# marianaGarcez/SpatialFlink

Measured on AMD Instinct MI355X. Metric: points/sec per window (kNN k=50, range r) at 1/2/4/8 MI355X; % HBM roofline, higher is better.
Workload: dtype f64

## Files before the change

### include/geoflink_hip.h

```cpp
#ifndef GEOFLINK_HIP_H
#define GEOFLINK_HIP_H

#include <stddef.h>
#include <stdint.h>

#ifdef __cplusplus
extern "C" {
#endif

#define GF_ABI_VERSION 2

#define GF_OK             0
#define GF_ERR_ARG       -1
#define GF_ERR_CAPACITY  -2
#define GF_ERR_HIP       -3
#define GF_ERR_NOMEM     -4
#define GF_ERR_LAYERS    -5
#define GF_ERR_ALIGN     -7
#define GF_ERR_COMM      -8

#define GF_METRIC_SQRT  0
#define GF_METRIC_HYPOT 1

#define GF_K_KNN_SCAN    0
#define GF_K_KNN_SAMPLE  1
#define GF_K_KNN_SELECT  2
#define GF_K_RANGE_SCAN  3
#define GF_K_ASSIGN      4
#define GF_K_JOIN_PROBE  5
#define GF_K_RANGE_TEST  6
#define GF_K_JOIN_BUCKET 7
#define GF_K_KNN_MERGE   8
#define GF_K_CSV_PARSE   9
#define GF_K_BUCKET      10
#define GF_K_JOIN_COMPACT 11
#define GF_K_TRAJ_GROUP  12
#define GF_K_TSTATS      13
#define GF_K_TRAJ_SELECT 14
#define GF_K_TAGG        15
#define GF_K_TKNN        16
#define GF_K_TJOIN       17
#define GF_K_TRANGE      18
#define GF_K_GEOM        19
#define GF_K_COUNT       20

typedef struct gf_ctx gf_ctx;

typedef struct {
  int32_t n;
  int32_t reserved;
  double minX, maxX, minY, maxY;
  double cellLength;
} gf_grid;

#define GF_OBJID_NUMERIC_MIN (-(INT64_C(1) << 62))
#define GF_OBJID_NUMERIC_END (INT64_C(1) << 62)
#define GF_OBJID_NULL INT64_MAX
typedef struct gf_objid_dict gf_objid_dict;

typedef struct {
  const double* x;
  const double* y;
  const int64_t* objID;
  const int64_t* ts;
  int64_t n;
} gf_points;

typedef struct {
  int32_t npoly;
  const int32_t* ring_off;
  const int32_t* vert_off;
  const double* vx;
  const double* vy;
} gf_polygons;

typedef struct {
  int32_t nline;
  const int32_t* vert_off;
  const double* vx;
  const double* vy;
} gf_linestrings;

int         gf_abi_version(void);
const char* gf_build_info(void);
int         gf_build_is_product(void);
const char* gf_status_string(int status);
int         gf_device_count(int* n);
int         gf_ctx_create(int device, gf_ctx** out);
void        gf_ctx_destroy(gf_ctx* ctx);
int         gf_ctx_set_stream(gf_ctx* ctx, void* hip_stream);
void*       gf_ctx_stream(gf_ctx* ctx);
int         gf_ctx_synchronize(gf_ctx* ctx);
int         gf_ctx_join(gf_ctx* ctx);
int         gf_ctx_fork(gf_ctx* ctx);
const char* gf_ctx_last_error(gf_ctx* ctx);
#define GF_FLAG_JOIN_LEGACY 1
#define GF_FLAG_JOIN_COARSE 2
#define GF_FLAG_GEOJSON_WALK 4
#define GF_FLAG_JOIN_STREAM 8
#define GF_FLAG_GEOJSON_WAVE 16
#define GF_FLAG_GEOJSON_CHECK 32
int gf_ctx_set_flag(gf_ctx* ctx, int flag, int value);
int gf_geojson_check_counts(gf_ctx* ctx, unsigned long long out[4]);

int         gf_ctx_set_timing(gf_ctx* ctx, int mask);
int         gf_ctx_set_timing_period(gf_ctx* ctx, int period);
int         gf_ctx_timing(gf_ctx* ctx, int kernel_id, double* total_ms, int64_t* launches);

int gf_grid_make(int32_t n, double minX, double maxX, double minY, double maxY, gf_grid* out);
int gf_grid_layers(const gf_grid* g, double r, int32_t* guaranteed, int32_t* candidate);
int gf_cell_of(const gf_grid* g, double x, double y, int32_t* cx, int32_t* cy);
int gf_format_cell_id(int32_t cx, int32_t cy, char* buf, int32_t cap);
int gf_parse_cell_id(const char* id, int32_t* cx, int32_t* cy);

int gf_assign_cells(gf_ctx* ctx, const gf_grid* g, const gf_points* pts, int32_t* cx, int32_t* cy);

int gf_bucket_by_cell(gf_ctx* ctx, const gf_grid* g, const gf_points* pts, uint32_t* perm,
                      uint32_t* cell_start);

int gf_shard_by_columns(gf_ctx* ctx, const gf_grid* g, const gf_points* pts, int32_t nbands, const int32_t* band_lo,
                        uint32_t* perm, uint32_t* offsets);
int gf_gather_points(gf_ctx* ctx, const gf_points* pts, const uint32_t* perm, int64_t begin, int64_t end, double* x,
                     double* y, int64_t* objID, int64_t* ts);

typedef struct gf_range_plan gf_range_plan;
int  gf_range_pp_plan_create(gf_ctx* ctx, const gf_grid* g, const double* qx, const double* qy,
                             int32_t nq, double r, int approximate, int metric, gf_range_plan** out);
int  gf_range_ppoly_plan_create(gf_ctx* ctx, const gf_grid* g, const gf_polygons* polys, double r,
                                int approximate, int metric, gf_range_plan** out);
void gf_range_plan_destroy(gf_range_plan* plan);
int  gf_range_run(gf_range_plan* plan, const gf_points* pts, uint64_t* bitmap,
                  uint64_t* multi_bitmap, int64_t* counts);
int  gf_range_run_batch(gf_range_plan* plan, int32_t nwin, const gf_points* pts, uint64_t* const* bitmaps,
                        int64_t* const* counts, uint32_t* const* idx, const int64_t* idx_cap, int64_t* const* idx_count);
int  gf_range_plan_stats(const gf_range_plan* plan, int64_t* none_cells, int64_t* candidate_cells,
                         int64_t* guaranteed_cells, int64_t* inside_cells);
int  gf_range_plan_set_tuning(gf_range_plan* plan, int32_t scan_blocks, int32_t defer_mode);
int  gf_range_plan_set_drain_lanes(gf_range_plan* plan, int32_t lanes);
int  gf_bitmap_to_indices(gf_ctx* ctx, const uint64_t* bitmap, int64_t n, uint32_t* idx,
                          int64_t cap, int64_t* count);
int  gf_bitmap_to_indices_async(gf_ctx* ctx, const uint64_t* bitmap, int64_t n, uint32_t* idx,
                                int64_t cap, int64_t* count);

typedef struct gf_knn_plan gf_knn_plan;
int    gf_knn_pp_plan_create(gf_ctx* ctx, const gf_grid* g, double qx, double qy, double r,
                             int32_t k, int metric, gf_knn_plan** out);
int    gf_knn_ppoly_plan_create(gf_ctx* ctx, const gf_grid* g, const gf_polygons* polys, double r, int32_t k,
                                int approximate, int metric, gf_knn_plan** out);
void   gf_knn_plan_destroy(gf_knn_plan* plan);
int    gf_knn_plan_set_capacity(gf_knn_plan* plan, int64_t cap);
int    gf_knn_plan_set_tuning(gf_knn_plan* plan, int32_t scan_blocks, int32_t unroll, int32_t nontemporal);
int    gf_knn_plan_set_hint(gf_knn_plan* plan, int enable);
int    gf_knn_plan_set_index_base(gf_knn_plan* plan, int64_t base);
int    gf_knn_plan_set_pipeline(gf_knn_plan* plan, int depth);
int    gf_knn_plan_flush(gf_knn_plan* plan);
typedef struct {
  int32_t status;
  int32_t n;
  int32_t k;
  int32_t flags;
  int64_t candidates;
  double threshold;
} gf_knn_header;
size_t gf_knn_result_bytes(int32_t k);
int    gf_knn_enqueue(gf_knn_plan* plan, const gf_points* pts, void* result);
int    gf_knn_decode(gf_knn_plan* plan, const gf_points* pts, const void* result_host,
                     int64_t* objID, double* dist, int64_t* idx, int32_t* n_out);
int    gf_knn_run(gf_knn_plan* plan, const gf_points* pts, int64_t* objID, double* dist,
                  int64_t* idx, int32_t* n_out);
int    gf_knn_merge_dev(gf_ctx* ctx, int32_t k, const void* records, int32_t nrec, void* result);
#define GF_MERGE_SHARD_MAJOR  0
#define GF_MERGE_WINDOW_MAJOR 1
#define GF_MERGE_FOREIGN_KEYS 0x100
#define GF_KNN_STATUS_FOREIGN_KEYS 2
int    gf_knn_merge_dev_batch(gf_ctx* ctx, int32_t k, const void* records, int32_t nrec, int32_t nwin,
                              int32_t layout, void* results);
size_t gf_knn_string_record_bytes(int32_t k, int64_t cap_bytes);
int gf_knn_attach_strings(gf_objid_dict* dict, int32_t k, const void* records, int32_t nrec, int64_t cap_bytes,
                          void* out);
int gf_knn_merge_dev_strings(gf_ctx* ctx, int32_t k, int64_t cap_bytes, const void* records, int32_t nrec,
                             int32_t nwin, int32_t layout, void* results);
int gf_knn_string_record_decode(const void* record, int32_t k, int64_t cap_bytes, int32_t* status, int64_t* objID,
                                double* dist, int64_t* idx, char* buf, int64_t buf_cap, int64_t* offs, int32_t* n_out);
int    gf_knn_merge_host(int32_t k, int32_t nlists, const int32_t* counts, const int64_t* objID,
                         const double* dist, const int64_t* idx, int64_t* out_objID,
                         double* out_dist, int64_t* out_idx, int32_t* n_out);

#define GF_COMM_ID_BYTES 128
typedef struct gf_comm gf_comm;
int  gf_comm_available(void);
int  gf_comm_unique_id(uint8_t* id);
int  gf_comm_create(const uint8_t* id, int32_t nranks, int32_t rank, int device, gf_comm** out);
int  gf_comm_create_all(int32_t ndev, const int* devices, gf_comm** out );
void gf_comm_destroy(gf_comm* comm);
int  gf_comm_info(const gf_comm* comm, int32_t* nranks, int32_t* rank, int* device);
const char* gf_comm_last_error(const gf_comm* comm);
int  gf_comm_check(gf_comm* comm);
int gf_knn_exchange_batch(gf_comm* comm, gf_ctx* ctx, int32_t k, const void* records, int32_t nwin, void* merged);
int gf_knn_exchange_strings_batch(gf_comm* comm, gf_objid_dict* dict, int32_t k, int64_t cap_bytes,
                                  const void* records, int32_t nwin, void* merged);
int gf_knn_exchange_group(int32_t n, gf_comm* const* comms, gf_ctx* const* ctxs, int32_t k,
                          const void* const* records, int32_t nwin, void* const* merged);

typedef struct gf_knn_sliding gf_knn_sliding;
int  gf_knn_sliding_create(gf_knn_plan* plan, int64_t size_ms, int64_t slide_ms, gf_knn_sliding** out);
void gf_knn_sliding_destroy(gf_knn_sliding* s);
int  gf_knn_sliding_geometry(const gf_knn_sliding* s, int64_t* pane_ms, int32_t* panes_per_window,
                             int32_t* panes_per_slide, int32_t* ring_panes);
int  gf_knn_sliding_push(gf_knn_sliding* s, int64_t pane_index, const gf_points* pane, void* window_result,
                         int32_t* closed, int64_t* window_end);
int  gf_knn_sliding_flush(gf_knn_sliding* s);
int  gf_knn_sliding_decode(gf_knn_sliding* s, int64_t window_end, const void* result_host, int64_t* objID,
                           double* dist, int64_t* idx, int32_t* n_out);

typedef struct gf_range_sliding gf_range_sliding;
int  gf_range_sliding_create(gf_range_plan* plan, int64_t size_ms, int64_t slide_ms, gf_range_sliding** out);
void gf_range_sliding_destroy(gf_range_sliding* s);
int  gf_range_sliding_geometry(const gf_range_sliding* s, int64_t* pane_ms, int32_t* panes_per_window,
                               int32_t* panes_per_slide);
int  gf_range_sliding_push(gf_range_sliding* s, int64_t pane_index, const gf_points* pane, uint32_t* idx,
                           int64_t cap, int64_t* count, int32_t* closed, int64_t* window_end, int64_t* window_n);

int  gf_pane_bounds(gf_ctx* ctx, const int64_t* ts, int64_t n, int64_t pane_ms, int64_t first_pane, int32_t npanes,
                    int64_t* bounds);

int  gf_objid_dict_create(gf_ctx* ctx, gf_objid_dict** out);
void gf_objid_dict_destroy(gf_objid_dict* d);
int  gf_ctx_objid_dict(gf_ctx* ctx, gf_objid_dict** out);
int  gf_objid_dict_size(const gf_objid_dict* d, int64_t* n);
int  gf_objid_intern(gf_objid_dict* d, const char* bytes, const int64_t* offs, int64_t n, int64_t* keys);
int  gf_objid_decode(gf_objid_dict* d, const int64_t* keys, int64_t n, char* buf, int64_t cap, int64_t* offs);

typedef struct {
  char delimiter;
  char reserved[3];
  int32_t objid_field;
  int32_t time_field;
  int32_t x_field;
  int32_t y_field;
} gf_csv_schema;
#define GF_CSV_OK              0
#define GF_CSV_NUMBER_FORMAT   1
#define GF_CSV_UNSUPPORTED     2
#define GF_CSV_MISSING_FIELD   3
#define GF_CSV_EMPTY_LINE      4
int gf_csv_parse(gf_ctx* ctx, const char* text, int64_t len, const gf_csv_schema* schema, const gf_grid* grid,
                 double* x, double* y, int64_t* objID, int64_t* ts, int32_t* cx, int32_t* cy, int64_t cap,
                 int64_t* n_out, int64_t* bad_line, int32_t* bad_kind);
int gf_csv_parse_dict(gf_ctx* ctx, gf_objid_dict* dict, const char* text, int64_t len, const gf_csv_schema* schema,
                      const gf_grid* grid, double* x, double* y, int64_t* objID, int64_t* ts, int32_t* cx, int32_t* cy,
                      int64_t cap, int64_t* n_out, int64_t* bad_line, int32_t* bad_kind);

typedef struct {
  const char* objid_property;
  const char* time_property;
  int32_t date_format;
  int32_t tz_offset_minutes;
  int32_t value_lines;
} gf_geojson_schema;
int gf_geojson_parse(gf_ctx* ctx, gf_objid_dict* dict, const char* text, int64_t len, const gf_geojson_schema* schema,
                     const gf_grid* grid, double* x, double* y, int64_t* objID, int64_t* ts, int32_t* cx,
                     int32_t* cy, int64_t cap, int64_t* n_out, int64_t* bad_line, int32_t* bad_kind);

typedef struct {
  int32_t kind;
  int64_t obj_cap, ring_cap, vert_cap;
  int32_t* ring_off;
  int32_t* vert_off;
  double *vx, *vy;
  int64_t *objID, *ts;
} gf_geoms_out;
int gf_geojson_parse_geoms(gf_ctx* ctx, gf_objid_dict* dict , const char* text, int64_t len,
                           const gf_geojson_schema* schema, const gf_geoms_out* out, int64_t* nobj, int64_t* nrings,
                           int64_t* nverts, int64_t* bad_line, int32_t* bad_kind);

int gf_join_pp(gf_ctx* ctx, const gf_grid* ugrid, const gf_grid* qgrid, const gf_points* ordinary,
               const gf_points* query, double r, int approximate, int metric, uint32_t* pairs,
               int64_t cap, int64_t* npairs);
int gf_join_pp_async(gf_ctx* ctx, const gf_grid* ugrid, const gf_grid* qgrid, const gf_points* ordinary,
                     const gf_points* query, double r, int approximate, int metric, uint32_t* pairs,
                     int64_t cap, unsigned long long* total);

int gf_join_ppoly_plan_create(gf_ctx* ctx, const gf_grid* qgrid, const gf_polygons* polys, double r,
                              int approximate, int metric, gf_range_plan** out);
int gf_join_ppoly_run(gf_range_plan* plan, const gf_grid* ugrid, const gf_points* points, uint32_t* pairs,
                      int64_t cap, int64_t* npairs);
int gf_join_ppoly(gf_ctx* ctx, const gf_grid* ugrid, const gf_grid* qgrid, const gf_points* points,
                  const gf_polygons* polys, double r, int approximate, int metric, uint32_t* pairs,
                  int64_t cap, int64_t* npairs);

int gf_range_pls_plan_create(gf_ctx* ctx, const gf_grid* g, const gf_linestrings* lines, double r,
                             int approximate, int metric, gf_range_plan** out);
int gf_knn_pls_plan_create(gf_ctx* ctx, const gf_grid* g, const gf_linestrings* lines , double r,
                           int32_t k, int approximate, int metric, gf_knn_plan** out);
int gf_join_pls_plan_create(gf_ctx* ctx, const gf_grid* qgrid, const gf_linestrings* lines, double r,
                            int approximate, int metric, gf_range_plan** out);
int gf_join_pls(gf_ctx* ctx, const gf_grid* ugrid, const gf_grid* qgrid, const gf_points* points,
                const gf_linestrings* lines, double r, int approximate, int metric, uint32_t* pairs,
                int64_t cap, int64_t* npairs);
int gf_range_plan_set_chain_mode(gf_range_plan* plan, int mode);
int gf_knn_plan_set_chain_mode(gf_knn_plan* plan, int mode);

typedef struct gf_traj_groups gf_traj_groups;
int  gf_traj_group(gf_ctx* ctx, const gf_points* pts, gf_traj_groups** out);
void gf_traj_groups_destroy(gf_traj_groups* g);
int  gf_traj_groups_info(const gf_traj_groups* g, int64_t* ntraj, int64_t* n);
int  gf_traj_groups_read(gf_traj_groups* g, int64_t* keys, int64_t* seg_off, uint32_t* perm);
int  gf_traj_groups_set_long_threshold(gf_traj_groups* g, int64_t len);
int  gf_tstats_run(gf_traj_groups* g, const gf_points* pts, const int64_t* id_set, int64_t nset,
                   int64_t* keys, double* spatial, int64_t* temporal, double* speed, int64_t cap, int64_t* count);
int  gf_traj_select(gf_traj_groups* g, const gf_points* pts, const uint64_t* bitmap, int64_t* keys, int64_t* off,
                    int64_t cap_traj, double* x, double* y, int64_t* ts, uint32_t* idx, int64_t cap_pts,
                    int64_t* ntraj_out, int64_t* npts_out);

typedef struct gf_tagg gf_tagg;
int  gf_tagg_group(gf_ctx* ctx, const gf_grid* grid, const gf_points* pts, gf_tagg** out);
int  gf_tagg_run(gf_tagg* t, const gf_points* pts);
void gf_tagg_destroy(gf_tagg* t);
int  gf_tagg_info(const gf_tagg* t, int64_t* cells, int64_t* groups, int64_t* n);
int  gf_tagg_set_thresholds(gf_tagg* t, int64_t long_group, int64_t big_cell);
int  gf_tagg_read_cells(gf_tagg* t, int32_t* cx, int32_t* cy, int64_t* count, int64_t* multi, int64_t* sum,
                        int64_t* minLen, int64_t* minKey, int64_t* maxLen, int64_t* maxKey, int64_t cap, int64_t* cells);
int  gf_tagg_read_all(gf_tagg* t, int64_t* off, int64_t* keys, int64_t* len, int64_t cap_cells, int64_t cap_groups,
                      int64_t* cells, int64_t* groups);
int  gf_tagg_rows(const char* function, int64_t cells, const int64_t* count, const int64_t* multi, const int64_t* sum,
                  const int64_t* minLen, const int64_t* minKey, const int64_t* maxLen, const int64_t* maxKey,
                  uint8_t* emit, int64_t* value, int64_t* key, int32_t* kind);

#define GF_TKNN_GRID  0
#define GF_TKNN_NAIVE 1
typedef struct gf_tknn gf_tknn;
int  gf_tknn_run(gf_traj_groups* g, const gf_grid* grid, const gf_points* pts, double qx, double qy, double r,
                 int32_t k, int mode, gf_tknn** out);
void gf_tknn_destroy(gf_tknn* t);
int  gf_tknn_info(const gf_tknn* t, int64_t* rows, int64_t* npts, int64_t* in_cells, int64_t* pairs, int64_t* records);
int  gf_tknn_read(gf_tknn* t, int64_t* keys, double* dist, int32_t* cells, int64_t* off, int64_t cap_rows, double* x,
                  double* y, int64_t* ts, uint32_t* idx, int64_t cap_pts);
int  gf_tknn_set_thresholds(gf_tknn* t, int64_t big_cell);

#define GF_TJOIN_PAIR 0
#define GF_TJOIN_SINGLE 1
typedef struct gf_tjoin gf_tjoin;
int  gf_tjoin_run(gf_traj_groups* go, const gf_points* opts, gf_traj_groups* gq, const gf_points* qpts,
                  const gf_grid* grid, double r, int mode, gf_tjoin** out);
void gf_tjoin_destroy(gf_tjoin* t);
int  gf_tjoin_info(const gf_tjoin* t, int64_t* rows, int64_t* emitted, int64_t* otraj, int64_t* opoints,
                   int64_t* qtraj, int64_t* qpoints, int64_t* probe_passes);
int  gf_tjoin_read_rows(gf_tjoin* t, int64_t* okey, int64_t* qkey, uint32_t* p_first, uint32_t* q_latest,
                        uint8_t* emit, int32_t* oslot, int32_t* qslot, int64_t cap);
int  gf_tjoin_read_trajs(gf_tjoin* t, int side, int64_t* keys, int64_t* off, int64_t cap_traj,
                         double* x, double* y, int64_t* ts, uint32_t* idx, int64_t cap_pts);
int  gf_tjoin_set_table_slots(gf_tjoin* t, int64_t slots);

typedef struct gf_trange_plan gf_trange_plan;
int  gf_trange_plan_create(gf_ctx* ctx, const gf_grid* g, const gf_polygons* polys, gf_trange_plan** out);
void gf_trange_plan_destroy(gf_trange_plan* p);
int  gf_trange_plan_stats(const gf_trange_plan* p, int64_t* none_cells, int64_t* test_cells, int64_t* inside_cells,
                          int64_t* list_entries, int64_t* wide_polygons);
int  gf_trange_plan_set_thresholds(gf_trange_plan* p, int32_t wide_ring);
int  gf_trange_points(gf_trange_plan* p, const gf_points* pts, uint64_t* bitmap, int64_t* count);
int  gf_trange_run(gf_trange_plan* p, gf_traj_groups* g, const gf_points* pts, int64_t* keys, int64_t* off,
                   int64_t cap_traj, double* x, double* y, int64_t* ts, uint32_t* idx, int64_t cap_pts,
                   int64_t* ntraj_out, int64_t* npts_out);
int  gf_trange_info(const gf_trange_plan* p, int64_t* cell_points, int64_t* inside_points, int64_t* wide_ring,
                    int64_t* wave_path);
int  gf_tfilter_run(gf_traj_groups* g, const gf_points* pts, const int64_t* id_set, int64_t nset, int64_t* keys,
                    int64_t* off, int64_t cap_traj, double* x, double* y, int64_t* ts, uint32_t* idx, int64_t cap_pts,
                    int64_t* ntraj_out, int64_t* npts_out);

#define GF_GEOM_POLYGON    1
#define GF_GEOM_LINESTRING 2
typedef struct {
  int32_t kind;
  int32_t nrings;
  int64_t nobj;
  const int32_t* ring_off;
  const int32_t* vert_off;
  const double* vx;
  const double* vy;
  const int64_t* objID;
  const int64_t* ts;
} gf_geoms;
typedef struct gf_geom_index gf_geom_index;
int  gf_geom_prepare(gf_ctx* ctx, const gf_grid* g, const gf_geoms* geoms, gf_geom_index** out);
void gf_geom_index_destroy(gf_geom_index* ix);
int  gf_geom_index_info(gf_geom_index* ix, int64_t* nobj, int64_t* nvert, int64_t* invalid, int64_t* wide);
int  gf_geom_index_read(gf_geom_index* ix, double* env, int32_t* cells);
int  gf_geom_index_set_thresholds(gf_geom_index* ix, int32_t wide_vertices);
typedef struct gf_geom_query gf_geom_query;
int  gf_geom_query_create(gf_ctx* ctx, const gf_grid* g, const double* qx, const double* qy, int32_t nq, double r,
                          int approximate, int metric, gf_geom_query** out);
void gf_geom_query_destroy(gf_geom_query* q);
int  gf_geom_range_run(gf_geom_query* q, gf_geom_index* ix, uint64_t* bitmap, int64_t* counts);
int  gf_geom_knn_enqueue(gf_geom_query* q, gf_geom_index* ix, int32_t k, void* result);
int  gf_geom_info(const gf_geom_query* q, int64_t* filtered, int64_t* all_guaranteed, int64_t* tested,
                  int64_t* wave_path);

int  gf_geom_query_create_polygons(gf_ctx* ctx, const gf_grid* g, const gf_polygons* polys, double r, int approximate,
                                   int metric, gf_geom_query** out);
int  gf_geom_query_create_linestrings(gf_ctx* ctx, const gf_grid* g, const gf_linestrings* lines, double r,
                                      int approximate, int metric, gf_geom_query** out);
int  gf_geom_query_set_chain_mode(gf_geom_query* q, int mode);

typedef struct gf_geom_join gf_geom_join;
int  gf_geom_join_create(gf_ctx* ctx, gf_geom_join** out);
void gf_geom_join_destroy(gf_geom_join* j);
int  gf_geom_join_run(gf_geom_join* j, gf_geom_index* ix_ord, gf_geom_index* ix_qry, double r, int approximate, int metric,
                      int first_is_ordinary, uint32_t* pairs, int64_t cap, int64_t* npairs, int64_t* nrep);
int  gf_geom_join_run_points(gf_geom_join* j, gf_geom_index* ix_ord, const gf_grid* qgrid, const gf_points* q, double r,
                             int approximate, int metric, uint32_t* pairs, int64_t cap, int64_t* npairs, int64_t* nrep);
int  gf_geom_join_info(const gf_geom_join* j, int64_t* candidates, int64_t* box_dropped, int64_t* tested,
                       int64_t* wave_path, int64_t* long_objects, int64_t* long_queries);
int  gf_geom_join_set_tuning(gf_geom_join* j, int32_t tile_side, int64_t long_tiles, int brute);

int  gf_pinned_alloc(size_t bytes, void** ptr);
void gf_pinned_free(void* ptr);

typedef struct gf_window gf_window;
int  gf_window_create(gf_ctx* ctx, int64_t capacity, gf_window** out);
void gf_window_destroy(gf_window* w);
int  gf_window_upload(gf_window* w, const double* x, const double* y, const int64_t* objID,
                      const int64_t* ts, int64_t n);
int  gf_window_points(gf_window* w, gf_points* out);
int  gf_window_upload_mapped(gf_window* w, const double* x, const double* y, const int64_t* objID_pinned, int64_t n);
int  gf_host_pinned(const void* p, int* pinned);

int gf_synth_uniform(int64_t seed, int64_t n, double minX, double maxX, double minY, double maxY,
                     double* x, double* y);

#ifdef __cplusplus
}
#endif
#endif
```

### spatialflink_amd/_lib.py

```python
from __future__ import annotations

import ctypes as C
import os
import threading

_HERE = os.path.dirname(os.path.abspath(__file__))
LIB_PATH = os.environ.get("GF_LIB_PATH") or os.path.join(_HERE, "libgeoflink_hip.so")

GF_OK = 0
OBJID_NUMERIC_MIN, OBJID_NUMERIC_END = -(1 << 62), 1 << 62
OBJID_NULL = (1 << 63) - 1
GF_MERGE_SHARD_MAJOR, GF_MERGE_WINDOW_MAJOR = 0, 1
GF_MERGE_FOREIGN_KEYS = 0x100
KNN_STATUS_FOREIGN_KEYS = 2
GF_ERR_ARG = -1
GF_ERR_CAPACITY = -2
GF_ERR_HIP = -3
GF_ERR_NOMEM = -4
GF_ERR_LAYERS = -5
GF_ERR_ALIGN = -7
GF_ERR_COMM = -8
GF_COMM_ID_BYTES = 128

METRIC_SQRT = 0
METRIC_HYPOT = 1
TKNN_GRID = 0
TKNN_NAIVE = 1
TJOIN_PAIR = 0
TJOIN_SINGLE = 1

FLAG_JOIN_LEGACY = 1
FLAG_JOIN_COARSE = 2
FLAG_GEOJSON_WALK = 4
FLAG_GEOJSON_WAVE = 16
FLAG_GEOJSON_CHECK = 32
FLAG_JOIN_STREAM = 8
(K_KNN_SCAN, K_KNN_SAMPLE, K_KNN_SELECT, K_RANGE_SCAN, K_ASSIGN, K_JOIN_PROBE, K_RANGE_TEST, K_JOIN_BUCKET,
 K_KNN_MERGE, K_CSV_PARSE, K_BUCKET, K_JOIN_COMPACT, K_TRAJ_GROUP, K_TSTATS, K_TRAJ_SELECT, K_TAGG, K_TKNN,
 K_TJOIN, K_TRANGE, K_GEOM) = range(20)
GEOM_POLYGON = 1
GEOM_LINESTRING = 2

EXPORTS = [
    "gf_abi_version", "gf_build_info", "gf_build_is_product", "gf_status_string", "gf_device_count", "gf_ctx_create", "gf_ctx_destroy",
    "gf_ctx_set_stream", "gf_ctx_stream", "gf_ctx_synchronize", "gf_ctx_join", "gf_ctx_fork", "gf_ctx_last_error", "gf_ctx_set_timing", "gf_ctx_set_timing_period", "gf_ctx_set_flag",
    "gf_geojson_check_counts",
    "gf_ctx_timing", "gf_grid_make", "gf_grid_layers", "gf_cell_of", "gf_format_cell_id", "gf_parse_cell_id",
    "gf_assign_cells", "gf_bucket_by_cell", "gf_range_pp_plan_create", "gf_range_ppoly_plan_create",
    "gf_range_plan_destroy", "gf_range_run", "gf_range_run_batch", "gf_range_plan_stats", "gf_range_plan_set_tuning", "gf_range_plan_set_drain_lanes", "gf_bitmap_to_indices", "gf_bitmap_to_indices_async", "gf_knn_pp_plan_create",
    "gf_knn_ppoly_plan_create",
    "gf_knn_plan_destroy", "gf_knn_plan_set_capacity", "gf_knn_plan_set_index_base", "gf_knn_plan_set_tuning", "gf_knn_plan_set_hint", "gf_knn_plan_set_pipeline", "gf_knn_plan_flush",
    "gf_knn_result_bytes", "gf_knn_enqueue",
    "gf_knn_decode", "gf_knn_run", "gf_knn_merge_dev", "gf_knn_merge_dev_batch", "gf_knn_merge_host",
    "gf_knn_sliding_create", "gf_knn_sliding_destroy", "gf_knn_sliding_geometry", "gf_knn_sliding_push",
    "gf_knn_sliding_flush", "gf_knn_sliding_decode", "gf_range_sliding_create", "gf_range_sliding_destroy",
    "gf_range_sliding_geometry", "gf_range_sliding_push", "gf_pane_bounds", "gf_csv_parse", "gf_csv_parse_dict", "gf_geojson_parse",
    "gf_geojson_parse_geoms",
    "gf_objid_dict_create", "gf_objid_dict_destroy", "gf_ctx_objid_dict", "gf_objid_dict_size", "gf_objid_intern",
    "gf_objid_decode", "gf_join_pp", "gf_join_pp_async",
    "gf_join_ppoly_plan_create", "gf_join_ppoly_run", "gf_join_ppoly",
    "gf_range_pls_plan_create", "gf_knn_pls_plan_create", "gf_join_pls_plan_create", "gf_join_pls",
    "gf_range_plan_set_chain_mode", "gf_knn_plan_set_chain_mode",
    "gf_window_create",
    "gf_window_destroy", "gf_window_upload", "gf_window_points", "gf_synth_uniform", "gf_pinned_alloc",
    "gf_pinned_free", "gf_knn_string_record_bytes", "gf_knn_attach_strings", "gf_knn_merge_dev_strings",
    "gf_knn_string_record_decode", "gf_window_upload_mapped", "gf_shard_by_columns", "gf_gather_points",
    "gf_host_pinned", "gf_comm_available", "gf_comm_unique_id", "gf_comm_create", "gf_comm_create_all",
    "gf_comm_destroy", "gf_comm_info", "gf_comm_last_error", "gf_comm_check", "gf_knn_exchange_batch",
    "gf_knn_exchange_strings_batch", "gf_knn_exchange_group",
    "gf_traj_group", "gf_traj_groups_destroy", "gf_traj_groups_info", "gf_traj_groups_read",
    "gf_traj_groups_set_long_threshold", "gf_tstats_run", "gf_traj_select",
    "gf_tagg_group", "gf_tagg_run", "gf_tagg_destroy", "gf_tagg_info", "gf_tagg_set_thresholds", "gf_tagg_read_cells",
    "gf_tagg_read_all", "gf_tagg_rows",
    "gf_tknn_run", "gf_tknn_destroy", "gf_tknn_info", "gf_tknn_read", "gf_tknn_set_thresholds",
    "gf_tjoin_run", "gf_tjoin_destroy", "gf_tjoin_info", "gf_tjoin_read_rows", "gf_tjoin_read_trajs",
    "gf_tjoin_set_table_slots",
    "gf_trange_plan_create", "gf_trange_plan_destroy", "gf_trange_plan_stats", "gf_trange_plan_set_thresholds",
    "gf_trange_points", "gf_trange_run", "gf_trange_info", "gf_tfilter_run",
    "gf_geom_prepare", "gf_geom_index_destroy", "gf_geom_index_info", "gf_geom_index_read",
    "gf_geom_index_set_thresholds", "gf_geom_query_create", "gf_geom_query_destroy", "gf_geom_range_run",
    "gf_geom_knn_enqueue", "gf_geom_info",
    "gf_geom_query_create_polygons", "gf_geom_query_create_linestrings", "gf_geom_query_set_chain_mode",
    "gf_geom_join_create", "gf_geom_join_destroy", "gf_geom_join_run", "gf_geom_join_run_points", "gf_geom_join_info",
    "gf_geom_join_set_tuning",
]


class GfGrid(C.Structure):
    _fields_ = [("n", C.c_int32), ("reserved", C.c_int32), ("minX", C.c_double), ("maxX", C.c_double),
                ("minY", C.c_double), ("maxY", C.c_double), ("cellLength", C.c_double)]


class GfPoints(C.Structure):
    _fields_ = [("x", C.c_void_p), ("y", C.c_void_p), ("objID", C.c_void_p), ("ts", C.c_void_p),
                ("n", C.c_int64)]


class GfPolygons(C.Structure):
    _fields_ = [("npoly", C.c_int32), ("ring_off", C.c_void_p), ("vert_off", C.c_void_p),
                ("vx", C.c_void_p), ("vy", C.c_void_p)]


class GfLineStrings(C.Structure):
    _fields_ = [("nline", C.c_int32), ("vert_off", C.c_void_p), ("vx", C.c_void_p), ("vy", C.c_void_p)]


class GfGeomsOut(C.Structure):
    _fields_ = [("kind", C.c_int32), ("obj_cap", C.c_int64), ("ring_cap", C.c_int64), ("vert_cap", C.c_int64),
                ("ring_off", C.c_void_p), ("vert_off", C.c_void_p), ("vx", C.c_void_p), ("vy", C.c_void_p),
                ("objID", C.c_void_p), ("ts", C.c_void_p)]


class GfGeoms(C.Structure):
    _fields_ = [("kind", C.c_int32), ("nrings", C.c_int32), ("nobj", C.c_int64), ("ring_off", C.c_void_p),
                ("vert_off", C.c_void_p), ("vx", C.c_void_p), ("vy", C.c_void_p), ("objID", C.c_void_p),
                ("ts", C.c_void_p)]


class GfKnnHeader(C.Structure):
    _fields_ = [("status", C.c_int32), ("n", C.c_int32), ("k", C.c_int32), ("flags", C.c_int32),
                ("candidates", C.c_int64), ("threshold", C.c_double)]


class GeoFlinkError(RuntimeError):
    def __init__(self, status, msg=""):
        self.status = status
        super().__init__(f"{msg} (status {status}: {status_string(status) if _lib else ''})")


class CandidateLayersError(GeoFlinkError):
    """The reference's System.exit(1): 'candidateNeighboringLayers cannot be 0 or less'
    (UniformGrid.java:272-276), raised instead of terminating the process."""


_lib = None
_lock = threading.Lock()


def lib():
    global _lib
    if _lib is not None:
        return _lib
    with _lock:
        if _lib is not None:
            return _lib
        if not os.path.exists(LIB_PATH):
            raise ImportError(
                f"{LIB_PATH} is missing: build it with `make` (or __graft_entry__.build()). "
                "There is no CPU fallback for the window-evaluation path.")
        import torch

        L = C.CDLL(LIB_PATH)
        P, i32, i64, d, sz = C.c_void_p, C.c_int32, C.c_int64, C.c_double, C.c_size_t
        pi32, pi64, pd = C.POINTER(i32), C.POINTER(i64), C.POINTER(d)
        sig = {
            "gf_abi_version": ([], C.c_int),
            "gf_build_info": ([], C.c_char_p),
            "gf_build_is_product": ([], C.c_int),
            "gf_status_string": ([C.c_int], C.c_char_p),
            "gf_device_count": ([C.POINTER(C.c_int)], C.c_int),
            "gf_ctx_create": ([C.c_int, C.POINTER(P)], C.c_int),
            "gf_ctx_destroy": ([P], None),
            "gf_ctx_set_stream": ([P, P], C.c_int),
            "gf_ctx_stream": ([P], P),
            "gf_ctx_synchronize": ([P], C.c_int),
            "gf_ctx_join": ([P], C.c_int),
            "gf_ctx_fork": ([P], C.c_int),
            "gf_ctx_last_error": ([P], C.c_char_p),
            "gf_ctx_set_timing": ([P, C.c_int], C.c_int),
            "gf_ctx_set_flag": ([P, C.c_int, C.c_int], C.c_int),
            "gf_geojson_check_counts": ([P, P], C.c_int),
            "gf_ctx_set_timing_period": ([P, C.c_int], C.c_int),
            "gf_ctx_timing": ([P, C.c_int, pd, pi64], C.c_int),
            "gf_grid_make": ([i32, d, d, d, d, C.POINTER(GfGrid)], C.c_int),
            "gf_grid_layers": ([C.POINTER(GfGrid), d, pi32, pi32], C.c_int),
            "gf_cell_of": ([C.POINTER(GfGrid), d, d, pi32, pi32], C.c_int),
            "gf_format_cell_id": ([i32, i32, C.c_char_p, i32], C.c_int),
            "gf_parse_cell_id": ([C.c_char_p, pi32, pi32], C.c_int),
            "gf_assign_cells": ([P, C.POINTER(GfGrid), C.POINTER(GfPoints), P, P], C.c_int),
            "gf_bucket_by_cell": ([P, C.POINTER(GfGrid), C.POINTER(GfPoints), P, P], C.c_int),
            "gf_range_pp_plan_create": ([P, C.POINTER(GfGrid), P, P, i32, d, C.c_int, C.c_int, C.POINTER(P)], C.c_int),
            "gf_range_ppoly_plan_create": ([P, C.POINTER(GfGrid), C.POINTER(GfPolygons), d, C.c_int, C.c_int,
                                            C.POINTER(P)], C.c_int),
            "gf_range_plan_destroy": ([P], None),
            "gf_range_run": ([P, C.POINTER(GfPoints), P, P, P], C.c_int),
            "gf_range_run_batch": ([P, i32, C.POINTER(GfPoints), C.POINTER(P), C.POINTER(P), C.POINTER(P), pi64,
                                    C.POINTER(P)], C.c_int),
            "gf_range_plan_stats": ([P, pi64, pi64, pi64, pi64], C.c_int),
            "gf_range_plan_set_tuning": ([P, C.c_int32, C.c_int32], C.c_int),
            "gf_range_plan_set_drain_lanes": ([P, i32], C.c_int),
            "gf_bitmap_to_indices": ([P, P, i64, P, i64, pi64], C.c_int),
            "gf_bitmap_to_indices_async": ([P, P, i64, P, i64, P], C.c_int),
            "gf_knn_pp_plan_create": ([P, C.POINTER(GfGrid), d, d, d, i32, C.c_int, C.POINTER(P)], C.c_int),
            "gf_knn_ppoly_plan_create": ([P, C.POINTER(GfGrid), C.POINTER(GfPolygons), d, i32, C.c_int, C.c_int,
                                          C.POINTER(P)], C.c_int),
            "gf_knn_plan_destroy": ([P], None),
            "gf_knn_plan_set_capacity": ([P, i64], C.c_int),
            "gf_knn_plan_set_index_base": ([P, i64], C.c_int),
            "gf_knn_plan_set_tuning": ([P, i32, i32, i32], C.c_int),
            "gf_knn_plan_set_hint": ([P, C.c_int], C.c_int),
            "gf_knn_plan_set_pipeline": ([P, C.c_int], C.c_int),
            "gf_knn_plan_flush": ([P], C.c_int),
            "gf_knn_result_bytes": ([i32], sz),
            "gf_knn_enqueue": ([P, C.POINTER(GfPoints), P], C.c_int),
            "gf_knn_decode": ([P, C.POINTER(GfPoints), P, P, P, P, pi32], C.c_int),
            "gf_knn_run": ([P, C.POINTER(GfPoints), P, P, P, pi32], C.c_int),
            "gf_knn_merge_dev": ([P, i32, P, i32, P], C.c_int),
            "gf_knn_merge_dev_batch": ([P, i32, P, i32, i32, i32, P], C.c_int),
            "gf_knn_merge_host": ([i32, i32, P, P, P, P, P, P, P, pi32], C.c_int),
            "gf_knn_sliding_create": ([P, i64, i64, C.POINTER(P)], C.c_int),
            "gf_knn_sliding_destroy": ([P], None),
            "gf_knn_sliding_geometry": ([P, pi64, pi32, pi32, pi32], C.c_int),
            "gf_knn_sliding_push": ([P, i64, C.POINTER(GfPoints), P, pi32, pi64], C.c_int),
            "gf_knn_sliding_flush": ([P], C.c_int),
            "gf_knn_sliding_decode": ([P, i64, P, P, P, P, pi32], C.c_int),
            "gf_range_sliding_create": ([P, i64, i64, C.POINTER(P)], C.c_int),
            "gf_range_sliding_destroy": ([P], None),
            "gf_range_sliding_geometry": ([P, pi64, pi32, pi32], C.c_int),
            "gf_range_sliding_push": ([P, i64, C.POINTER(GfPoints), P, i64, P, pi32, pi64, pi64], C.c_int),
            "gf_pane_bounds": ([P, P, i64, i64, i64, i32, P], C.c_int),
            "gf_csv_parse": ([P, P, i64, P, C.POINTER(GfGrid), P, P, P, P, P, P, i64, pi64, pi64, pi32], C.c_int),
            "gf_geojson_parse": ([P, P, P, i64, P, C.POINTER(GfGrid), P, P, P, P, P, P, i64, pi64, pi64, pi32],
                                 C.c_int),
            "gf_geojson_parse_geoms": ([P, P, P, i64, P, C.POINTER(GfGeomsOut), pi64, pi64, pi64, pi64, pi32], C.c_int),
            "gf_csv_parse_dict": ([P, P, P, i64, P, C.POINTER(GfGrid), P, P, P, P, P, P, i64, pi64, pi64, pi32],
                                  C.c_int),
            "gf_objid_dict_create": ([P, C.POINTER(P)], C.c_int),
            "gf_objid_dict_destroy": ([P], None),
            "gf_ctx_objid_dict": ([P, C.POINTER(P)], C.c_int),
            "gf_objid_dict_size": ([P, pi64], C.c_int),
            "gf_objid_intern": ([P, C.c_char_p, P, i64, P], C.c_int),
            "gf_objid_decode": ([P, P, i64, P, i64, P], C.c_int),
            "gf_join_pp": ([P, C.POINTER(GfGrid), C.POINTER(GfGrid), C.POINTER(GfPoints), C.POINTER(GfPoints), d,
                            C.c_int, C.c_int, P, i64, pi64], C.c_int),
            "gf_join_pp_async": ([P, C.POINTER(GfGrid), C.POINTER(GfGrid), C.POINTER(GfPoints), C.POINTER(GfPoints), d,
                                  C.c_int, C.c_int, P, i64, P], C.c_int),
            "gf_join_ppoly_plan_create": ([P, C.POINTER(GfGrid), C.POINTER(GfPolygons), d, C.c_int, C.c_int,
                                           C.POINTER(P)], C.c_int),
            "gf_join_ppoly_run": ([P, C.POINTER(GfGrid), C.POINTER(GfPoints), P, i64, pi64], C.c_int),
            "gf_join_ppoly": ([P, C.POINTER(GfGrid), C.POINTER(GfGrid), C.POINTER(GfPoints), C.POINTER(GfPolygons), d,
                               C.c_int, C.c_int, P, i64, pi64], C.c_int),
            "gf_range_pls_plan_create": ([P, C.POINTER(GfGrid), C.POINTER(GfLineStrings), d, C.c_int, C.c_int,
                                          C.POINTER(P)], C.c_int),
            "gf_knn_pls_plan_create": ([P, C.POINTER(GfGrid), C.POINTER(GfLineStrings), d, i32, C.c_int, C.c_int,
                                        C.POINTER(P)], C.c_int),
            "gf_join_pls_plan_create": ([P, C.POINTER(GfGrid), C.POINTER(GfLineStrings), d, C.c_int, C.c_int,
                                         C.POINTER(P)], C.c_int),
            "gf_join_pls": ([P, C.POINTER(GfGrid), C.POINTER(GfGrid), C.POINTER(GfPoints), C.POINTER(GfLineStrings), d,
                             C.c_int, C.c_int, P, i64, pi64], C.c_int),
            "gf_range_plan_set_chain_mode": ([P, C.c_int], C.c_int),
            "gf_knn_plan_set_chain_mode": ([P, C.c_int], C.c_int),
            "gf_window_create": ([P, i64, C.POINTER(P)], C.c_int),
            "gf_window_destroy": ([P], None),
            "gf_window_upload": ([P, P, P, P, P, i64], C.c_int),
            "gf_window_points": ([P, C.POINTER(GfPoints)], C.c_int),
            "gf_window_upload_mapped": ([P, P, P, P, i64], C.c_int),
            "gf_shard_by_columns": ([P, C.POINTER(GfGrid), C.POINTER(GfPoints), i32, P, P, P], C.c_int),
            "gf_gather_points": ([P, C.POINTER(GfPoints), P, i64, i64, P, P, P, P], C.c_int),
            "gf_host_pinned": ([P, C.POINTER(C.c_int)], C.c_int),
            "gf_synth_uniform": ([i64, i64, d, d, d, d, P, P], C.c_int),
            "gf_pinned_alloc": ([sz, C.POINTER(P)], C.c_int),
            "gf_pinned_free": ([P], None),
            "gf_knn_string_record_bytes": ([i32, i64], sz),
            "gf_knn_attach_strings": ([P, i32, P, i32, i64, P], C.c_int),
            "gf_knn_merge_dev_strings": ([P, i32, i64, P, i32, i32, i32, P], C.c_int),
            "gf_knn_string_record_decode": ([P, i32, i64, pi32, P, P, P, P, i64, P, pi32], C.c_int),
            "gf_comm_available": ([], C.c_int),
            "gf_comm_unique_id": ([P], C.c_int),
            "gf_comm_create": ([P, i32, i32, C.c_int, C.POINTER(P)], C.c_int),
            "gf_comm_create_all": ([i32, P, P], C.c_int),
            "gf_comm_destroy": ([P], None),
            "gf_comm_info": ([P, pi32, pi32, C.POINTER(C.c_int)], C.c_int),
            "gf_comm_last_error": ([P], C.c_char_p),
            "gf_comm_check": ([P], C.c_int),
            "gf_knn_exchange_batch": ([P, P, i32, P, i32, P], C.c_int),
            "gf_knn_exchange_strings_batch": ([P, P, i32, i64, P, i32, P], C.c_int),
            "gf_knn_exchange_group": ([i32, P, P, i32, P, i32, P], C.c_int),
            "gf_traj_group": ([P, C.POINTER(GfPoints), C.POINTER(P)], C.c_int),
            "gf_traj_groups_destroy": ([P], None),
            "gf_traj_groups_info": ([P, pi64, pi64], C.c_int),
            "gf_traj_groups_read": ([P, P, P, P], C.c_int),
            "gf_traj_groups_set_long_threshold": ([P, i64], C.c_int),
            "gf_tstats_run": ([P, C.POINTER(GfPoints), P, i64, P, P, P, P, i64, pi64], C.c_int),
            "gf_traj_select": ([P, C.POINTER(GfPoints), P, P, P, i64, P, P, P, P, i64, pi64, pi64], C.c_int),
            "gf_tagg_group": ([P, C.POINTER(GfGrid), C.POINTER(GfPoints), C.POINTER(P)], C.c_int),
            "gf_tagg_run": ([P, C.POINTER(GfPoints)], C.c_int),
            "gf_tagg_destroy": ([P], None),
            "gf_tagg_info": ([P, pi64, pi64, pi64], C.c_int),
            "gf_tagg_set_thresholds": ([P, i64, i64], C.c_int),
            "gf_tagg_read_cells": ([P, P, P, P, P, P, P, P, P, P, i64, pi64], C.c_int),
            "gf_tagg_read_all": ([P, P, P, P, i64, i64, pi64, pi64], C.c_int),
            "gf_tagg_rows": ([C.c_char_p, i64, P, P, P, P, P, P, P, P, P, P, pi32], C.c_int),
            "gf_tknn_run": ([P, C.POINTER(GfGrid), C.POINTER(GfPoints), C.c_double, C.c_double, C.c_double, C.c_int32,
                             C.c_int, C.POINTER(P)], C.c_int),
            "gf_tknn_destroy": ([P], None),
            "gf_tknn_info": ([P, pi64, pi64, pi64, pi64, pi64], C.c_int),
            "gf_tknn_read": ([P, P, P, P, P, i64, P, P, P, P, i64], C.c_int),
            "gf_tknn_set_thresholds": ([P, i64], C.c_int),
            "gf_tjoin_run": ([P, C.POINTER(GfPoints), P, C.POINTER(GfPoints), C.POINTER(GfGrid), C.c_double, C.c_int,
                              C.POINTER(P)], C.c_int),
            "gf_tjoin_destroy": ([P], None),
            "gf_tjoin_info": ([P, pi64, pi64, pi64, pi64, pi64, pi64, pi64], C.c_int),
            "gf_tjoin_read_rows": ([P, P, P, P, P, P, P, P, i64], C.c_int),
            "gf_tjoin_read_trajs": ([P, C.c_int, P, P, i64, P, P, P, P, i64], C.c_int),
            "gf_tjoin_set_table_slots": ([P, i64], C.c_int),
            "gf_trange_plan_create": ([P, C.POINTER(GfGrid), C.POINTER(GfPolygons), C.POINTER(P)], C.c_int),
            "gf_trange_plan_destroy": ([P], None),
            "gf_trange_plan_stats": ([P, pi64, pi64, pi64, pi64, pi64], C.c_int),
            "gf_trange_plan_set_thresholds": ([P, C.c_int32], C.c_int),
            "gf_trange_points": ([P, C.POINTER(GfPoints), P, P], C.c_int),
            "gf_trange_run": ([P, P, C.POINTER(GfPoints), P, P, i64, P, P, P, P, i64, pi64, pi64], C.c_int),
            "gf_trange_info": ([P, pi64, pi64, pi64, pi64], C.c_int),
            "gf_tfilter_run": ([P, C.POINTER(GfPoints), P, i64, P, P, i64, P, P, P, P, i64, pi64, pi64], C.c_int),
            "gf_geom_prepare": ([P, C.POINTER(GfGrid), C.POINTER(GfGeoms), C.POINTER(P)], C.c_int),
            "gf_geom_index_destroy": ([P], None),
            "gf_geom_index_info": ([P, pi64, pi64, pi64, pi64], C.c_int),
            "gf_geom_index_read": ([P, P, P], C.c_int),
            "gf_geom_index_set_thresholds": ([P, i32], C.c_int),
            "gf_geom_query_create": ([P, C.POINTER(GfGrid), P, P, i32, d, C.c_int, C.c_int, C.POINTER(P)], C.c_int),
            "gf_geom_query_destroy": ([P], None),
            "gf_geom_range_run": ([P, P, P, P], C.c_int),
            "gf_geom_knn_enqueue": ([P, P, i32, P], C.c_int),
            "gf_geom_info": ([P, pi64, pi64, pi64, pi64], C.c_int),
            "gf_geom_query_create_polygons": ([P, C.POINTER(GfGrid), C.POINTER(GfPolygons), d, C.c_int, C.c_int,
                                              C.POINTER(P)], C.c_int),
            "gf_geom_query_create_linestrings": ([P, C.POINTER(GfGrid), C.POINTER(GfLineStrings), d, C.c_int, C.c_int,
                                                 C.POINTER(P)], C.c_int),
            "gf_geom_query_set_chain_mode": ([P, C.c_int], C.c_int),
            "gf_geom_join_create": ([P, C.POINTER(P)], C.c_int),
            "gf_geom_join_destroy": ([P], None),
            "gf_geom_join_run": ([P, P, P, d, C.c_int, C.c_int, C.c_int, P, i64, pi64, pi64], C.c_int),
            "gf_geom_join_run_points": ([P, P, C.POINTER(GfGrid), C.POINTER(GfPoints), d, C.c_int, C.c_int, P, i64, pi64,
                                         pi64], C.c_int),
            "gf_geom_join_info": ([P, pi64, pi64, pi64, pi64, pi64, pi64], C.c_int),
            "gf_geom_join_set_tuning": ([P, i32, i64, C.c_int], C.c_int),
        }
        for name, (argt, rest) in sig.items():
            if os.environ.get("GF_LIB_PATH") and not hasattr(L, name):
                continue
            fn = getattr(L, name)
            fn.argtypes = argt
            fn.restype = rest
        _lib = L
        return _lib


def status_string(s):
    return lib().gf_status_string(int(s)).decode()


def check(status, ctx=None, what=""):
    if status == GF_OK:
        return
    detail = ""
    if ctx is not None:
        try:
            detail = lib().gf_ctx_last_error(ctx).decode()
        except Exception:
            detail = ""
    msg = f"{what}: {detail}" if detail else what
    if status == GF_ERR_LAYERS:
        raise CandidateLayersError(status, msg or "candidateNeighboringLayers cannot be 0 or less")
    if status == GF_ERR_ARG:
        raise ValueError(f"{msg} (IllegalArgumentException)")
    raise GeoFlinkError(status, msg)


class Context:

    def __init__(self, device: int = 0):
        h = C.c_void_p()
        st = lib().gf_ctx_create(int(device), C.byref(h))
        if st != GF_OK:
            raise GeoFlinkError(st, f"gf_ctx_create(device={device}) failed: is a GPU visible?")
        self.handle = h
        self.device = device

    def __del__(self):
        h = getattr(self, "handle", None)
        if h and _lib is not None:
            _lib.gf_ctx_destroy(h)
            self.handle = None

    def set_stream(self, stream_ptr: int | None):
        check(lib().gf_ctx_set_stream(self.handle, C.c_void_p(stream_ptr or 0)), self.handle, "set_stream")

    def synchronize(self):
        check(lib().gf_ctx_synchronize(self.handle), self.handle, "synchronize")

    def set_timing(self, mask: int):
        check(lib().gf_ctx_set_timing(self.handle, int(mask)), self.handle, "set_timing")

    def set_timing_period(self, period: int):
        check(lib().gf_ctx_set_timing_period(self.handle, int(period)), self.handle, "set_timing_period")

    def timing(self, kernel_id: int):
        ms, n = C.c_double(), C.c_int64()
        check(lib().gf_ctx_timing(self.handle, int(kernel_id), C.byref(ms), C.byref(n)), self.handle, "timing")
        return ms.value, n.value


_ctx_cache: dict = {}


def context(device: int | None = None) -> Context:
    import torch

    if device is None:
        device = torch.cuda.current_device()
    key = (int(device), threading.get_ident())
    ctx = _ctx_cache.get(key)
    if ctx is None:
        ctx = Context(int(device))
        _ctx_cache[key] = ctx
    ctx.set_stream(torch.cuda.current_stream(device).cuda_stream)
    return ctx


def device_count() -> int:
    n = C.c_int()
    lib().gf_device_count(C.byref(n))
    return n.value
```

### spatialflink_amd/csrc/geomingest.cpp

```cpp
#define GF_TU_NAME geomingest_cpp
#include "gf_buildtag.hpp"

#include <cstring>
#include <string>

#include "gf_host.hpp"
#include "k_geomingest.hpp"

using namespace gf;

constexpr int64_t kGeomMeanLineDefault = 768;

static int32_t geom_lds_cap(int64_t mean) {
  const int64_t cap = (mean * kGeomLines * 5 / 4 + 1023) & ~(int64_t)1023;
  return (int32_t)std::min<int64_t>(std::max<int64_t>(cap, 16 * 1024), kCsvLdsMax);
}

static int geom_bad_line(gf_ctx* ctx, const CsvErr& he, int64_t* bad_line, int32_t* bad_kind) {
  if (bad_line) *bad_line = (int64_t)he.line;
  if (bad_kind) *bad_kind = he.kind;
  static const char* what[] = {"ok", "a position's ordinate is not a number",
                               "outside the restated subset (see gf_geojson_parse_geoms)",
                               "malformed JSON / no geometry / a ring or linestring JTS refuses", "empty line"};
  const int k = he.kind >= 0 && he.kind <= 4 ? he.kind : 1;
  return set_err(ctx, GF_ERR_ARG, "gf_geojson_parse_geoms: line " + std::to_string(he.line) + ": " + what[k]);
}

extern "C" int gf_geojson_parse_geoms(gf_ctx* ctx, gf_objid_dict* dict, const char* text, int64_t len,
                                      const gf_geojson_schema* sc, const gf_geoms_out* out, int64_t* nobj,
                                      int64_t* nrings, int64_t* nverts, int64_t* bad_line, int32_t* bad_kind) {
  if (!ctx) return GF_ERR_ARG;
  const char* fn = "gf_geojson_parse_geoms: ";
  if (!sc || (sc->date_format != 0 && sc->date_format != 1) || (sc->value_lines != 0 && sc->value_lines != 1))
    return set_err(ctx, GF_ERR_ARG, std::string(fn) + "bad schema");
  if (!out || (out->kind != GF_GEOM_POLYGON && out->kind != GF_GEOM_LINESTRING))
    return set_err(ctx, GF_ERR_ARG, std::string(fn) + "kind must be GF_GEOM_POLYGON or GF_GEOM_LINESTRING");
  const bool poly = out->kind == GF_GEOM_POLYGON;
  const int64_t obj_cap = out->obj_cap, ring_cap = poly ? out->ring_cap : 0, vert_cap = out->vert_cap;
  const bool any_cap = obj_cap > 0 || ring_cap > 0 || vert_cap > 0;
  if (!nobj || !nrings || !nverts || len < 0 || (len > 0 && !text) || obj_cap < 0 || out->ring_cap < 0 || vert_cap < 0 ||
      (obj_cap > 0 && (!out->objID || !out->ts)) || (vert_cap > 0 && (!out->vx || !out->vy)) ||
      (any_cap && !out->vert_off) || (poly && any_cap && !out->ring_off))
    return set_err(ctx, GF_ERR_ARG, std::string(fn) + "bad argument");
  if ((uintptr_t)text & 15) return set_err(ctx, GF_ERR_ALIGN, std::string(fn) + "text must be 16-byte aligned");
  if (len >= ((int64_t)1 << 33)) return set_err(ctx, GF_ERR_ARG, std::string(fn) + "text of 8 GiB or more");
  if (dict && dict->ctx != ctx) return set_err(ctx, GF_ERR_ARG, std::string(fn) + "dictionary of another context");
  GeomIngestArgs a{};
  a.len_obj = a.len_ts = -1;
  for (int k = 0; k < 2; ++k) {
    const char* name = k ? sc->time_property : sc->objid_property;
    if (!name) continue;
    const size_t n = std::strlen(name);
    if (n >= (size_t)kGeoPropMax) return set_err(ctx, GF_ERR_ARG, std::string(fn) + "property name longer than 63 bytes");
    std::memcpy(k ? a.prop_ts : a.prop_obj, name, n);
    (k ? a.len_ts : a.len_obj) = (int32_t)n;
  }
  int st = bind(ctx);
  if (st) return st;
  if (!dict && (st = ctx_dict(ctx, &dict))) return st;
  *nobj = *nrings = *nverts = 0;
  if (bad_line) *bad_line = -1;
  if (bad_kind) *bad_kind = GF_CSV_OK;
  if (len == 0) {
    if (out->vert_off) GF_HIP_CHECK(ctx, hipMemsetAsync(out->vert_off, 0, sizeof(int32_t), ctx->stream));
    if (poly && out->ring_off) GF_HIP_CHECK(ctx, hipMemsetAsync(out->ring_off, 0, sizeof(int32_t), ctx->stream));
    GF_HIP_CHECK(ctx, hipStreamSynchronize(ctx->stream));
    return GF_OK;
  }
  a.text = text;
  a.len = len;
  a.kind = out->kind;
  a.value_lines = sc->value_lines;
  a.date_fmt = sc->date_format;
  a.tz_off_ms = (int64_t)sc->tz_offset_minutes * 60000;
  a.lds_cap = geom_lds_cap(ctx->geom_mean_line > 0 ? ctx->geom_mean_line : kGeomMeanLineDefault);
  const int64_t nseg = (len + kCsvSeg - 1) / kCsvSeg;
  int64_t nl_cap = len / 32 + 2;
  GeomHead h{};
  GeomHead* d_head = nullptr;
  for (int pass = 0; pass < 2; ++pass) {
    const int64_t G = nl_cap + 1;
    Arena ar;
    uint32_t *tot = nullptr, *cnt_r = nullptr, *cnt_v = nullptr, *off_r = nullptr, *off_v = nullptr;
    CsvErr* err = nullptr;
    int64_t* nl = nullptr;
    ar.take(d_head, 1);
    ar.take(tot, 1);
    ar.take(err, 1);
    ar.take(nl, (size_t)nl_cap);
    ar.take(cnt_r, (size_t)G);
    ar.take(cnt_v, (size_t)G);
    ar.take(off_r, (size_t)G + 1);
    ar.take(off_v, (size_t)G + 1);
    ar.take(a.cpos, (size_t)G);
    ar.take(a.tcode, (size_t)G);
    ar.take(a.ts_s, (size_t)G);
    ar.take(a.obj_s, (size_t)G);
    const size_t tmp_n = (size_t)std::max<int64_t>(ring_cap, 1);
    ar.take(a.tmp.area, tmp_n);
    ar.take(a.tmp.start, tmp_n);
    ar.take(a.tmp.count, tmp_n);
    ar.take(a.tmp.order, tmp_n);
    if ((st = ar.alloc(ctx))) return st;
    if ((st = dict_reserve_batch(dict, (uint64_t)G, (uint64_t)G))) return st;
    if ((st = lookback_launch(ctx, nseg, nseg, "launch_csv_nlindex", [&](const ExpandState& es) {
          return launch_csv_nlindex(ctx->stream, text, len, nseg, nl, nl_cap, tot, es, err, dict->counters + 2);
        })))
      return st;
    a.nl = nl;
    a.nl_total = tot;
    a.nl_cap = nl_cap;
    a.grid_lines = G;
    a.cnt_r = cnt_r;
    a.cnt_v = cnt_v;
    a.off_r = off_r;
    a.off_v = off_v;
    a.err = err;
    a.head = d_head;
    a.dict_work = (DictWork*)dict->work[0];
    a.dict_n = (uint32_t*)(dict->counters + 2);
    a.dict_bytes = dict->counters + 3;
    GF_HIP_CHECK(ctx, launch_geomingest_a(ctx, a));
    if ((st = scan1(ctx, cnt_r, G, off_r))) return st;
    if ((st = scan1(ctx, cnt_v, G, off_v))) return st;
    GF_HIP_CHECK(ctx, launch_geomingest_head(ctx, a));
    if ((st = read_scalar_sync(ctx, d_head, &h))) return st;
    if ((int64_t)h.newlines <= nl_cap) break;
    nl_cap = (int64_t)h.newlines + 1;
  }
  const int64_t lines = (int64_t)h.lines;
  if (lines >= (int64_t)INT32_MAX) return set_err(ctx, GF_ERR_ARG, std::string(fn) + "2^31 - 1 lines or more");
  if (h.err.line != ~0ull) {
    a.fill = 0;
    a.limit = (int64_t)h.err.line;
    if (a.limit > 0) {
      GF_HIP_CHECK(ctx, launch_geomingest_b(ctx, a));
      GF_HIP_CHECK(ctx, launch_geomingest_head(ctx, a));
      if ((st = read_scalar_sync(ctx, d_head, &h))) return st;
    }
    return geom_bad_line(ctx, h.err, bad_line, bad_kind);
  }
  if (h.nrings > (unsigned long long)INT32_MAX || h.nverts > (unsigned long long)INT32_MAX)
    return set_err(ctx, GF_ERR_ARG, std::string(fn) + "the window's rings or vertices do not fit int32 offsets");
  *nobj = lines;
  *nrings = (int64_t)h.nrings;
  *nverts = (int64_t)h.nverts;
  ctx->geom_mean_line = (len + lines - 1) / lines;
  if (lines > obj_cap || *nrings > ring_cap || *nverts > vert_cap)
    return set_err(ctx, GF_ERR_CAPACITY, std::string(fn) + "the window exceeds a capacity (counts returned)");
  a.fill = 1;
  a.limit = lines;
  a.lds_cap = geom_lds_cap(ctx->geom_mean_line);
  a.ring_off = out->ring_off;
  a.vert_off = out->vert_off;
  a.vx = out->vx;
  a.vy = out->vy;
  a.objID = out->objID;
  a.ts = out->ts;
  GF_HIP_CHECK(ctx, launch_geomingest_b(ctx, a));
  GF_HIP_CHECK(ctx, launch_geomingest_head(ctx, a));
  if ((st = read_scalar_sync(ctx, d_head, &h))) return st;
  if (h.err.line != ~0ull) return geom_bad_line(ctx, h.err, bad_line, bad_kind);
  const uint32_t nw = (uint32_t)h.dict_n;
  if (nw > 0) {
    if ((st = dict_reserve_table(dict, nw, h.dict_bytes))) return st;
    if ((st = dict_run(dict, text, 1, nw, (uint64_t)lines, out->objID))) return st;
  }
  return GF_OK;
}
```

### spatialflink_amd/csrc/gf_geojson.hpp

```cpp
#pragma once

#include <cstdint>

#include "gf_text.hpp"

namespace gf {

GF_DHD inline bool jws(char c) { return c == ' ' || c == '\t' || c == '\n' || c == '\r'; }
template <class Src>
GF_DHD inline int64_t jskip(const Src& s, int64_t p, int64_t e) {
  while (p < e && jws(s(p))) ++p;
  return p;
}
template <class Src>
GF_DHD inline int64_t jstr_end(const Src& s, int64_t p, int64_t e, bool* esc) {
  for (++p; p < e; ++p) {
    const char c = s(p);
    if (c == '\\') {
      *esc = true;
      ++p;
    } else if (c == '"') {
      return p + 1;
    }
  }
  return -1;
}
template <class Src>
GF_DHD inline int64_t jval_end(const Src& s, int64_t p, int64_t e) {
  char c = s(p);
  if (c == '"') {
    bool esc = false;
    return jstr_end(s, p, e, &esc);
  }
  if (c == '{' || c == '[') {
    int depth = 0;
    while (p < e) {
      c = s(p);
      if (c == '"') {
        bool esc = false;
        p = jstr_end(s, p, e, &esc);
        if (p < 0) return -1;
        continue;
      }
      if (c == '{' || c == '[') ++depth;
      else if ((c == '}' || c == ']') && --depth == 0) return p + 1;
      ++p;
    }
    return -1;
  }
  int64_t q = p;
  while (q < e && !(s(q) == ',' || s(q) == '}' || s(q) == ']' || jws(s(q)))) ++q;
  return q > p ? q : -1;
}
template <class Src>
GF_DHD inline int64_t jfind(const Src& s, int64_t p, int64_t e, const char* key, int klen) {
  int64_t found = -1;
  bool esc_key = false;
  p = jskip(s, p + 1, e);
  if (p < e && s(p) == '}') return -1;
  while (p < e && s(p) == '"') {
    bool esc = false;
    const int64_t ke = jstr_end(s, p, e, &esc);
    if (ke < 0) return -3;
    esc_key |= esc;
    bool match = !esc && ke - p - 2 == klen;
    for (int i = 0; match && i < klen; ++i) match = s(p + 1 + i) == key[i];
    p = jskip(s, jskip(s, ke, e) + 1, e);
    const int64_t ve = jval_end(s, p, e);
    if (ve < 0) return -3;
    if (match) found = p;
    p = jskip(s, ve, e);
    if (p >= e || s(p) != ',') break;
    p = jskip(s, p + 1, e);
  }
  return esc_key ? -3 : found;
}
template <class Src>
GF_DHD inline bool jnumber(const Src& s, int64_t p, int64_t q, bool* integral) {
  int64_t i = p;
  if (i < q && s(i) == '-') ++i;
  if (i >= q) return false;
  if (s(i) == '0') ++i;
  else if (s(i) >= '1' && s(i) <= '9') while (i < q && s(i) >= '0' && s(i) <= '9') ++i;
  else return false;
  *integral = true;
  if (i < q && s(i) == '.') {
    *integral = false;
    const int64_t d = ++i;
    while (i < q && s(i) >= '0' && s(i) <= '9') ++i;
    if (i == d) return false;
  }
  if (i < q && (s(i) == 'e' || s(i) == 'E')) {
    *integral = false;
    ++i;
    if (i < q && (s(i) == '+' || s(i) == '-')) ++i;
    const int64_t d = i;
    while (i < q && s(i) >= '0' && s(i) <= '9') ++i;
    if (i == d) return false;
  }
  return i == q;
}
GF_DHD inline int64_t days_from_civil(int64_t y, int64_t m) {
  y -= m <= 2;
  const int64_t era = (y >= 0 ? y : y - 399) / 400;
  const int64_t yoe = y - era * 400;
  const int64_t doy = (153 * (m + (m > 2 ? -3 : 9)) + 2) / 5;
  return era * 146097 + yoe * 365 + yoe / 4 - yoe / 100 + doy - 719468;
}
template <class Src>
GF_DHD inline int jdate(const Src& s, int64_t p, int64_t q, int64_t tz_off_ms, int64_t* ms) {
  const char sep[5] = {'-', '-', ' ', ':', ':'};
  int64_t f[6];
  for (int k = 0; k < 6; ++k) {
    int nd = 0;
    int64_t v = 0;
    while (p < q && s(p) >= '0' && s(p) <= '9' && nd < 10) {
      v = v * 10 + (s(p) - '0');
      ++p;
      ++nd;
    }
    if (nd == 0) return 1;
    if (nd == 10) return 2;
    f[k] = v;
    if (k < 5) {
      if (p >= q || s(p) != sep[k]) return 1;
      ++p;
    }
  }
  const int64_t m0 = f[1] - 1;
  const int64_t y = f[0] + (m0 >= 0 ? m0 / 12 : (m0 - 11) / 12);
  const int64_t m = m0 - 12 * (y - f[0]) + 1;
  const int64_t days = days_from_civil(y, m) + f[2] - 1;
  const int64_t secs = ((days * 24 + f[3]) * 60 + f[4]) * 60 + f[5];
  if (secs < -12219292800ll) return 2;
  *ms = secs * 1000 - tz_off_ms;
  return 0;
}

constexpr int kGeoMaxDepth = 256;
GF_DHD inline bool jtok_char(char c) {
  return (c >= '0' && c <= '9') || (c >= 'a' && c <= 'z') || (c >= 'A' && c <= 'Z') || c == '+' || c == '-' || c == '.';
}
template <class Src>
GF_DHD inline bool jtoo_deep(const Src& s, int64_t p, int64_t e) {
  int d = 0;
  bool str = false;
  for (int64_t i = p; i < e; ++i) {
    const char c = s(i);
    if (str) {
      if (c == '\\') ++i;
      else if (c == '"') str = false;
    } else if (c == '"') {
      str = true;
    } else if (c == '{' || c == '[') {
      if (++d > kGeoMaxDepth) return true;
    } else if (c == '}' || c == ']') {
      --d;
    }
  }
  return false;
}
GF_DHD inline bool jhex(char c) { return (c >= '0' && c <= '9') || (c >= 'a' && c <= 'f') || (c >= 'A' && c <= 'F'); }
template <class Src>
GF_DHD inline int64_t jstr_valid(const Src& s, int64_t p, int64_t e) {
  for (++p; p < e; ++p) {
    const uint8_t c = (uint8_t)s(p);
    if (c == '"') return p + 1;
    if (c < 0x20) return -1;
    if (c == '\\') {
      if (++p >= e) return -1;
      const char x = s(p);
      if (x == 'u') {
        if (p + 4 >= e) return -1;
        for (int k = 1; k <= 4; ++k)
          if (!jhex(s(p + k))) return -1;
        p += 4;
      } else if (!(x == '"' || x == '\\' || x == '/' || x == 'b' || x == 'f' || x == 'n' || x == 'r' || x == 't')) {
        return -1;
      }
    } else if (c >= 0x80) {
      const int n = (c & 0xE0) == 0xC0 ? 1 : (c & 0xF0) == 0xE0 ? 2 : (c & 0xF8) == 0xF0 ? 3 : -1;
      if (n < 0) return -1;
      for (int k = 0; k < n; ++k)
        if (++p >= e || ((uint8_t)s(p) & 0xC0) != 0x80) return -1;
    }
  }
  return -1;
}
template <class Src>
GF_DHD inline int jtok_valid(const Src& s, int64_t p, int64_t q, const uint64_t* T) {
  const int64_t n = q - p;
  const char c = s(p);
  if (c == 't' || c == 'f' || c == 'n') {
    const char* w = c == 't' ? "true" : c == 'f' ? "false" : "null";
    const int wl = c == 'f' ? 5 : 4;
    if (n != wl) return 1;
    for (int k = 0; k < wl; ++k)
      if (s(p + k) != w[k]) return 1;
    return 0;
  }
  bool integral;
  if (!jnumber(s, p, q, &integral)) return 1;
  if (integral) {
    int64_t v;
    return n < 19 || parse_java_long(s, Field{p, q}, &v) == kNumOk ? 0 : 2;
  }
  double v;
  if (parse_java_double(s, Field{p, q}, T, &v) != kNumOk) return 2;
  return (v == v && v - v != 0.0) ? 2 : 0;
}
template <class Src>
GF_DHD GF_NOINLINE int jvalidate(Src s, int64_t p, int64_t e, const uint64_t* T) {
  if (jtoo_deep(s, p, e)) return kCsvUnsupported;
  enum { V, A0, K0, K, CO, AF };
  uint64_t obj[kGeoMaxDepth / 64] = {0, 0, 0, 0};
  int depth = 0, st = V;
  bool poison = false;
  int64_t i = p;
  while (true) {
    i = jskip(s, i, e);
    if (i >= e) break;
    const char c = s(i);
    if (st == V || st == A0) {
      if (c == '{' || c == '[') {
        const int d = depth++;
        const uint64_t bit = 1ull << (d & 63);
        obj[d >> 6] = c == '{' ? obj[d >> 6] | bit : obj[d >> 6] & ~bit;
        st = c == '{' ? K0 : A0;
        ++i;
      } else if (c == '"') {
        if ((i = jstr_valid(s, i, e)) < 0) return kCsvMissingField;
        st = AF;
      } else if (jtok_char(c)) {
        int64_t q = i;
        while (q < e && jtok_char(s(q))) ++q;
        const int t = jtok_valid(s, i, q, T);
        if (t == 1) return kCsvMissingField;
        poison |= t == 2;
        i = q;
        st = AF;
      } else if (st == A0 && c == ']') {
        --depth;
        ++i;
        st = AF;
      } else {
        return kCsvMissingField;
      }
    } else if (st == K0 || st == K) {
      if (c == '"') {
        if ((i = jstr_valid(s, i, e)) < 0) return kCsvMissingField;
        st = CO;
      } else if (st == K0 && c == '}') {
        --depth;
        ++i;
        st = AF;
      } else {
        return kCsvMissingField;
      }
    } else if (st == CO) {
      if (c != ':') return kCsvMissingField;
      ++i;
      st = V;
    } else {
      if (depth == 0) return kCsvMissingField;
      const bool isobj = (obj[(depth - 1) >> 6] >> ((depth - 1) & 63)) & 1;
      if (c == ',') {
        st = isobj ? K : V;
      } else if (c == (isobj ? '}' : ']')) {
        --depth;
        st = AF;
      } else {
        return kCsvMissingField;
      }
      ++i;
    }
  }
  if (st != AF || depth != 0) return kCsvMissingField;
  return poison ? kCsvUnsupported : kCsvOk;
}

struct GeoPos {
  int64_t V, tV, cV, gV, tG, cG, prV, tsP, qP;
  bool escV, escG, escP;
};
enum { kTyNone, kTyPoint, kTyOtherGeom, kTyFeature, kTyFeatureColl, kTyEscaped,
       kTyLineString, kTyPolygon, kTyMultiPoint, kTyMultiLineString, kTyMultiPolygon, kTyGeomColl };
template <class Src>
GF_DHD inline int geo_type_full(const Src& s, int64_t t, int64_t e) {
  if (t < 0 || s(t) != '"') return kTyNone;
  bool esc = false;
  const int64_t te = jstr_end(s, t, e, &esc);
  if (esc) return kTyEscaped;
  const int n = (int)(te - t - 2);
  auto is = [&](const char* w, int wl) {
    if (n != wl) return false;
    for (int k = 0; k < wl; ++k)
      if (s(t + 1 + k) != w[k]) return false;
    return true;
  };
  if (is("Point", 5)) return kTyPoint;
  if (is("LineString", 10)) return kTyLineString;
  if (is("Polygon", 7)) return kTyPolygon;
  if (is("MultiPoint", 10)) return kTyMultiPoint;
  if (is("MultiLineString", 15)) return kTyMultiLineString;
  if (is("MultiPolygon", 12)) return kTyMultiPolygon;
  if (is("GeometryCollection", 18)) return kTyGeomColl;
  if (is("Feature", 7)) return kTyFeature;
  if (is("FeatureCollection", 17)) return kTyFeatureColl;
  return kTyNone;
}
template <class Src>
GF_DHD inline int geo_type(const Src& s, int64_t t, int64_t e) {
  const int ty = geo_type_full(s, t, e);
  return ty >= kTyLineString ? (int)kTyOtherGeom : ty;
}
template <class Src>
GF_DHD inline int point_coords(const Src& s, int64_t c, int64_t e, const uint64_t* T, double* x, double* y) {
  if (c < 0 || s(c) != '[') return kCsvMissingField;
  int64_t i = jskip(s, c + 1, e);
  double x0 = 0.0, y0 = 0.0;
  int n = 0;
  while (i < e && s(i) != ']') {
    const int64_t ve = jval_end(s, i, e);
    if (n < 3) {
      const char c0 = s(i);
      if (c0 == '-' || (c0 >= '0' && c0 <= '9')) {
        if (n < 2) {
          bool integral = false;
          jnumber(s, i, ve, &integral);
          double v;
          const int st = parse_java_double(s, Field{i, ve}, T, &v);
          if (st) return st == kNumUnsupported ? kCsvUnsupported : kCsvNumberFormat;
          v = integral && v == 0.0 ? 0.0 : v;
          if (n == 0) x0 = v;
          else y0 = v;
        }
      } else {
        return n < 2 ? kCsvNumberFormat : kCsvUnsupported;
      }
    }
    ++n;
    i = jskip(s, ve, e);
    if (i < e && s(i) == ',') i = jskip(s, i + 1, e);
  }
  if (n < 2) return kCsvUnsupported;
  *x = x0;
  *y = y0;
  return kCsvOk;
}

struct GeoProps {
  const char* kts;
  const char* kobj;
  int32_t len_ts, len_obj, date_fmt;
  int64_t tz_off_ms;
  const uint64_t* pow5;
};

template <class Src>
GF_DHD inline int geo_props(const GeoProps& a, const Src& s, int64_t e, int64_t t, int64_t q, LineOut* o) {
  if (a.len_ts >= 0 && t >= 0) {
    const int64_t te = jval_end(s, t, e);
    if (a.date_fmt == 0) {
      bool integral;
      if (!jnumber(s, t, te, &integral) || !integral) return kCsvNumberFormat;
      if (parse_java_long(s, Field{t, te}, &o->ts)) return kCsvNumberFormat;
    } else {
      if (s(t) != '"') return kCsvNumberFormat;
      bool esc = false;
      jstr_end(s, t, e, &esc);
      if (esc) return kCsvUnsupported;
      int64_t ms = 0;
      const int st = jdate(s, t + 1, te - 1, a.tz_off_ms, &ms);
      if (st == 2) return kCsvUnsupported;
      if (st == 0) o->ts = ms;
    }
  }
  if (a.len_obj >= 0 && q >= 0) {
    const int64_t qe = jval_end(s, q, e);
    Field f{q, qe};
    const char c0 = s(q);
    if (c0 == '"') {
      bool esc = false;
      jstr_end(s, q, e, &esc);
      if (esc) return kCsvUnsupported;
      f = Field{q + 1, qe - 1};
    } else if (c0 == '{' || c0 == '[') {
      return kCsvUnsupported;
    } else if (c0 == '-' || (c0 >= '0' && c0 <= '9')) {
      bool integral;
      jnumber(s, q, qe, &integral);
      if (!integral) return kCsvUnsupported;
      if (qe - q == 2 && c0 == '-' && s(q + 1) == '0') {
        o->obj = 0;
        return kCsvOk;
      }
    }
    o->dict = !canonical_objid_key(s, f, &o->obj);
    o->f_obj = f;
    if (o->dict && f.e - f.b > (int64_t)kDictLenMask) return kCsvUnsupported;
  }
  return kCsvOk;
}

template <class Src>
GF_DHD inline int geo_eval_body(const GeoProps& a, const Src& s, int64_t e, const GeoPos& g, LineOut* o) {
  if (g.V < 0 || s(g.V) != '{') return kCsvMissingField;
  if (g.escV) return kCsvUnsupported;
  o->ts = 0;
  o->obj = GF_OBJID_NULL;
  o->dict = false;
  bool have = false;
  const int tv = geo_type(s, g.tV, e);
  if (tv == kTyOtherGeom || tv == kTyFeatureColl || tv == kTyEscaped) return kCsvUnsupported;
  if (tv == kTyPoint) {
    const int st = point_coords(s, g.cV, e, a.pow5, &o->x, &o->y);
    if (st == kCsvUnsupported) return st;
    have = st == kCsvOk;
  }
  if (!have) {
    if (g.gV < 0 || s(g.gV) != '{') return kCsvMissingField;
    if (g.escG) return kCsvUnsupported;
    const int tg = geo_type(s, g.tG, e);
    if (tg == kTyNone) return kCsvMissingField;
    if (tg != kTyPoint) return kCsvUnsupported;
    const int st = point_coords(s, g.cG, e, a.pow5, &o->x, &o->y);
    if (st) return st;
  }
  if (g.prV < 0 || s(g.prV) != '{') return kCsvOk;
  if (g.escP && (a.len_ts >= 0 || a.len_obj >= 0)) return kCsvUnsupported;
  return geo_props(a, s, e, g.tsP, g.qP, o);
}
template <class Src>
GF_DHD GF_NOINLINE int geo_eval(const GeoProps& a, const Src& s, int64_t e, const GeoPos& g, LineOut* o) {
  return geo_eval_body(a, s, e, g, o);
}

template <class Src>
GF_DHD inline int geo_walk_find(const GeoProps& a, const Src& s, int64_t p, int64_t e, int vlines, GeoPos* gp) {
  GeoPos g{-1, -1, -1, -1, -1, -1, -1, -1, -1, false, false, false};
  auto find = [&](int64_t obj, const char* k, int kl, int64_t* out) {
    if (obj < 0 || s(obj) != '{') return true;
    const int64_t f = jfind(s, obj, e, k, kl);
    *out = f < 0 ? -1 : f;
    return f != -3;
  };
  if (vlines) g.V = p;
  else if (!find(p, "value", 5, &g.V)) return kCsvUnsupported;
  g.escV = !find(g.V, "type", 4, &g.tV);
  find(g.V, "coordinates", 11, &g.cV);
  find(g.V, "geometry", 8, &g.gV);
  find(g.V, "properties", 10, &g.prV);
  g.escG = !find(g.gV, "type", 4, &g.tG);
  find(g.gV, "coordinates", 11, &g.cG);
  g.escP = !find(g.prV, a.kts, a.len_ts >= 0 ? a.len_ts : 0, &g.tsP);
  find(g.prV, a.kobj, a.len_obj >= 0 ? a.len_obj : 0, &g.qP);
  *gp = g;
  return kCsvOk;
}
template <class Src>
GF_DHD GF_NOINLINE int eval_geojson_walk(GeoProps a, Src s, int64_t p, int64_t e, int vlines, LineOut* o) {
  const int vs = jvalidate(s, p, e, a.pow5);
  if (vs) return vs;
  GeoPos g;
  const int fs = geo_walk_find(a, s, p, e, vlines, &g);
  if (fs) return fs;
  return geo_eval(a, s, e, g, o);
}

enum : uint8_t { JS_VAL, JS_ARR0, JS_OBJ0, JS_KEY, JS_COLON, JS_AFT, JS_VSTR, JS_KSTR, JS_TOK, JS_N, JS_ERR = 9 };
enum : uint8_t { JC_WS, JC_LBRACE, JC_RBRACE, JC_LBRACK, JC_RBRACK, JC_QUOTE, JC_COMMA, JC_COLON, JC_BSL, JC_TOK,
                 JC_OTHER, JC_WSC, JC_CTRL, JC_HIGH };
enum : uint8_t { JA_NONE, JA_PUSH_OBJ, JA_PUSH_ARR, JA_POP_OBJ, JA_POP_ARR, JA_COMMA, JA_KEY_BEGIN, JA_KEY_END };
enum : int { JR_NONE, JR_TOP, JR_VAL, JR_GEO, JR_PROP };
enum : int { JK_NONE, JK_VALUE, JK_GEO, JK_PROP };
enum : uint8_t { TS_IDLE, TS_S0, TS_NEED1, TS_NEED2, TS_NEED3, TS_MINUS, TS_ZERO, TS_INT, TS_DOT, TS_FRAC, TS_E,
                 TS_ESIGN, TS_EXP1, TS_EXP2, TS_LIT, TS_ERR };
constexpr uint32_t kTsAccept = (1u << TS_ZERO) | (1u << TS_INT) | (1u << TS_FRAC) | (1u << TS_EXP1) | (1u << TS_EXP2);
constexpr int kGeoKeys = 7;

GF_DHD inline uint8_t jclass(int c) {
  switch (c) {
    case ' ': return JC_WS;
    case '\t': case '\n': case '\r': return JC_WSC;
    case '{': return JC_LBRACE;
    case '}': return JC_RBRACE;
    case '[': return JC_LBRACK;
    case ']': return JC_RBRACK;
    case '"': return JC_QUOTE;
    case ',': return JC_COMMA;
    case ':': return JC_COLON;
    case '\\': return JC_BSL;
    default: break;
  }
  if (c < 0x20) return JC_CTRL;
  if (c >= 0x80) return JC_HIGH;
  if ((c >= '0' && c <= '9') || (c >= 'a' && c <= 'z') || (c >= 'A' && c <= 'Z') || c == '+' || c == '-' || c == '.')
    return JC_TOK;
  return JC_OTHER;
}
GF_DHD inline uint8_t jtrans(int st, int cl) {
  auto E = [](int n, int act) { return (uint8_t)(n | act << 4); };
  if (st == JS_VSTR || st == JS_KSTR) {
    if (cl == JC_QUOTE) return st == JS_VSTR ? E(JS_AFT, 0) : E(JS_COLON, JA_KEY_END);
    if (cl == JC_BSL || cl == JC_WSC || cl == JC_CTRL) return E(JS_ERR, 0);
    return E(st, 0);
  }
  if (st == JS_TOK) {
    if (cl == JC_TOK) return E(JS_TOK, 0);
    st = JS_AFT;
  }
  if (cl == JC_WS || cl == JC_WSC) return E(st, 0);
  switch (st) {
    case JS_VAL: case JS_ARR0:
      if (cl == JC_LBRACE) return E(JS_OBJ0, JA_PUSH_OBJ);
      if (cl == JC_LBRACK) return E(JS_ARR0, JA_PUSH_ARR);
      if (cl == JC_QUOTE) return E(JS_VSTR, 0);
      if (cl == JC_TOK) return E(JS_TOK, 0);
      if (st == JS_ARR0 && cl == JC_RBRACK) return E(JS_AFT, JA_POP_ARR);
      return E(JS_ERR, 0);
    case JS_OBJ0:
      if (cl == JC_QUOTE) return E(JS_KSTR, JA_KEY_BEGIN);
      if (cl == JC_RBRACE) return E(JS_AFT, JA_POP_OBJ);
      return E(JS_ERR, 0);
    case JS_KEY: return cl == JC_QUOTE ? E(JS_KSTR, JA_KEY_BEGIN) : E(JS_ERR, 0);
    case JS_COLON: return cl == JC_COLON ? E(JS_VAL, 0) : E(JS_ERR, 0);
    case JS_AFT:
      if (cl == JC_COMMA) return E(JS_VAL, JA_COMMA);
      if (cl == JC_RBRACE) return E(JS_AFT, JA_POP_OBJ);
      if (cl == JC_RBRACK) return E(JS_AFT, JA_POP_ARR);
      return E(JS_ERR, 0);
    default: return E(JS_ERR, 0);
  }
}
GF_DHD inline uint8_t jtok_trans(int t, int b) {
  const bool dig = b >= '0' && b <= '9', e = b == 'e' || b == 'E';
  const bool let = (b >= 'a' && b <= 'z') || (b >= 'A' && b <= 'Z');
  switch (t) {
    case TS_IDLE:
      if (b == '"') return TS_S0;
      if (b == '-') return TS_MINUS;
      if (b == '0') return TS_ZERO;
      if (dig) return TS_INT;
      if (b == 't' || b == 'f' || b == 'n') return TS_LIT;
      return TS_ERR;
    case TS_S0:
      if (b < 0x80) return TS_S0;
      if ((b & 0xE0) == 0xC0) return TS_NEED1;
      if ((b & 0xF0) == 0xE0) return TS_NEED2;
      if ((b & 0xF8) == 0xF0) return TS_NEED3;
      return TS_ERR;
    case TS_NEED1: return (b & 0xC0) == 0x80 ? TS_S0 : TS_ERR;
    case TS_NEED2: return (b & 0xC0) == 0x80 ? TS_NEED1 : TS_ERR;
    case TS_NEED3: return (b & 0xC0) == 0x80 ? TS_NEED2 : TS_ERR;
    case TS_MINUS: return b == '0' ? TS_ZERO : dig ? TS_INT : TS_ERR;
    case TS_ZERO: return b == '.' ? TS_DOT : e ? TS_E : TS_ERR;
    case TS_INT: return dig ? TS_INT : b == '.' ? TS_DOT : e ? TS_E : TS_ERR;
    case TS_DOT: return dig ? TS_FRAC : TS_ERR;
    case TS_FRAC: return dig ? TS_FRAC : e ? TS_E : TS_ERR;
    case TS_E: return dig ? TS_EXP1 : (b == '+' || b == '-') ? TS_ESIGN : TS_ERR;
    case TS_ESIGN: return dig ? TS_EXP1 : TS_ERR;
    case TS_EXP1: return dig ? TS_EXP2 : TS_ERR;
    case TS_EXP2: return TS_ERR;
    case TS_LIT: return let ? TS_LIT : TS_ERR;
    default: return TS_ERR;
  }
}

struct K16 {
  uint64_t hi, lo;
};
GF_DHD constexpr K16 geo_pack16(const char* s, int n) {
  uint64_t hi = 0, lo = 0;
  for (int i = 0; i < n; ++i) {
    hi = (hi << 8) | (lo >> 56);
    lo = (lo << 8) | (uint8_t)s[i];
  }
  return K16{hi, lo};
}
struct GeoTabs {
  GF_LDS_PTR(uint64_t) tab;
  GF_LDS_PTR(uint64_t) ttab;
  GF_LDS_PTR(char) keys;
  int32_t klen[kGeoKeys];
  K16 pts, pobj;
};

template <class Src>
GF_DHD inline bool jkey_eq(const Src& s, int64_t ks, int len, const GeoTabs& gt, int k) {
  if (gt.klen[k] != len) return false;
  bool eq = true;
  for (int i = 0; eq && i < len; ++i) eq = s(ks + i) == gt.keys[k * kGeoPropMax + i];
  return eq;
}

template <class Src>
GF_DHD inline int64_t jmember_value(const Src& s, int64_t k, int64_t e) {
  return jskip(s, jskip(s, k + 1, e) + 1, e);
}

enum { GN_V, GN_TV, GN_CV, GN_GV, GN_PRV, GN_TG, GN_CG, GN_TP, GN_QP, kGeoNotes };
struct GeoLoc {
  int st, depth, pend;
  uint32_t ts;
  bool bad;
  uint64_t kinds;
  uint32_t roles;
  int32_t ks, tb;
  uint64_t khi, klo;
  int32_t n[kGeoNotes];
};
GF_DHD inline void geo_loc_init(GeoLoc& L) {
  L.st = JS_VAL;
  L.depth = 0;
  L.pend = JK_NONE;
  L.ts = TS_IDLE;
  L.bad = false;
  L.kinds = 0;
  L.roles = 0;
  L.ks = 0;
  L.tb = 0;
  L.khi = 0;
  L.klo = 0;
  for (int k = 0; k < kGeoNotes; ++k) L.n[k] = -1;
}
GF_DHD inline void geo_step(GeoLoc& L, uint32_t byte, int32_t i, const LBytes& s, int64_t p, const GeoTabs& gt,
                            int top_role) {
  constexpr K16 kValue = geo_pack16("value", 5), kGeom = geo_pack16("geometry", 8);
  constexpr K16 kProps = geo_pack16("properties", 10), kCoord = geo_pack16("coordinates", 11);
  constexpr K16 kType = geo_pack16("type", 4);
  const int32_t lts = gt.klen[4], lobj = gt.klen[5];
  const int st = L.st;
  const uint32_t ts = L.ts;
  const uint32_t ent = (uint32_t)(gt.tab[byte] >> (7 * st)) & 0x7Fu;
  const uint32_t nts = (uint32_t)(gt.ttab[byte] >> (4 * ts)) & 15u;
  int nst = (int)(ent & 15u);
  const int act = (int)(ent >> 4);
  const bool in_tok = nst == JS_TOK, in_str = nst == JS_VSTR || nst == JS_KSTR;
  const bool tok_end = st == JS_TOK && !in_tok;
  const bool lit = tok_end && ts == TS_LIT;
  bool bad = L.bad;
  bad |= tok_end && !lit && !(((kTsAccept >> ts) & 1u) && i - L.tb < 19);
  if (lit) {
    const int n = i - L.tb;
    const char c0 = s(p + L.tb);
    bool ok = n == (c0 == 'f' ? 5 : 4);
    const char* wd = c0 == 't' ? "true" : c0 == 'f' ? "false" : "null";
    for (int q = 1; ok && q < n; ++q) ok = s(p + L.tb + q) == wd[q];
    bad |= !ok;
  }
  L.tb = in_tok && st != JS_TOK ? i : L.tb;
  bad |= (in_str || st == JS_VSTR || st == JS_KSTR) && nts == TS_ERR;
  L.ts = in_tok || in_str ? nts : TS_IDLE;
  const bool in_key = st == JS_KSTR && nst == JS_KSTR;
  const uint64_t khi = L.khi, klo = L.klo;
  const uint64_t nhi = (khi << 8) | (klo >> 56), nlo = (klo << 8) | byte;
  const bool kb = act == JA_KEY_BEGIN;
  L.khi = kb ? 0ull : in_key ? nhi : khi;
  L.klo = kb ? 0ull : in_key ? nlo : klo;
  L.ks = kb ? i + 1 : L.ks;
  const int depth = L.depth;
  const int role = (unsigned)depth <= 7u ? (int)(L.roles >> (4 * depth)) & 15 : JR_NONE;
  const bool push = act == JA_PUSH_OBJ || act == JA_PUSH_ARR, pop = act == JA_POP_OBJ || act == JA_POP_ARR;
  int child = depth == 0 ? top_role
            : role == JR_TOP ? (int)(0x0020u >> (4 * L.pend)) & 15
            : role == JR_VAL ? (int)(0x4300u >> (4 * L.pend)) & 15
            : JR_NONE;
  child = act == JA_PUSH_ARR ? JR_NONE : child;
  const int nd = depth + 1;
  const uint64_t nbit = 1ull << (nd & 63);
  L.kinds = push ? (act == JA_PUSH_OBJ ? L.kinds | nbit : L.kinds & ~nbit) : L.kinds;
  const uint32_t rsh = 4u * (uint32_t)(nd & 7);
  L.roles = push && nd <= 7 ? (L.roles & ~(15u << rsh)) | ((uint32_t)child << rsh) : L.roles;
  const bool kobj = (L.kinds >> (depth & 63)) & 1;
  bad |= push && nd > 63;
  bad |= pop && (depth <= 0 || kobj != (act == JA_POP_OBJ));
  bad |= act == JA_COMMA && depth <= 0;
  nst = act == JA_COMMA ? (kobj ? JS_KEY : JS_VAL) : nst;
  L.depth = depth + (int)push - (int)pop;
  const bool kend = act == JA_KEY_END;
  const int len = i - L.ks;
  const uint64_t chi = L.khi, clo = L.klo;
  const bool e_type = len == 4 && clo == kType.lo, e_value = len == 5 && clo == kValue.lo;
  const bool e_geom = len == 8 && clo == kGeom.lo;
  const bool e_props = len == 10 && clo == kProps.lo && chi == kProps.hi;
  const bool e_coord = len == 11 && clo == kCoord.lo && chi == kCoord.hi;
  const bool top = kend && role == JR_TOP, val = kend && role == JR_VAL;
  const bool geo = kend && role == JR_GEO, prop = kend && role == JR_PROP;
  const bool m_value = top && e_value;
  const bool v_type = val && e_type, v_coord = val && e_coord;
  const bool v_geom = val && e_geom, v_props = val && e_props;
  bool p_ts = prop && len == lts && lts <= 16 && clo == gt.pts.lo && chi == gt.pts.hi;
  bool p_obj = prop && len == lobj && lobj <= 16 && clo == gt.pobj.lo && chi == gt.pobj.hi;
  if ((lts > 16 || lobj > 16) && prop && len > 16) {
    p_ts = jkey_eq(s, p + L.ks, len, gt, 4);
    p_obj = jkey_eq(s, p + L.ks, len, gt, 5);
  }
  L.pend = kend ? (m_value ? JK_VALUE : v_geom ? JK_GEO : v_props ? JK_PROP : JK_NONE) : L.pend;
  L.n[GN_V] = m_value ? i : L.n[GN_V];
  L.n[GN_TV] = v_type ? i : L.n[GN_TV];
  L.n[GN_CV] = v_coord ? i : L.n[GN_CV];
  L.n[GN_GV] = v_geom ? i : L.n[GN_GV];
  L.n[GN_PRV] = v_props ? i : L.n[GN_PRV];
  L.n[GN_TG] = geo && e_type ? i : L.n[GN_TG];
  L.n[GN_CG] = geo && e_coord ? i : L.n[GN_CG];
  L.n[GN_TP] = p_ts ? i : L.n[GN_TP];
  L.n[GN_QP] = p_obj ? i : L.n[GN_QP];
  bad |= nst == JS_ERR;
  L.bad = bad;
  L.st = nst == JS_ERR ? JS_AFT : nst;
}
GF_DHD inline bool geo_loc_ok(const GeoLoc& L) { return !L.bad && L.st == JS_AFT && L.depth == 0; }
template <class Src>
GF_DHD inline void geo_notes_pos(const Src& s, int64_t p, int64_t e, int vlines, const int32_t* n, GeoPos* g) {
  auto val = [&](int32_t k) { return k < 0 ? (int64_t)-1 : jmember_value(s, p + k, e); };
  const int32_t vb = vlines ? -1 : n[GN_V];
  g->V = vlines ? p : val(n[GN_V]);
  g->tV = val(n[GN_TV] > vb ? n[GN_TV] : -1);
  g->cV = val(n[GN_CV] > vb ? n[GN_CV] : -1);
  const int32_t gv = n[GN_GV] > vb ? n[GN_GV] : -1, pv = n[GN_PRV] > vb ? n[GN_PRV] : -1;
  g->gV = val(gv);
  g->tG = val(gv >= 0 && n[GN_TG] > gv ? n[GN_TG] : -1);
  g->cG = val(gv >= 0 && n[GN_CG] > gv ? n[GN_CG] : -1);
  g->prV = val(pv);
  g->tsP = val(pv >= 0 && n[GN_TP] > pv ? n[GN_TP] : -1);
  g->qP = val(pv >= 0 && n[GN_QP] > pv ? n[GN_QP] : -1);
  g->escV = g->escG = g->escP = false;
}
#ifndef GF_GEO_UNROLL
#define GF_GEO_UNROLL 2
#endif
GF_DHD inline void geo_word(GeoLoc& L, int32_t w, int32_t o0, int32_t o1, const LBytes& s, int64_t p, const GeoTabs& gt,
                            int top_role) {
  const uint32_t word = *reinterpret_cast<const uint32_t*>(s.p + w);
#pragma unroll GF_GEO_UNROLL
  for (int k = 0; k < 4; ++k) {
    const int32_t i = w + k - o0;
    const uint32_t byte = i < 0 || w + k >= o1 ? (uint32_t)' ' : (word >> (8 * k)) & 0xFFu;
    geo_step(L, byte, i, s, p, gt, top_role);
  }
}

GF_DHD inline bool geo_locate_notes(const LBytes& s, int64_t p, int64_t e, const GeoTabs& gt, int vlines,
                                    int32_t* n) {
  if (e - p >= INT32_MAX) return false;
  GeoLoc L;
  geo_loc_init(L);
  const int top_role = vlines ? JR_VAL : JR_TOP;
  const int32_t o0 = (int32_t)(p - s.base), o1 = (int32_t)(e - s.base);
  for (int32_t w = o0 & ~3; w < o1 && !L.bad; w += 4) geo_word(L, w, o0, o1, s, p, gt, top_role);
  if (!geo_loc_ok(L)) return false;
  for (int k = 0; k < kGeoNotes; ++k) n[k] = L.n[k];
  return true;
}
GF_DHD inline bool geo_locate(const LBytes& s, int64_t p, int64_t e, const GeoTabs& gt, int vlines,
                                           GeoPos* g) {
  int32_t n[kGeoNotes];
  if (!geo_locate_notes(s, p, e, gt, vlines, n)) return false;
  geo_notes_pos(s, p, e, vlines, n, g);
  return true;
}


template <class Src>
GF_DHD inline int geojson_line(const GeoTabs& gt, const GeoProps& gp, const Src& s, int64_t p, int64_t e, int vlines,
                               LineOut* o) {
  LineOut w{0, 0, 0.0, 0.0, false, {0, 0}};
  const int st = eval_geojson_walk(gp, s, p, e, vlines, &w);
  *o = w;
  return st;
}
GF_DHD inline int geojson_line(const GeoTabs& gt, const GeoProps& gp, const LBytes& s, int64_t p, int64_t e,
                               int vlines, bool fast, LineOut* o) {
  if (fast) {
    GeoPos g;
    if (geo_locate(s, p, e, gt, vlines, &g)) return geo_eval_body(gp, s, e, g, o);
  }
  LineOut w{0, 0, 0.0, 0.0, false, {0, 0}};
  const int st = eval_geojson_walk(gp, s, p, e, vlines, &w);
  *o = w;
  return st;
}

enum : uint32_t {
  WB_Q = 1u << 0,
  WB_BAD = 1u << 1,
  WB_WSC = 1u << 2,
  WB_OTH = 1u << 3,
  WB_OB = 1u << 4, WB_CB = 1u << 5, WB_OA = 1u << 6, WB_CA = 1u << 7, WB_CO = 1u << 8, WB_CM = 1u << 9,
  WB_TOK = 1u << 10,
  WB_DOT = 1u << 11, WB_E = 1u << 12
};
enum : uint32_t { WT_NONE, WT_OB, WT_OA, WT_CB, WT_CA, WT_CO, WT_CM, WT_SK, WT_SV, WT_TK };
constexpr uint32_t kWtValueEnd = (1u << WT_CB) | (1u << WT_CA) | (1u << WT_SV) | (1u << WT_TK);
GF_DHD inline uint32_t wave_class(int b) {
  const int cl = jclass(b);
  uint32_t f = 0, t = WT_NONE;
  switch (cl) {
    case JC_QUOTE: f = WB_Q; t = WT_SV; break;
    case JC_BSL: case JC_CTRL: case JC_HIGH: f = WB_BAD; break;
    case JC_WSC: f = WB_WSC; break;
    case JC_OTHER: f = WB_OTH; break;
    case JC_LBRACE: f = WB_OB; t = WT_OB; break;
    case JC_RBRACE: f = WB_CB; t = WT_CB; break;
    case JC_LBRACK: f = WB_OA; t = WT_OA; break;
    case JC_RBRACK: f = WB_CA; t = WT_CA; break;
    case JC_COLON: f = WB_CO; t = WT_CO; break;
    case JC_COMMA: f = WB_CM; t = WT_CM; break;
    case JC_TOK:
      f = WB_TOK | (b == '.' ? WB_DOT : 0u) | (b == 'e' || b == 'E' ? WB_E : 0u);
      t = WT_TK;
      break;
    default: break;
  }
  return f | t << 24;
}

GF_DHD inline void geo_tab_entry(int b, uint64_t* tab, uint64_t* ttab) {
  const int cl = jclass(b);
  uint64_t t = 0, u = 0;
  for (int st = 0; st < JS_N; ++st) t |= (uint64_t)jtrans(st, cl) << (7 * st);
  for (int ts = 0; ts < 16; ++ts) u |= (uint64_t)jtok_trans(ts, b) << (4 * ts);
  *tab = t;
  *ttab = u;
}

}
```

### spatialflink_amd/csrc/gf_geojson_geom.hpp

```cpp
#pragma once

#include "gf_geojson.hpp"

namespace gf {

struct GeomNote {
  int32_t tcode;
  int32_t nrings;
  int32_t nverts;
  int64_t cpos;
};

GF_DHD inline bool jnum_start(char c) { return c == '-' || (c >= '0' && c <= '9'); }
template <class Src>
GF_DHD inline int64_t jarr_next(const Src& s, int64_t ve, int64_t e) {
  int64_t i = jskip(s, ve, e);
  if (i < e && s(i) == ',') i = jskip(s, i + 1, e);
  return i;
}
template <class Src>
GF_DHD inline double jnum_value(const Src& s, int64_t p, int64_t e, const uint64_t* T, int64_t* end) {
  const int64_t ve = jval_end(s, p, e);
  bool integral = false;
  jnumber(s, p, ve, &integral);
  double v = 0.0;
  parse_java_double(s, Field{p, ve}, T, &v);
  *end = ve;
  return integral && v == 0.0 ? 0.0 : v;
}

template <class Src>
GF_DHD inline int gpos_check(const Src& s, int64_t p, int64_t e, int64_t* end) {
  if (s(p) != '[') return kCsvMissingField;
  int64_t i = jskip(s, p + 1, e);
  int n = 0;
  while (i < e && s(i) != ']') {
    if (n < 2 && !jnum_start(s(i))) return kCsvNumberFormat;
    n += n < 3;
    i = jarr_next(s, jval_end(s, i, e), e);
  }
  *end = i + 1;
  return n == 2 ? kCsvOk : kCsvUnsupported;
}
template <class Src>
GF_DHD inline int gchain_check(const Src& s, int64_t p, int64_t e, int least, int64_t* count, int64_t* end) {
  if (s(p) != '[') return kCsvMissingField;
  int64_t i = jskip(s, p + 1, e);
  if (i < e && s(i) == ']') return kCsvUnsupported;
  int64_t n = 0;
  while (i < e && s(i) != ']') {
    int64_t pe = 0;
    const int st = gpos_check(s, i, e, &pe);
    if (st) return st;
    ++n;
    i = jarr_next(s, pe, e);
  }
  *count = n;
  *end = i + 1;
  return n < least ? kCsvMissingField : kCsvOk;
}
template <class Src>
GF_DHD inline int gpoly_check(const Src& s, int64_t p, int64_t e, int64_t* nrings, int64_t* nverts, int64_t* end) {
  if (s(p) != '[') return kCsvMissingField;
  int64_t i = jskip(s, p + 1, e);
  if (i < e && s(i) == ']') return kCsvUnsupported;
  int64_t nr = 0, nv = 0;
  while (i < e && s(i) != ']') {
    int64_t n = 0, re = 0;
    const int st = gchain_check(s, i, e, 4, &n, &re);
    if (st) return st;
    ++nr;
    nv += n;
    i = jarr_next(s, re, e);
  }
  *nrings = nr;
  *nverts = nv;
  *end = i + 1;
  return kCsvOk;
}
template <class Src>
GF_DHD inline int64_t geom_taken(const Src& s, int64_t cpos, int64_t e, int tcode) {
  return tcode == kTyMultiPolygon || tcode == kTyMultiLineString ? jskip(s, cpos + 1, e) : cpos;
}
template <class Src>
GF_DHD inline int geom_struct(const Src& s, int64_t cpos, int64_t e, int tcode, int64_t* nrings, int64_t* nverts) {
  const bool poly = tcode == kTyPolygon || tcode == kTyMultiPolygon;
  int64_t end = 0, nr = 0, nv = 0;
  if (tcode == kTyPolygon) return gpoly_check(s, cpos, e, nrings, nverts, &end);
  *nrings = 0;
  if (tcode == kTyLineString) return gchain_check(s, cpos, e, 2, nverts, &end);
  int64_t i = jskip(s, cpos + 1, e);
  if (i < e && s(i) == ']') return kCsvUnsupported;
  for (bool first = true; i < e && s(i) != ']'; first = false) {
    const int st = poly ? gpoly_check(s, i, e, &nr, &nv, &end) : gchain_check(s, i, e, 2, &nv, &end);
    if (st) return st;
    if (first) {
      *nrings = nr;
      *nverts = nv;
    }
    i = jarr_next(s, end, e);
  }
  return kCsvOk;
}

template <class Src>
GF_DHD inline int64_t gpos_read(const Src& s, int64_t p, int64_t e, const uint64_t* T, double* x, double* y) {
  int64_t i = jskip(s, p + 1, e), ve = 0;
  *x = jnum_value(s, i, e, T, &ve);
  i = jarr_next(s, ve, e);
  *y = jnum_value(s, i, e, T, &ve);
  return jskip(s, ve, e) + 1;
}
template <class Src>
GF_DHD inline bool gring_closed(const Src& s, int64_t p, int64_t e, const uint64_t* T, int64_t* end) {
  int64_t i = jskip(s, p + 1, e), last = i;
  double x0, y0, x1, y1;
  gpos_read(s, i, e, T, &x0, &y0);
  while (s(i) != ']') {
    last = i;
    i = jarr_next(s, jval_end(s, i, e), e);
  }
  gpos_read(s, last, e, T, &x1, &y1);
  *end = i + 1;
  return x0 == x1 && y0 == y1;
}
template <class Src>
GF_DHD inline bool gpoly_closed(const Src& s, int64_t p, int64_t e, const uint64_t* T, int64_t* end) {
  int64_t i = jskip(s, p + 1, e);
  while (s(i) != ']') {
    int64_t re = 0;
    if (!gring_closed(s, i, e, T, &re)) return false;
    i = jarr_next(s, re, e);
  }
  *end = i + 1;
  return true;
}
template <class Src>
GF_DHD inline bool geom_closed(const Src& s, int64_t cpos, int64_t e, int tcode, const uint64_t* T) {
  int64_t end = 0;
  if (tcode == kTyPolygon) return gpoly_closed(s, cpos, e, T, &end);
  if (tcode != kTyMultiPolygon) return true;
  int64_t i = jskip(s, cpos + 1, e);
  while (s(i) != ']') {
    if (!gpoly_closed(s, i, e, T, &end)) return false;
    i = jarr_next(s, end, e);
  }
  return true;
}

template <class Src>
GF_DHD inline bool jdup_names(const Src& s, int64_t obj, int64_t e) {
  bool esc = false;
  auto after = [&](int64_t ke) {
    return jskip(s, jval_end(s, jskip(s, jskip(s, ke, e) + 1, e), e), e);
  };
  int64_t p = jskip(s, obj + 1, e);
  while (p < e && s(p) == '"') {
    const int64_t ke = jstr_end(s, p, e, &esc);
    const int64_t nx = after(ke);
    int64_t q = nx;
    while (q < e && s(q) == ',') {
      q = jskip(s, q + 1, e);
      const int64_t qe = jstr_end(s, q, e, &esc);
      bool same = qe - q == ke - p;
      for (int64_t k = 0; same && k < ke - p; ++k) same = s(q + k) == s(p + k);
      if (same) return true;
      q = after(qe);
    }
    if (nx >= e || s(nx) != ',') break;
    p = jskip(s, nx + 1, e);
  }
  return false;
}
GF_DHD inline bool geom_type_allowed(int kind, int t) {
  return kind == GF_GEOM_POLYGON ? (t == kTyPolygon || t == kTyMultiPolygon)
                                 : (t == kTyLineString || t == kTyMultiLineString);
}
template <class Src>
GF_DHD inline int geom_build(const Src& s, int64_t V, int64_t c, int64_t e, int tcode, bool values, const uint64_t* T,
                             GeomNote* o) {
  if (c < 0 || s(c) != '[') return kCsvMissingField;
  for (int64_t i = V; i < c; ++i) {
    const char b = s(i);
    if (b == '[' || b == ']' || b == '\\') return kCsvUnsupported;
  }
  int64_t nr = 0, nv = 0;
  const int st = geom_struct(s, c, e, tcode, &nr, &nv);
  if (st) return st;
  if (values && !geom_closed(s, c, e, tcode, T)) return kCsvMissingField;
  o->tcode = tcode;
  o->nrings = (int32_t)nr;
  o->nverts = (int32_t)nv;
  o->cpos = c;
  return kCsvOk;
}

template <class Src>
GF_DHD inline int geom_eval_body(const GeoProps& a, const Src& s, int64_t e, const GeoPos& g, int kind, bool values,
                                 GeomNote* n, LineOut* o) {
  if (g.V < 0 || s(g.V) != '{') return kCsvMissingField;
  if (g.escV) return kCsvUnsupported;
  if (jdup_names(s, g.V, e)) return kCsvUnsupported;
  o->ts = 0;
  o->obj = GF_OBJID_NULL;
  o->dict = false;
  const int tv = geo_type_full(s, g.tV, e);
  if (tv == kTyFeatureColl || tv == kTyEscaped) return kCsvUnsupported;
  const bool own = tv == kTyPoint || tv >= kTyLineString;
  bool have = false;
  if (own) {
    if (!geom_type_allowed(kind, tv)) return kCsvUnsupported;
    const int st = geom_build(s, g.V, g.cV, e, tv, values, a.pow5, n);
    if (st == kCsvUnsupported) return st;
    have = st == kCsvOk;
  }
  if (!have) {
    if (g.gV < 0 || s(g.gV) != '{') return kCsvMissingField;
    if (g.escG) return kCsvUnsupported;
    if (jdup_names(s, g.gV, e)) return kCsvUnsupported;
    const int tg = geo_type_full(s, g.tG, e);
    if (tg == kTyNone) return kCsvMissingField;
    if (!geom_type_allowed(kind, tg)) return kCsvUnsupported;
    const int st = geom_build(s, g.V, g.cG, e, tg, values, a.pow5, n);
    if (st) return st;
    if (own) return kCsvUnsupported;
  }
  if (g.prV < 0 || s(g.prV) != '{') return kCsvOk;
  if (g.escP && (a.len_ts >= 0 || a.len_obj >= 0)) return kCsvUnsupported;
  return geo_props(a, s, e, g.tsP, g.qP, o);
}

template <class Src>
GF_DHD GF_NOINLINE int geom_line_eval(GeoProps a, Src s, int64_t p, int64_t e, int vlines, int kind, bool values,
                                      GeomNote* n, LineOut* o) {
  if (e - p >= (int64_t)INT32_MAX) return kCsvUnsupported;
  const int vs = jvalidate(s, p, e, a.pow5);
  if (vs) return vs;
  GeoPos g;
  const int fs = geo_walk_find(a, s, p, e, vlines, &g);
  if (fs) return fs;
  return geom_eval_body(a, s, e, g, kind, values, n, o);
}

template <class Src>
GF_DHD inline int32_t gchain_read(const Src& s, int64_t p, int64_t e, const uint64_t* T, double* x, double* y,
                                  double* area2, int64_t* end) {
  int64_t i = jskip(s, p + 1, e);
  int32_t n = 0;
  double a = 0.0, px = 0.0, py = 0.0;
  while (s(i) != ']') {
    double cx, cy;
    const int64_t pe = gpos_read(s, i, e, T, &cx, &cy);
    if (x) {
      x[n] = cx;
      y[n] = cy;
    }
    if (n > 0) a += px * cy - cx * py;
    px = cx;
    py = cy;
    ++n;
    i = jarr_next(s, pe, e);
  }
  *area2 = a;
  *end = i + 1;
  return n;
}
struct RingTmp {
  double* area;
  int64_t* start;
  int32_t* count;
  int32_t* order;
};
template <class Src>
GF_DHD inline void geom_fill(const Src& s, int64_t e, const GeomNote& n, const uint64_t* T, int32_t vbase, int32_t* voff,
                             const RingTmp& t, double* vx, double* vy) {
  const int64_t op = geom_taken(s, n.cpos, e, n.tcode);
  double a2 = 0.0;
  int64_t end = 0;
  if (n.nrings == 0) {
    gchain_read(s, op, e, T, vx + vbase, vy + vbase, &a2, &end);
    return;
  }
  if (n.nrings == 1) {
    voff[0] = vbase;
    gchain_read(s, jskip(s, op + 1, e), e, T, vx + vbase, vy + vbase, &a2, &end);
    return;
  }
  int64_t i = jskip(s, op + 1, e);
  for (int32_t r = 0; r < n.nrings; ++r) {
    t.start[r] = i;
    t.count[r] = gchain_read(s, i, e, T, (double*)nullptr, (double*)nullptr, &a2, &end);
    t.area[r] = (a2 < 0.0 ? -a2 : a2) / 2.0;
    i = jarr_next(s, end, e);
  }
  int32_t m = 0;
  for (int32_t r = 0; r < n.nrings; ++r) {
    const double ar = t.area[r];
    if (m == 0 || t.area[t.order[m - 1]] >= ar) {
      t.order[m++] = r;
      continue;
    }
    int32_t at = 0;
    while (at < m && !(t.area[t.order[at]] <= ar)) ++at;
    for (int32_t k = m; k > at; --k) t.order[k] = t.order[k - 1];
    t.order[at] = r;
    ++m;
  }
  int32_t off = vbase;
  for (int32_t k = 0; k < n.nrings; ++k) {
    const int32_t r = t.order[k];
    voff[k] = off;
    gchain_read(s, t.start[r], e, T, vx + off, vy + off, &a2, &end);
    off += t.count[r];
  }
}

}
```

### spatialflink_amd/csrc/gf_internal.hpp

```cpp
#pragma once

#include <hip/hip_runtime.h>

#include <cstdint>
#include <string>
#include <vector>

#include "../../include/geoflink_hip.h"
#include "gf_text.hpp"
#include "gf_numerics.hpp"

struct gf_ctx {
  int device = 0;
  hipStream_t stream = nullptr;
  hipStream_t own_stream = nullptr;
  std::string last_error;
  int timing = 0;
  int timing_period = 1;
  int64_t timing_seq[GF_K_COUNT] = {};
  struct Ev { hipEvent_t a, b; int kid; };
  std::vector<Ev> pending;
  std::vector<hipEvent_t> pool;
  std::vector<hipEvent_t> order_pool;
  double acc_ms[GF_K_COUNT] = {};
  int64_t acc_n[GF_K_COUNT] = {};
  void* scratch = nullptr;
  size_t scratch_bytes = 0;
  void* pinned = nullptr;
  size_t pinned_bytes = 0;
  int num_cus = 256;
  int join_legacy = 0;
  int join_coarse = 0;
  int join_stream = 0;
  int geojson_walk = 0;
  int geojson_wave = 0;
  unsigned long long* geojson_check = nullptr;
  int64_t csv_mean_line[2] = {0, 0};
  int64_t geom_mean_line = 0;
  int join_async_done = 0;
  double join_ppp = 0.0;
  hipStream_t aux = nullptr;
  hipStream_t aux2 = nullptr;
  gf_objid_dict* dict = nullptr;
  unsigned long long* expand_ticket = nullptr;
  unsigned long long expand_base = 0;
  unsigned long long* expand_status = nullptr;
  int64_t expand_status_cap = 0;
  uint32_t expand_epoch = 0;
  unsigned long long* join_gctr = nullptr;
  unsigned long long* join_hint = nullptr;
  void* csv_head = nullptr;
  uint64_t* join_hist = nullptr;
  unsigned long long* join_ovf = nullptr;
  int64_t join_hint_no = 0;
};

struct gf_objid_dict {
  gf_ctx* ctx = nullptr;
  void* slots = nullptr;
  uint64_t cap = 0;
  char* arena = nullptr;
  uint64_t arena_cap = 0;
  unsigned long long* counters = nullptr;
  unsigned long long* idmap = nullptr;
  uint64_t idmap_cap = 0;
  int64_t size = 0;
  uint32_t round = 2;
  void* work[3] = {nullptr, nullptr, nullptr};
  uint64_t work_cap = 0;
  uint32_t* slot_of = nullptr;
  uint32_t* flag = nullptr;
  uint32_t* rank = nullptr;
  uint32_t* tmp = nullptr;
  uint64_t line_cap = 0;
  char* src = nullptr;
  uint64_t src_cap = 0;
  std::vector<unsigned long long> h_idmap;
  std::vector<char> h_arena;
};

namespace gf {

int set_err(gf_ctx* ctx, int code, const std::string& msg);
int hip_err(gf_ctx* ctx, hipError_t e, const char* what);
void* ctx_scratch(gf_ctx* ctx, size_t bytes, int* status);
int sync_aux(gf_ctx* ctx);
void* ctx_pinned(gf_ctx* ctx, size_t bytes, int* status);
int bind(gf_ctx* ctx);

#define GF_HIP_CHECK(ctx, call)                                   \
  do {                                                            \
    hipError_t _e = (call);                                       \
    if (_e != hipSuccess) return ::gf::hip_err((ctx), _e, #call); \
  } while (0)

struct KTimer {
  gf_ctx* ctx;
  int kid;
  hipEvent_t a = nullptr, b = nullptr;
  KTimer(gf_ctx* c, int k);
  ~KTimer();
};

constexpr int kBlock = 256;
constexpr int kMaxK = 512;
constexpr int kFusedSelectMaxK = 256;
constexpr int kSampleBlocks = 128;
constexpr int kSamplePerBlock = 2048;
constexpr int64_t kSampleMinN = 1 << 20;

__device__ __forceinline__ void lds_barrier() {
  __atomic_signal_fence(__ATOMIC_SEQ_CST);
  __builtin_amdgcn_s_waitcnt(0xC07F);
  __builtin_amdgcn_s_barrier();
  __atomic_signal_fence(__ATOMIC_SEQ_CST);
}

__device__ __forceinline__ void wave_lds_sync() {
  __builtin_amdgcn_fence(__ATOMIC_RELEASE, "wavefront");
  __builtin_amdgcn_wave_barrier();
  __builtin_amdgcn_fence(__ATOMIC_ACQUIRE, "wavefront");
}

struct QueryRect {
  AxisIv cgx, cgy;
  AxisIv gx, gy;
  int g_any;
  double minX, minY;
};

struct KnnState {
  uint32_t hist[kDistBins];
  uint32_t ticket;
  uint32_t pad;
  double T;
  double s_pre;
  unsigned long long count;
  double hint_T;
  unsigned long long tr[4];
  unsigned long long maybe;
};

struct KnnScanArgs {
  const double* x;
  const double* y;
  const int64_t* objID;
  int64_t begin, end;
  double qx, qy;
  QueryRect qr;
  double T, s_pre;
  int use_state;
  int metric;
  KnnState* st;
  double* cand_d;
  uint32_t* cand_i;
  int64_t* cand_o;
  unsigned long long cap;
};

struct KnnSampleArgs {
  const double* x;
  const double* y;
  int64_t n;
  double qx, qy;
  QueryRect qr;
  double r, s_r;
  int32_t k;
  int metric;
  int use_hint;
  KnnState* st;
};

struct PolyView {
  const int32_t* ring_off;
  const int32_t* vert_off;
  const double* vx;
  const double* vy;
  const double* ring_env;
  int metric;
  const uint8_t* rect;
};

constexpr int kChainRun = 32;
constexpr int kChainPlainRuns = 2;
constexpr int kChainPlainRunsValue = 4;
struct ChainView {
  const int32_t* run_off;
  const int32_t* vert_off;
  const double* vx;
  const double* vy;
  const double* run_env;
  int metric;
};

struct KnnPolyArgs {
  const double* x;
  const double* y;
  const int64_t* objID;
  int64_t begin, end;
  QueryRect qr;
  PolyView poly;
  double bbox[4];
  int approx;
  double r;
  int32_t k;
  int use_state;
  int use_hint;
  KnnState* st;
  double* cand_d;
  uint32_t* cand_i;
  int64_t* cand_o;
  unsigned long long cap;
  uint32_t* maybe_i;
};

struct KnnSelectArgs {
  KnnState* st;
  const double* cand_d;
  const uint32_t* cand_i;
  const int64_t* cand_o;
  unsigned long long cap;
  int use_state;
  double T;
  double r;
  int32_t k;
  int write_hint;
  int64_t idx_base;
  void* result;
};

constexpr int kRangeMaxParts = 4096;
constexpr int kRangeTicketSlot = 2 * kRangeMaxParts;

struct RangeArgs {
  const double* x;
  const double* y;
  int64_t n;
  uint64_t* bitmap;
  uint64_t* multi;
  uint64_t* partials;
  int64_t* counts;
  int32_t nq;
  QueryRect qr;
  int32_t grid_n;
  double minX, minY, cl;
  const uint8_t* table;
  const uint32_t* rows;
  const uint32_t* rowoff;
  const uint8_t* spans;
  int32_t span_bytes;
  int32_t span_lds;
  const double* xt;
  const double* yt;
  double x_lo, x_hi, y_lo, y_hi;
  double sx_lo, sx_hi;
  double sy_lo, sy_hi;
  int span_mode;
  double inv_cl;
  const int32_t* extra;
  int32_t n_extra;
  const int32_t* cand_off;
  const int32_t* cand_list;
  int approx;
  int metric;
  double r, s_r;
  double thr;
  double qx0, qy0;
  const double* qx;
  const double* qy;
  int32_t npoly;
  const int32_t* ring_off;
  const int32_t* vert_off;
  const double* vx;
  const double* vy;
  const double* bbox;
  const double* ring_env;
  uint32_t* queue;
  uint32_t* queue_count;
  double* queue_xy;
  int64_t seg_cap;
  int32_t drain_lanes;
  const uint8_t* rect;
  const int32_t* brect;
  int32_t g_layers, c_layers;
};

hipError_t launch_assign(gf_ctx* ctx, const gf_grid* g, const gf_points* p, int32_t* cx, int32_t* cy);
hipError_t launch_histogram(hipStream_t s, const uint32_t* keys, int64_t n, uint32_t* hist);
constexpr int kRadixMaxBits = 9;
constexpr int kRadixMaxDigits = 1 << kRadixMaxBits;
constexpr int kRadixThreads = 1024;
constexpr int kRadixTile = 8192;
#ifndef GF_BUCKET_BITS
#define GF_BUCKET_BITS 9
#endif
constexpr int kBucketBits = GF_BUCKET_BITS;
static_assert(kBucketBits >= 1 && kBucketBits <= kRadixMaxBits, "K2 digit bits");
struct RadixArgs {
  const double* x;
  const double* y;
  int64_t n;
  double minX, minY, cl;
  int32_t gn;
  const uint32_t* kin;
  const uint32_t* vin;
  uint32_t* kout;
  uint32_t* vout;
  int shift, bits;
  int nblk;
  uint32_t* M;
  const uint32_t* Ms;
  const uint32_t* n_dev;
  int32_t nbands;
  int32_t band_lo[64];
  uint32_t bins;
  int32_t tile;
  int32_t rowmode;
  int32_t seg;
  const uint32_t* MsA;
  int32_t nblkA;
  uint32_t* cstart;
  uint16_t* kout16;
  const uint16_t* kin16;
  int32_t self_count;
  int32_t rowsort;
  uint32_t* multiseg;
};
int radix_threads();
inline int radix_tile() { return radix_threads() / 64 * 512; }
inline int radix_max_blocks(int num_cus) { return num_cus * (1024 / radix_threads()); }
int radix_row_sort_cap();
constexpr int kMaxShardBands = 64;
size_t radix_scatter_lds_bytes();
hipError_t launch_gather_points(hipStream_t s, const gf_points& in, const uint32_t* perm, int64_t begin, int64_t m,
                                double* ox, double* oy, int64_t* oo, int64_t* ot);
hipError_t launch_radix(gf_ctx* ctx, int stage, const RadixArgs& a, int blocks);
size_t scan_tmp_elems(int64_t L);
hipError_t launch_exclusive_scan(hipStream_t s, const uint32_t* in, int64_t L, uint32_t* out, uint32_t* tmp);
hipError_t launch_word_popcounts(hipStream_t s, const uint64_t* bitmap, int64_t words, uint32_t* pc);
hipError_t launch_expand_bitmap(hipStream_t s, const uint64_t* bitmap, int64_t words, int64_t n,
                                const uint32_t* off, uint32_t* idx, int64_t cap);
constexpr uint64_t kLbAgg = 1ull, kLbInc = 2ull;
__device__ __forceinline__ uint64_t lb_pack(uint32_t epoch, uint64_t flag, uint64_t v) {
  return ((uint64_t)(epoch & 0x3FFFFFFu) << 38) | (flag << 36) | v;
}
struct ExpandState {
  unsigned long long* ticket;
  unsigned long long base;
  unsigned long long* status;
  uint32_t epoch;
};
constexpr int kExpandWords = 1024;
int64_t expand_blocks(int64_t words);
int64_t scan1_blocks(int64_t L);
hipError_t launch_scan1(hipStream_t s, uint32_t* in, int64_t L, uint32_t* out, uint32_t* out2, int64_t n2, int64_t nz,
                        const ExpandState& st, const uint32_t* skip_if_zero = nullptr);
hipError_t launch_expand_bitmap_async(hipStream_t s, const uint64_t* bitmap, int64_t words, int64_t n, uint32_t* idx,
                                      int64_t cap, int64_t* count, const ExpandState& st);
constexpr int kRangeBatchMax = 16;
struct ExpandBatch {
  const uint64_t* bm[kRangeBatchMax];
  int64_t n[kRangeBatchMax];
  uint32_t* idx[kRangeBatchMax];
  int64_t cap[kRangeBatchMax];
  int64_t* count[kRangeBatchMax];
  int32_t tile0[kRangeBatchMax + 1];
  int32_t nwin;
};
hipError_t launch_expand_batch(hipStream_t s, const ExpandBatch& b, const ExpandState& st);

struct DictSlot {
  unsigned long long tag;
  unsigned long long meta;
  long long id;
  unsigned int first;
  unsigned int round;
};
struct DictWork {
  int64_t b;
  int32_t n;
  uint32_t line;
};
struct DictDev {
  DictSlot* slots;
  uint64_t mask;
  char* arena;
  unsigned long long* arena_used;
  unsigned long long* idmap;
};
struct DictBatch {
  const char* src;
  int quotes;
  const DictWork* work;
  uint32_t nwork;
  DictWork* pend_out;
  uint32_t* npend_out;
  uint32_t* slot_of;
  uint32_t* flag;
  const uint32_t* rank;
  uint32_t round, round0;
  int64_t id_base;
  int64_t* keys;
};
hipError_t launch_dict(hipStream_t st, int stage, const DictDev& d, const DictBatch& B);
hipError_t launch_dict_rehash(hipStream_t st, const DictDev& d, int64_t n);
int dict_reserve_batch(gf_objid_dict* d, uint64_t nwork, uint64_t lines);
int dict_reserve_table(gf_objid_dict* d, uint64_t more, uint64_t bytes);
int dict_run(gf_objid_dict* d, const char* src, int quotes, uint32_t nwork, uint64_t lines, int64_t* keys);
int ctx_dict(gf_ctx* ctx, gf_objid_dict** out);

constexpr int64_t kCsvSeg = 64 * 1024;
constexpr int kCsvLds = 24 * 1024;
constexpr int kCsvLdsMax = 64 * 1024;
struct CsvErr {
  unsigned long long line;
  int kind;
  int pad;
};
struct CsvHead {
  unsigned long long newlines;
  unsigned long long lines;
  unsigned long long dict_n;
  unsigned long long dict_bytes;
  CsvErr err;
};
struct CsvArgs {
  const char* text;
  int64_t len;
  const int64_t* nl;
  const uint32_t* nl_total;
  int64_t nl_cap;
  int64_t cap;
  int64_t grid_lines;
  int64_t mean_line;
  CsvHead* head;
  char delim;
  int32_t want[4];
  double* x;
  double* y;
  int64_t* objID;
  int64_t* ts;
  int32_t* cx;
  int32_t* cy;
  double minX, minY, cl;
  CsvErr* err;
  DictWork* dict_work;
  uint32_t* dict_n;
  unsigned long long* dict_bytes;
  int32_t format;
  int32_t len_obj, len_ts;
  int32_t date_fmt;
  int64_t tz_off_ms;
  char prop_obj[kGeoPropMax];
  char prop_ts[kGeoPropMax];
  int32_t lds_cap;
  int32_t geo_fast;
  int32_t geo_wave;
  unsigned long long* geo_check;
  int32_t value_lines;
};
hipError_t launch_csv_nlindex(hipStream_t st, const char* text, int64_t len, int64_t nseg, int64_t* nl, int64_t nl_cap,
                              uint32_t* total, const ExpandState& es, CsvErr* err, unsigned long long* dict_counters);
int lookback_state(gf_ctx* ctx, int64_t blocks, ExpandState* es);
hipError_t launch_csv_parse(gf_ctx* ctx, const CsvArgs& a);

hipError_t launch_pane_bounds(hipStream_t s, const int64_t* ts, int64_t n, int64_t pane_ms, int64_t first_pane,
                              int32_t nb, int64_t* bounds);

constexpr unsigned long long kTrajEmpty = 0x7FFFFFFFFFFFFFFEull;
constexpr int64_t kTrajLongLen = 2048;
struct TrajTable {
  unsigned long long* key;
  uint32_t* first;
  uint64_t mask;
};
struct TrajGroupArgs {
  TrajTable t;
  const int64_t* objID;
  int64_t n;
  uint32_t* flag;
  const uint32_t* rank;
  int64_t* keys;
  uint32_t* did;
  const uint32_t* sorted;
  uint32_t ntraj;
  uint32_t* seg_off;
};
enum TrajGroupStage {
  kTrajGroupInsert = 0,
  kTrajGroupAssign = 1,
  kTrajGroupBounds = 2,
};
hipError_t launch_traj_group(gf_ctx* ctx, int stage, const TrajGroupArgs& a);
struct TStatsArgs {
  const double* x;
  const double* y;
  const int64_t* ts;
  const uint32_t* perm;
  const uint32_t* seg_off;
  int64_t ntraj;
  uint32_t long_len;
  double* S;
  int64_t* T;
  double* V;
  uint32_t* long_list;
  uint32_t* long_count;
};
hipError_t launch_tstats(gf_ctx* ctx, const TStatsArgs& a);
enum TStatsFilterStage {
  kTStatsFilterMark = 0,
  kTStatsFilterPack = 1,
};
hipError_t launch_tstats_filter(gf_ctx* ctx, const TStatsArgs& a, const int64_t* keys, const int64_t* set, int64_t nset,
                                uint32_t* sel, const uint32_t* rank, int64_t* ok, double* oS, int64_t* oT, double* oV,
                                int stage);
struct TrajSelectArgs {
  const double* x;
  const double* y;
  const int64_t* ts;
  int64_t n, ntraj;
  const uint64_t* bitmap;
  const uint32_t* did;
  const uint32_t* sorted;
  const uint32_t* perm;
  const uint32_t* seg_off;
  const int64_t* keys;
  uint32_t* hit;
  uint32_t* len;
  const uint32_t* row;
  const uint32_t* off;
  int64_t* okeys;
  uint32_t* ooff;
  double* ox;
  double* oy;
  int64_t* ots;
  uint32_t* oidx;
};
enum TrajSelectStage {
  kTrajSelectHit = 0,
  kTrajSelectGather = 1,
  kTrajSelectLens = 2,
};
hipError_t launch_traj_select(gf_ctx* ctx, int stage, const TrajSelectArgs& a);

constexpr int64_t kTaggLongLen = 2048;
constexpr int64_t kTaggBigCell = 1024;
struct TaggArgs {
  const double* x;
  const double* y;
  int64_t n;
  double minX, minY, cl;
  int64_t* ckey;
  const uint32_t* cid;
  const uint32_t* oid;
  int64_t* comp;
  const int64_t* ts;
  const uint32_t* perm;
  const uint32_t* seg_off;
  const uint32_t* sorted;
  const int64_t* gkeys;
  const int64_t* okeys;
  int64_t ngroups;
  uint32_t long_len;
  uint32_t* g_cell;
  uint32_t* g_m;
  int64_t* g_key;
  int64_t* g_L;
  int64_t* g_e;
  uint32_t* g_f;
  uint32_t* g_s;
  uint32_t* list;
  uint32_t* list_count;
  const uint32_t* gperm;
  const uint32_t* cell_off;
  const int64_t* ckeys;
  int64_t ncells;
  uint32_t big_cell;
  int32_t* c_cx;
  int32_t* c_cy;
  int64_t* c_count;
  int64_t* c_multi;
  int64_t* c_sum;
  int64_t* c_minLen;
  int64_t* c_minKey;
  int64_t* c_maxLen;
  int64_t* c_maxKey;
  int64_t* all_key;
  int64_t* all_len;
};
enum TaggStage {
  kTaggCellKeys = 0,
  kTaggPairKeys = 1,
  kTaggGroupStats = 2,
  kTaggCells = 3,
};
hipError_t launch_tagg(gf_ctx* ctx, int stage, const TaggArgs& a);

constexpr int64_t kTknnBigCell = 512;
constexpr unsigned long long kTknnNaN = 0x7FF8000000000000ull;
constexpr unsigned long long kTknnNone = ~0ull;
struct TknnArgs {
  const double* x;
  const double* y;
  const uint32_t* did;
  int64_t n;
  double minX, minY, cl, qx, qy;
  int32_t xlo, xhi, ylo, yhi;
  int32_t naive;
  int64_t* e_ckey;
  uint32_t* e_t;
  unsigned long long* e_d;
  uint32_t* e_i;
  uint32_t* counters;
  int64_t m;
  const uint32_t* cid;
  int64_t* comp;
  const uint32_t* pid;
  int64_t npairs;
  const int64_t* pkeys;
  uint32_t* p_first;
  unsigned long long* p_d;
  uint32_t* p_cell;
  uint32_t* p_rec;
  const uint32_t* gperm;
  const uint32_t* gcell;
  const uint32_t* cell_off;
  const uint32_t* sperm;
  uint32_t big_cell;
  int32_t k;
  int64_t ntraj;
  const uint32_t* seg_off;
  unsigned long long* tr_D;
  uint32_t* tr_cells;
  uint32_t* surv;
  const uint32_t* srank;
  uint32_t* slist;
  int64_t rows, npts;
  const uint32_t* order;
  const int64_t* tkeys;
  const uint32_t* perm;
  const int64_t* ts;
  int64_t* o_key;
  double* o_dist;
  int32_t* o_cells;
  uint32_t* o_traj;
  uint32_t* o_len;
  const uint32_t* o_off;
  double* o_x;
  double* o_y;
  int64_t* o_ts;
  uint32_t* o_idx;
};
enum TknnStage {
  kTknnScanWindow = 0,
  kTknnCompose = 1,
  kTknnPairMin = 2,
  kTknnRankSmall = 3,
  kTknnRankBig = 4,
  kTknnCombine = 5,
  kTknnSurvivors = 6,
  kTknnRows = 7,
  kTknnGather = 8,
};
hipError_t launch_tknn(gf_ctx* ctx, int stage, const TknnArgs& a);
hipError_t launch_tknn_word(gf_ctx* ctx, const unsigned long long* src, const uint32_t* index, int shift,
                            const uint32_t* cur, int64_t cnt, uint32_t* out);

constexpr int64_t kTjoinSlots = 1 << 16;
constexpr int64_t kTjoinMinSlots = 16;
constexpr unsigned long long kTjoinEmpty = ~0ull;
constexpr int kTjoinShardStride = 32;
constexpr uint32_t kTjoinMaxShards = 1024;
struct TjoinTable {
  unsigned long long* key;
  uint32_t* qrank;
  uint32_t* pfirst;
  uint64_t mask;
  uint32_t* count;
  uint32_t shard_shift;
  uint32_t shard_cap;
  uint32_t* overflow;
};
struct TjoinArgs {
  const double* qx;
  const double* qy;
  const int64_t* qts;
  const uint32_t* qdid;
  const uint32_t* qseg;
  const uint32_t* qperm;
  const int64_t* qkeys;
  int64_t nq, ntq;
  const uint32_t* bkey;
  const int32_t* qcx;
  const int32_t* qcy;
  unsigned long long* its;
  unsigned long long* comp;
  const uint32_t* ord;
  uint32_t* qrank;
  uint32_t* qord;
  const uint32_t* sidx;
  double2* sxy;
  int4* smeta;
  uint32_t* sqr;
  uint32_t* flag;
  const uint32_t* fscan;
  uint32_t* rstart;
  uint32_t* boff;
  int64_t nb;
  const double* ox;
  const double* oy;
  const int64_t* ots;
  const uint32_t* odid;
  const uint32_t* oseg;
  const uint32_t* operm;
  const int64_t* okeys;
  int64_t no, nto;
  unsigned long long* ocell;
  const uint32_t* oord;
  double minX, minY, cl, r;
  int32_t qn;
  int64_t c;
  int32_t single;
  TjoinTable t;
  int64_t slots, rows;
  uint32_t* occ;
  const uint32_t* cpos;
  unsigned long long* rkey;
  uint32_t* rqr;
  uint32_t* rpf;
  const uint32_t* rorder;
  int64_t* o_okey;
  int64_t* o_qkey;
  uint32_t* o_pfirst;
  uint32_t* o_qlatest;
  uint8_t* o_emit;
  int32_t* o_oslot;
  int32_t* o_qslot;
  uint32_t* o_to;
  uint32_t* o_tq;
  uint32_t* mark[2];
  const uint32_t* mrank[2];
  uint32_t* counters;
  int32_t side;
  int64_t nt;
  uint32_t* tlist[2];
  uint32_t* tlen[2];
  const uint32_t* toff[2];
  int64_t m, npts;
  int64_t* c_keys;
  double* c_x;
  double* c_y;
  int64_t* c_ts;
  uint32_t* c_idx;
};
enum TjoinStage {
  kTjoinQueryKeys = 0,
  kTjoinQueryRank = 1,
  kTjoinQueryScatter = 2,
  kTjoinRunStarts = 3,
  kTjoinRunEnds = 4,
  kTjoinCellKeys = 5,
  kTjoinProbe = 6,
  kTjoinOccupied = 7,
  kTjoinCompact = 8,
  kTjoinRows = 9,
  kTjoinRowSlots = 10,
  kTjoinSideList = 11,
  kTjoinTotals = 12,
  kTjoinGather = 13,
};
hipError_t launch_tjoin(gf_ctx* ctx, int stage, const TjoinArgs& a);

struct TrangeArgs {
  const double* x;
  const double* y;
  int64_t n;
  const uint32_t* did;
  uint32_t* hit;
  uint64_t* bitmap;
  int32_t grid_n;
  double minX, minY, cl;
  const uint8_t* cls;
  const int32_t* cand_off;
  const int32_t* cand_list;
  const int32_t* extra;
  int32_t n_extra;
  PolyView poly;
  const uint8_t* wide;
  uint2* work;
  uint32_t work_cap;
  unsigned long long* ctr;
  int64_t* count;
};
enum TrangeStage {
  kTrangeMark = 0,
  kTrangeWaves = 1,
  kTrangeCount = 2,
};
hipError_t launch_trange(gf_ctx* ctx, int stage, const TrangeArgs& a);

struct GeomArgs {
  int32_t kind;
  int64_t nobj, nrings;
  const int32_t* ring_off;
  const int32_t* vert_off;
  const double* vx;
  const double* vy;
  const int64_t* objID;
  int32_t wide_vertices;
  double minX, minY, cl;
  double* ring_env;
  uint8_t* ring_ok;
  uint32_t* ring_wide;
  double* env;
  int32_t* cells;
  uint8_t* valid;
  int32_t* nvert;
  unsigned long long* ictr;
  int32_t grid_n;
  const int32_t* satN;
  const int32_t* satG;
  const double* qx;
  const double* qy;
  int32_t nq;
  double r;
  int approx, metric;
  int knn;
  uint64_t* bitmap;
  uint32_t* work_short;
  uint32_t* work_wide;
  unsigned long long* qctr;
  int64_t* counts;
  KnnState* st;
  double* cand_d;
  uint32_t* cand_i;
  int64_t* cand_o;
};
enum GeomStage {
  kGeomRingEnv = 0,
  kGeomRingEnvWide = 1,
  kGeomObjects = 2,
  kGeomClassify = 3,
  kGeomExactShort = 4,
  kGeomExactWide = 5,
  kGeomCount = 6,
};
hipError_t launch_geom(gf_ctx* ctx, int stage, const GeomArgs& a);

struct GeomPairArgs {
  GeomArgs g;
  int32_t qkind;
  const int32_t* q_ring_off;
  const int32_t* q_vert_off;
  const double* qvx;
  const double* qvy;
  const double* q_ring_env;
  const double* q_env;
  const int32_t* q_run_off;
  const double* q_run_env;
  int32_t corner;
  int32_t q_rect[4];
};
enum GeomPairStage {
  kGeomPairClassify = 0,
  kGeomPairShort = 1,
  kGeomPairWide = 2,
};
hipError_t launch_geompair(gf_ctx* ctx, int stage, const GeomPairArgs& a);

struct GeomJoinSide {
  int32_t kind;
  int32_t wide_vertices;
  int64_t n;
  const int32_t* ring_off;
  const int32_t* vert_off;
  const double* vx;
  const double* vy;
  const double* ring_env;
  const double* env;
  const int32_t* cells;
  const uint8_t* valid;
  const int32_t* nvert;
};
struct GeomJoinArgs {
  GeomJoinSide o, q;
  const double* px;
  const double* py;
  int32_t* pcells;
  double qminX, qminY, qcl;
  int32_t n;
  int32_t c;
  int32_t out_members;
  int32_t whole;
  double r;
  int approx, metric, first_is_ordinary;
  int32_t shift;
  int64_t nt;
  int64_t long_tiles;
  int brute;
  uint32_t* short_o;
  uint32_t* long_o;
  uint32_t* short_q;
  uint32_t* long_q;
  uint32_t* act_q;
  uint32_t* tile_cnt;
  uint32_t* tile_off;
  uint32_t* tile_cur;
  uint32_t* tile_q;
  uint32_t* cand;
  unsigned long long n_lane, n_wave;
  unsigned long long rect_pairs;
  uint32_t* pairs;
  int64_t cap;
  unsigned long long* ctr;
};
enum GeomJoinCtr {
  kGeomJoinCtrShortO = 0, kGeomJoinCtrLongO = 1, kGeomJoinCtrShortQ = 2, kGeomJoinCtrLongQ = 3, kGeomJoinCtrActQ = 4,
  kGeomJoinCtrEntries = 5,
  kGeomJoinCtrCand = 6,
  kGeomJoinCtrFar = 7,
  kGeomJoinCtrLane = 8,
  kGeomJoinCtrWave = 9,
  kGeomJoinCtrLaneCur = 10,
  kGeomJoinCtrWaveCur = 11,
  kGeomJoinCtrHits = 12,
  kGeomJoinCtrRep = 13,
  kGeomJoinCtrOut = 14,
  kGeomJoinCtrs = 16,
};
enum GeomJoinStage {
  kGeomJoinPointCells = 0,
  kGeomJoinClass = 1,
  kGeomJoinScatter = 2,
  kGeomJoinProbeCount = 3,
  kGeomJoinProbeWrite = 4,
  kGeomJoinExact = 5,
};
hipError_t launch_geomjoin(gf_ctx* ctx, int stage, const GeomJoinArgs& a);
int knn_sorted_record(gf_ctx* ctx, const double* cd, const int64_t* co, const uint32_t* ci, unsigned long long* count,
                      unsigned long long* maybe, int64_t m, int32_t k, double T, int64_t idx_base, void* result);

hipError_t launch_knn_sample(gf_ctx* ctx, const KnnSampleArgs& a);
hipError_t launch_knn_scan(gf_ctx* ctx, const KnnScanArgs& a, int blocks, int unroll, int nt);
hipError_t launch_knn_select(gf_ctx* ctx, const KnnSelectArgs& a);
struct KnnLargeArgs {
  const double* cd;
  const int64_t* co;
  const uint32_t* ci;
  uint32_t* perm;
  int64_t m;
  int field;
  uint32_t* keys;
  uint32_t* out;
  uint32_t* cnt;
  int pass;
  unsigned long long* lane_count;
  unsigned long long* lane_maybe;
  int32_t k;
  double T;
  int64_t idx_base;
  void* result;
};
hipError_t launch_knn_large(gf_ctx* ctx, int op, const KnnLargeArgs& a);
constexpr int32_t kMaxKLarge = 1 << 24;
int knn_exact_record(gf_knn_plan* P, const gf_points* pts, void* result);

hipError_t launch_knn_poly_sample(gf_ctx* ctx, const KnnPolyArgs& a, int chain);
hipError_t launch_knn_poly_scan(gf_ctx* ctx, const KnnPolyArgs& a, int blocks, int chain);
struct KnnSelectArgs;
struct KnnMergeArgs;
hipError_t launch_knn_poly_fused(gf_ctx* ctx, const KnnPolyArgs& a, const KnnSelectArgs& prev, int has_prev,
                                 int blocks, const KnnMergeArgs* merge, int chain);
__host__ __device__ inline size_t merge_any_hash(int64_t e) {
  size_t h = 1024;
  while (h < 2 * (size_t)e) h <<= 1;
  return h;
}
__host__ __device__ inline size_t merge_any_bytes(int32_t nrec, int32_t k) {
  const int64_t e = (int64_t)nrec * k;
  return ((size_t)e * 24 + merge_any_hash(e) * 12 + 255) & ~(size_t)255;
}
hipError_t launch_knn_merge(gf_ctx* ctx, int32_t k, const void* records, int32_t nrec, size_t rec_stride,
                            int32_t nwin, size_t win_stride, void* result, size_t res_stride, int foreign,
                            void* scratch);
__host__ __device__ inline size_t str_side_off(int32_t k) { return ((size_t)4 * (k + 1) + 7) & ~(size_t)7; }
__host__ __device__ inline size_t str_record_bytes(int32_t k, int64_t cap) {
  return 32 + (size_t)24 * k + 16 + str_side_off(k) + (((size_t)cap + 7) & ~(size_t)7);
}
__host__ __device__ inline size_t strmerge_pow2(int64_t e) {
  size_t p = 2;
  while (p < (size_t)e) p <<= 1;
  return p;
}
__host__ __device__ inline size_t strmerge_bytes(int32_t nrec, int32_t k) {
  const int64_t e = (int64_t)nrec * k;
  return ((size_t)e * 40 + strmerge_pow2(e) * 4 + strmerge_pow2(2 * e) * 8 + (size_t)k * 16 + 1024) & ~(size_t)255;
}
hipError_t launch_knn_attach_strings(gf_ctx* ctx, int32_t k, const unsigned long long* idmap, const char* arena,
                                     int64_t dict_size, const void* records, int32_t nrec, int64_t cap, void* out);
hipError_t launch_knn_merge_strings(gf_ctx* ctx, int32_t k, int64_t cap, const void* records, int32_t nrec,
                                    size_t rec_stride, int32_t nwin, size_t win_stride, void* results, void* scratch);
constexpr int kMaxMergeRecs = 64;
struct KnnRecList {
  const char* rec[kMaxMergeRecs];
};
hipError_t launch_knn_merge_list(gf_ctx* ctx, int32_t k, const KnnRecList& list, int32_t nrec, void* result,
                                 void* scratch);
constexpr int kFusedMergeMaxK = 128;
struct KnnMergeArgs {
  int32_t nrec;
  void* result;
  KnnRecList list;
};
hipError_t launch_knn_fused(gf_ctx* ctx, const KnnScanArgs& a, const KnnSelectArgs& prev, int has_prev,
                            int scan_blocks, int unroll, int nt, const KnnMergeArgs* merge);
int knn_enqueue_merge(gf_knn_plan* P, const gf_points* pts, void* result, const KnnMergeArgs* merge, int* merged);
bool knn_select_pending(const gf_knn_plan* P);

hipError_t launch_range(gf_ctx* ctx, const RangeArgs& a, int table_mode, int poly, int blocks);
struct RangeWin {
  const double* x;
  const double* y;
  int64_t n;
  uint64_t* bitmap;
  uint64_t* multi;
  uint64_t* partials;
  int64_t* counts;
};
struct RangeBatch {
  RangeWin w[kRangeBatchMax];
};
hipError_t launch_range_batch(gf_ctx* ctx, const RangeArgs& a, const RangeBatch& b, int nwin, int table_mode, int poly,
                              int blocks);
struct RangeGatherArgs {
  const uint32_t* list[kMaxMergeRecs];
  const int64_t* cnt[kMaxMergeRecs];
  int64_t base[kMaxMergeRecs];
  int32_t npanes;
  int64_t total;
  uint32_t* out;
  int64_t* count;
};
hipError_t launch_range_window_gather(hipStream_t s, const RangeGatherArgs& a);
hipError_t launch_join_ppoly(gf_ctx* ctx, const RangeArgs& a, int blocks, int jblocks, uint32_t* ecnt, uint32_t* ecand,
                             uint32_t* btot, unsigned long long* total, uint32_t* pairs, int64_t cap, int aligned,
                             int poly);

struct JoinArgs {
  const double* ox;
  const double* oy;
  int64_t no;
  double u_minX, u_minY, u_cl;
  int32_t qn;
  int64_t c;
  const uint32_t* q_off;
  const double* sqx;
  const double* sqy;
  const int32_t* sqcx;
  const int32_t* sqcy;
  const uint32_t* sqidx;
  int approx;
  int metric;
  double r;
  uint32_t* counts;
  const uint32_t* offsets;
  uint32_t* pairs;
};
hipError_t launch_join_qkeys(hipStream_t s, const double* qx, const double* qy, int64_t nq, double minX,
                             double minY, double cl, int32_t qn, uint32_t* keys, int32_t* qcx, int32_t* qcy);
hipError_t launch_join_qscatter(hipStream_t s, const double* qx, const double* qy, const int32_t* qcx,
                                const int32_t* qcy, const uint32_t* keys, int64_t nq, uint32_t* cursor,
                                double* sqx, double* sqy, int32_t* sqcx, int32_t* sqcy, uint32_t* sqidx);
hipError_t launch_join_probe(gf_ctx* ctx, const JoinArgs& a, int write_pass, int blocks);

constexpr int kJoinTask = 8192;
constexpr int kJoinThreads = 1024;
constexpr int kJoinMaxRows = 16;
struct JoinOut {
  uint32_t* pairs;
  uint64_t cap;
  int aligned;
  uint32_t chunk;
  uint2* spill;
  uint64_t spill_cap;
  unsigned long long* gctr;
  uint64_t* tail_base;
  uint32_t* tail_fill;
  uint32_t nwaves;
  int regions;
  uint64_t* bcount;
  uint64_t* bslice;
  uint64_t* hist;
  unsigned long long* ovf;
  uint64_t e_lim;
  double ppp;
};
struct JoinFixup {
  JoinOut o;
  unsigned long long* total;
  unsigned long long* hint;
  uint64_t* hole_start;
  uint64_t* hole_pref;
  uint64_t* seg_start;
  uint64_t* seg_pref;
  uint32_t* counts;
};
struct JoinRowArgs {
  const double* ox;
  const double* oy;
  int64_t no;
  double u_minX, u_minY, u_cl;
  int32_t qn;
  int64_t c;
  const uint32_t* q_off;
  const double* sqx;
  const double* sqy;
  const int32_t* sqcx;
  const int32_t* sqcy;
  const uint32_t* sqidx;
  int approx, metric;
  double r, s_r;
  int32_t nblk;
  int32_t nrows;
  uint32_t* row_mat;
  const uint32_t* row_mat_scan;
  uint32_t mat_base;
  uint32_t* row_off_w;
  const uint32_t* row_off;
  uint32_t* task_off_w;
  const uint32_t* task_off;
  double* soxy;
  uint32_t* soidx;
  JoinOut out;
  int lds_budget;
  int32_t f;
  double fs;
  JoinFixup fx;
  unsigned long long* ticket;
};
__device__ __forceinline__ void join_store(uint32_t* pairs, int aligned, uint64_t pos, uint2 v) {
  if (aligned) {
    reinterpret_cast<uint2*>(pairs)[pos] = v;
  } else {
    pairs[2 * pos] = v.x;
    pairs[2 * pos + 1] = v.y;
  }
}
__device__ __forceinline__ uint2 join_load(const uint32_t* pairs, int aligned, uint64_t pos) {
  if (aligned) return reinterpret_cast<const uint2*>(pairs)[pos];
  return make_uint2(pairs[2 * pos], pairs[2 * pos + 1]);
}
hipError_t launch_join_fixup(gf_ctx* ctx, const JoinFixup& f);
hipError_t launch_join_stream(gf_ctx* ctx, const JoinRowArgs& a);
hipError_t launch_join_band(gf_ctx* ctx, const JoinRowArgs& a, int blocks);
constexpr int kJoinReg = 3;
__host__ __device__ inline size_t join_row_lds_bytes(int64_t W, uint32_t m) {
  return ((size_t)(W + 1) * 2 + 15) / 16 * 16 + (size_t)m * 16;
}
int join_probe_budget(int64_t nq, int32_t qn, int64_t c, int32_t f);
int32_t join_fine_factor(double cl, double r, int32_t qn, double maxabs);
struct JoinQueryArgs {
  const double* qx;
  const double* qy;
  int64_t nq;
  double minX, minY, cl;
  int32_t qn;
  int32_t nblk;
  uint32_t* qmat;
  const uint32_t* qmat_scan;
  double* txy;
  uint32_t* tidx;
  uint32_t* q_off;
  double* sqx;
  double* sqy;
  int32_t* sqcx;
  int32_t* sqcy;
  uint32_t* sqidx;
  int32_t f;
  double fs;
};
hipError_t launch_join_rows(gf_ctx* ctx, const JoinRowArgs& a, const JoinQueryArgs& q, int stage);
size_t join_scatter_lds_bytes(int32_t nrows, int tile);


}

struct gf_range_plan {
  gf_ctx* ctx = nullptr;
  gf_grid grid{};
  double r = 0;
  int approx = 0, metric = 0, poly = 0, table_mode = 0;
  int32_t nq = 0, g_layers = 0, c_layers = 0;
  gf::QueryRect qr{};
  double qx0 = 0, qy0 = 0;
  uint8_t* table = nullptr;
  uint32_t* rows = nullptr;
  uint32_t* rowoff = nullptr;
  uint8_t* spans = nullptr;
  int64_t span_bytes = 0;
  double* xt = nullptr;
  double* yt = nullptr;
  double x_lo = 0, x_hi = 0, y_lo = 0, y_hi = 0;
  double sx_lo = 0, sx_hi = 0;
  double sy_lo = 0, sy_hi = 0;
  double span_frac = 1.0;
  int32_t* extra = nullptr;
  int32_t n_extra = 0;
  int32_t* cand_off = nullptr;
  int32_t* cand_list = nullptr;
  double* qx = nullptr;
  double* qy = nullptr;
  int32_t npoly = 0;
  int32_t* ring_off = nullptr;
  int32_t* vert_off = nullptr;
  double* vx = nullptr;
  double* vy = nullptr;
  double* bbox = nullptr;
  double* ring_env = nullptr;
  uint64_t* partials = nullptr;
  uint64_t* batch_partials = nullptr;
  int blocks = 0;
  uint32_t* queue = nullptr;
  double* queue_xy = nullptr;
  int64_t queue_cap = 0;
  uint32_t* queue_count = nullptr;
  int64_t cls_cells[4] = {0, 0, 0, 0};
  int32_t scan_blocks = 0;
  int32_t defer_mode = 0;
  int32_t drain_lanes = 0;
  int join = 0;
  int32_t* brect = nullptr;
  uint8_t* rect = nullptr;
  uint32_t* jecnt = nullptr;
  uint32_t* jecand = nullptr;
  uint32_t* jbtot = nullptr;
  unsigned long long* jtotal = nullptr;
  int chain_mode = 0;
  int32_t* run_off = nullptr;
  double* run_env = nullptr;
};

struct gf_knn_plan {
  gf_ctx* ctx = nullptr;
  gf_grid grid{};
  double qx = 0, qy = 0, r = 0;
  int32_t k = 0;
  int metric = 0;
  gf::QueryRect qr{};
  struct Lane {
    gf::KnnState* st = nullptr;
    double* cand_d = nullptr;
    uint32_t* cand_i = nullptr;
    int64_t* cand_o = nullptr;
  } lane[6];
  int64_t cap = 0;
  int pipeline = 1;
  uint64_t seq = 0;
  int lane_warm[6] = {0, 0, 0, 0, 0, 0};
  struct Pend {
    int lane;
    void* result;
    int64_t idx_base;
    uint64_t seq;
  };
  Pend pq[3];
  int npq = 0;
  int use_hint = 1;
  int64_t idx_base = 0;
  void* tmp_result = nullptr;
  void* host_result = nullptr;
  int scan_blocks = 0;
  int scan_unroll = 2;
  int scan_nt = 1;
  int large = 0;
  int poly = 0, approx = 0;
  int32_t* ring_off = nullptr;
  int32_t* vert_off = nullptr;
  double* vx = nullptr;
  double* vy = nullptr;
  double* ring_env = nullptr;
  double bbox[4] = {0, 0, 0, 0};
  uint32_t* maybe_i[3] = {nullptr, nullptr, nullptr};
  int64_t maybe_cap = 0;
  int chain_mode = 0;
};

struct gf_window {
  gf_ctx* ctx = nullptr;
  int64_t capacity = 0, n = 0;
  double* x = nullptr;
  double* y = nullptr;
  int64_t* objID = nullptr;
  int64_t* ts = nullptr;
  bool has_objid = false, has_ts = false;
  const int64_t* objid_mapped = nullptr;
  hipStream_t copy = nullptr;
  hipEvent_t ready = nullptr, fence_main = nullptr, fence_aux = nullptr, fence_aux2 = nullptr;
  bool pending = false;
};
```

### spatialflink_amd/csrc/gf_text.hpp

```cpp
#pragma once

#include <cstdint>

#include "../../include/geoflink_hip.h"
#include "gf_decimal.hpp"

#if defined(__HIPCC__)
#define GF_NOINLINE __noinline__
#else
#define GF_NOINLINE __attribute__((noinline))
#endif

#if defined(__HIP_DEVICE_COMPILE__)
#define GF_LDS_PTR(T) const __attribute__((address_space(3))) T*
#else
#define GF_LDS_PTR(T) const T*
#endif

namespace gf {

enum { kCsvOk = 0, kCsvNumberFormat = 1, kCsvUnsupported = 2, kCsvMissingField = 3, kCsvEmptyLine = 4 };
constexpr int kGeoPropMax = 64;
constexpr int kDictLenBits = 20;
constexpr uint64_t kDictLenMask = (1ull << kDictLenBits) - 1;

struct LineOut {
  int64_t obj, ts;
  double x, y;
  bool dict;
  Field f_obj;
};

struct GBytes {
  const char* p;
  GF_DHD char operator()(int64_t i) const { return p[i]; }
};
struct LBytes {
  GF_LDS_PTR(char) p;
  int64_t base;
  GF_DHD char operator()(int64_t i) const { return p[i - base]; }
};

}
```

### spatialflink_amd/csrc/k_geomingest.hip

```cpp
#define GF_TU_NAME k_geomingest_hip
#include "gf_buildtag.hpp"

#include "k_geomingest.hpp"

namespace gf {

static __device__ const uint64_t kPow5Geom[] = {GF_POW5_TABLE};

__device__ __forceinline__ bool geom_counts(const GeomIngestArgs& a, int64_t& newlines, int64_t& lines) {
  newlines = (int64_t)*a.nl_total;
  lines = newlines + (a.text[a.len - 1] != '\n' ? 1 : 0);
  return newlines <= a.nl_cap && lines <= a.grid_lines;
}
template <class Src>
__device__ __forceinline__ int geom_bounds(const GeomIngestArgs& a, const Src& s, int64_t j, int64_t newlines, int64_t& p,
                                           int64_t& e) {
  const int64_t b = j == 0 ? 0 : a.nl[j - 1] + 1;
  e = j < newlines ? a.nl[j] : a.len;
  if (e > b && s(e - 1) == '\r') --e;
  if (e <= b) return kCsvEmptyLine;
  p = jskip(s, b, e);
  if (p >= e || s(p) != '{') return kCsvMissingField;
  return kCsvOk;
}
__device__ __forceinline__ bool geom_stage(const GeomIngestArgs& a, char* lds, int64_t L0, int64_t L1, int64_t newlines,
                                           int64_t& a0) {
  const int64_t b0 = L0 == 0 ? 0 : a.nl[L0 - 1] + 1;
  const int64_t b1 = L1 - 1 < newlines ? a.nl[L1 - 1] : a.len;
  a0 = b0 & ~(int64_t)15;
  if (b1 - a0 > a.lds_cap) return false;
  for (int64_t off = a0 + 16 * threadIdx.x; off < b1; off += 16 * kGeomLines) {
    if (off + 16 <= a.len) {
      *reinterpret_cast<uint4*>(lds + (off - a0)) = *reinterpret_cast<const uint4*>(a.text + off);
    } else {
      for (int k = 0; k < 16 && off + k < a.len; ++k) lds[off - a0 + k] = a.text[off + k];
    }
  }
  __syncthreads();
  return true;
}
__device__ __forceinline__ GeoProps geom_props(const GeomIngestArgs& a, char* keys) {
  for (int i = threadIdx.x; i < 2 * kGeoPropMax; i += blockDim.x)
    keys[i] = i < kGeoPropMax ? a.prop_ts[i] : a.prop_obj[i - kGeoPropMax];
  __syncthreads();
  return GeoProps{keys, keys + kGeoPropMax, a.len_ts, a.len_obj, a.date_fmt, a.tz_off_ms, kPow5Geom};
}

template <class Src>
__device__ __forceinline__ int geom_eval_line(const GeomIngestArgs& a, const GeoProps& gp, const Src& s, int64_t j,
                                              int64_t newlines, bool values, GeomNote* n, LineOut* o) {
  int64_t p = 0, e = 0;
  const int bs = geom_bounds(a, s, j, newlines, p, e);
  if (bs) return bs;
  return geom_line_eval(gp, s, p, e, a.value_lines, a.kind, values, n, o);
}
template <class Src>
__device__ __forceinline__ bool geom_a_line(const GeomIngestArgs& a, const GeoProps& gp, const Src& s, int64_t j,
                                            int64_t newlines, DictWork* w) {
  GeomNote n{0, 0, 0, 0};
  LineOut o{0, 0, 0.0, 0.0, false, {0, 0}};
  const int st = geom_eval_line(a, gp, s, j, newlines, false, &n, &o);
  if (st != kCsvOk) {
    atomicMin(&a.err->line, (unsigned long long)j);
    a.cnt_r[j] = 0u;
    a.cnt_v[j] = 0u;
    return false;
  }
  a.cnt_r[j] = (uint32_t)n.nrings;
  a.cnt_v[j] = (uint32_t)n.nverts;
  a.cpos[j] = n.cpos;
  a.tcode[j] = n.tcode;
  a.ts_s[j] = o.ts;
  a.obj_s[j] = o.dict ? 0 : o.obj;
  if (o.dict) *w = DictWork{o.f_obj.b, (int32_t)(o.f_obj.e - o.f_obj.b), (uint32_t)j};
  return o.dict;
}

__global__ __launch_bounds__(kGeomLines) void geom_pass_a_kernel(GeomIngestArgs a) {
  extern __shared__ __attribute__((aligned(16))) char lds[];
  __shared__ char keys[2 * kGeoPropMax];
  int64_t newlines, lines;
  const bool ok = geom_counts(a, newlines, lines);
  const int64_t L0 = (int64_t)blockIdx.x * kGeomLines;
  const int64_t j = L0 + threadIdx.x;
  if (!ok || L0 >= lines) {
    if (j < a.grid_lines) {
      a.cnt_r[j] = 0u;
      a.cnt_v[j] = 0u;
    }
    return;
  }
  const int64_t L1 = L0 + kGeomLines < lines ? L0 + kGeomLines : lines;
  const GeoProps gp = geom_props(a, keys);
  DictWork w{0, 0, 0};
  bool need = false;
  int64_t a0 = 0;
  if (geom_stage(a, lds, L0, L1, newlines, a0)) {
    if (j < L1) need = geom_a_line(a, gp, LBytes{(GF_LDS_PTR(char))lds, a0}, j, newlines, &w);
  } else if (j < L1) {
    need = geom_a_line(a, gp, GBytes{a.text}, j, newlines, &w);
  }
  if (j >= L1 && j < a.grid_lines) {
    a.cnt_r[j] = 0u;
    a.cnt_v[j] = 0u;
  }
  const uint64_t m = __ballot(need);
  if (m) {
    const int lane = threadIdx.x & 63;
    unsigned long long nb = need ? (unsigned long long)w.n : 0ull;
#pragma unroll
    for (int o = 32; o > 0; o >>= 1) nb += __shfl_xor(nb, o, 64);
    uint32_t base = 0;
    if (lane == 0) {
      base = atomicAdd(a.dict_n, (uint32_t)__popcll(m));
      atomicAdd(a.dict_bytes, nb);
    }
    base = __shfl(base, 0, 64);
    if (need) a.dict_work[base + (uint32_t)__popcll(m & ((1ull << lane) - 1ull))] = w;
  }
}

__global__ void geom_head_kernel(GeomIngestArgs a) {
  __shared__ char keys[2 * kGeoPropMax];
  int64_t newlines, lines;
  const bool ok = geom_counts(a, newlines, lines);
  const GeoProps gp = geom_props(a, keys);
  if (threadIdx.x != 0) return;
  const unsigned long long j = a.err->line;
  if (ok && j != ~0ull) {
    GeomNote n{0, 0, 0, 0};
    LineOut o{0, 0, 0.0, 0.0, false, {0, 0}};
    a.err->kind = geom_eval_line(a, gp, GBytes{a.text}, (int64_t)j, newlines, true, &n, &o);
  }
  a.head->newlines = (unsigned long long)newlines;
  a.head->lines = (unsigned long long)lines;
  a.head->nrings = ok ? a.off_r[a.grid_lines] : 0ull;
  a.head->nverts = ok ? a.off_v[a.grid_lines] : 0ull;
  a.head->dict_n = *a.dict_n;
  a.head->dict_bytes = *a.dict_bytes;
  a.head->err = *a.err;
}

template <class Src>
__device__ __forceinline__ void geom_b_line(const GeomIngestArgs& a, const Src& s, int64_t j, int64_t newlines,
                                            int64_t lines) {
  const int64_t e0 = j < newlines ? a.nl[j] : a.len;
  const int64_t b = j == 0 ? 0 : a.nl[j - 1] + 1;
  const int64_t e = e0 > b && s(e0 - 1) == '\r' ? e0 - 1 : e0;
  const GeomNote n{a.tcode[j], (int32_t)a.cnt_r[j], (int32_t)a.cnt_v[j], a.cpos[j]};
  const bool closed = geom_closed(s, n.cpos, e, n.tcode, kPow5Geom);
  if (!closed) atomicMin(&a.err->line, (unsigned long long)j);
  if (!a.fill) return;
  const int32_t r0 = (int32_t)a.off_r[j], v0 = (int32_t)a.off_v[j];
  const bool poly = a.kind == GF_GEOM_POLYGON;
  if (poly) a.ring_off[j] = r0;
  else a.vert_off[j] = v0;
  a.ts[j] = a.ts_s[j];
  a.objID[j] = a.obj_s[j];
  if (j == lines - 1) {
    const int32_t nr = (int32_t)a.off_r[a.grid_lines], nv = (int32_t)a.off_v[a.grid_lines];
    if (poly) {
      a.ring_off[lines] = nr;
      a.vert_off[nr] = nv;
    } else {
      a.vert_off[lines] = nv;
    }
  }
  if (!closed) return;
  const RingTmp t{a.tmp.area + r0, a.tmp.start + r0, a.tmp.count + r0, a.tmp.order + r0};
  geom_fill(s, e, n, kPow5Geom, v0, poly ? a.vert_off + r0 : (int32_t*)nullptr, t, a.vx, a.vy);
}

__global__ __launch_bounds__(kGeomLines) void geom_pass_b_kernel(GeomIngestArgs a) {
  extern __shared__ __attribute__((aligned(16))) char lds[];
  int64_t newlines, lines;
  geom_counts(a, newlines, lines);
  const int64_t L0 = (int64_t)blockIdx.x * kGeomLines;
  if (L0 >= a.limit) return;
  const int64_t L1 = L0 + kGeomLines < a.limit ? L0 + kGeomLines : a.limit;
  const int64_t j = L0 + threadIdx.x;
  int64_t a0 = 0;
  if (geom_stage(a, lds, L0, L1, newlines, a0)) {
    if (j < L1) geom_b_line(a, LBytes{(GF_LDS_PTR(char))lds, a0}, j, newlines, lines);
  } else if (j < L1) {
    geom_b_line(a, GBytes{a.text}, j, newlines, lines);
  }
}

hipError_t launch_geomingest_a(gf_ctx* ctx, const GeomIngestArgs& a) {
  const unsigned blocks = (unsigned)((a.grid_lines + kGeomLines - 1) / kGeomLines);
  hipLaunchKernelGGL(geom_pass_a_kernel, dim3(blocks), dim3(kGeomLines), (size_t)a.lds_cap, ctx->stream, a);
  return hipGetLastError();
}
hipError_t launch_geomingest_head(gf_ctx* ctx, const GeomIngestArgs& a) {
  hipLaunchKernelGGL(geom_head_kernel, dim3(1), dim3(64), 0, ctx->stream, a);
  return hipGetLastError();
}
hipError_t launch_geomingest_b(gf_ctx* ctx, const GeomIngestArgs& a) {
  if (a.limit <= 0) return hipSuccess;
  const unsigned blocks = (unsigned)((a.limit + kGeomLines - 1) / kGeomLines);
  hipLaunchKernelGGL(geom_pass_b_kernel, dim3(blocks), dim3(kGeomLines), (size_t)a.lds_cap, ctx->stream, a);
  return hipGetLastError();
}

}
```

### spatialflink_amd/csrc/k_geomingest.hpp

```cpp
#pragma once

#include "gf_geojson_geom.hpp"
#include "gf_internal.hpp"

namespace gf {

constexpr int kGeomLines = 64;
struct GeomHead {
  unsigned long long newlines;
  unsigned long long lines;
  unsigned long long nrings, nverts;
  unsigned long long dict_n, dict_bytes;
  CsvErr err;
};
struct GeomIngestArgs {
  const char* text;
  int64_t len;
  const int64_t* nl;
  const uint32_t* nl_total;
  int64_t nl_cap;
  int64_t grid_lines;
  int32_t kind;
  int32_t value_lines, len_obj, len_ts, date_fmt;
  int64_t tz_off_ms;
  char prop_obj[kGeoPropMax];
  char prop_ts[kGeoPropMax];
  int32_t lds_cap;
  uint32_t* cnt_r;
  uint32_t* cnt_v;
  int64_t* cpos;
  int32_t* tcode;
  int64_t* ts_s;
  int64_t* obj_s;
  const uint32_t* off_r;
  const uint32_t* off_v;
  CsvErr* err;
  GeomHead* head;
  DictWork* dict_work;
  uint32_t* dict_n;
  unsigned long long* dict_bytes;
  int32_t fill;
  int64_t limit;
  int32_t* ring_off;
  int32_t* vert_off;
  double* vx;
  double* vy;
  int64_t* objID;
  int64_t* ts;
  RingTmp tmp;
};

hipError_t launch_geomingest_a(gf_ctx* ctx, const GeomIngestArgs& a);
hipError_t launch_geomingest_head(gf_ctx* ctx, const GeomIngestArgs& a);
hipError_t launch_geomingest_b(gf_ctx* ctx, const GeomIngestArgs& a);

}
```

Measured before the change: 788.8 billion.

## Route long GeoJSON lines to whole-wave parsing with chunked LDS windows

Adds a routing kernel that lists lines at or above a byte threshold. Those lines are then parsed cooperatively by a full wavefront in dedicated blocks, using a double-buffered LDS chunk window and a ballot/prefix-scan bracket span scanner that counts rings and vertices and fills coordinates in parallel. The change targets the serial per-thread parsing of very long geometry lines, which stalls a whole wave and can overflow the staging buffer. In exchange it adds an extra kernel launch, a memset, more complex staging that skips long-line bytes, and a new tunable threshold. The measured kNN/range metric likely does not exercise GeoJSON geometry ingest.

```diff
diff --git a/include/geoflink_hip.h b/include/geoflink_hip.h
--- a/include/geoflink_hip.h
+++ b/include/geoflink_hip.h
@@ -273,6 +273,7 @@
 int gf_geojson_parse_geoms(gf_ctx* ctx, gf_objid_dict* dict , const char* text, int64_t len,
                            const gf_geojson_schema* schema, const gf_geoms_out* out, int64_t* nobj, int64_t* nrings,
                            int64_t* nverts, int64_t* bad_line, int32_t* bad_kind);
+int gf_geojson_geoms_set_long_line_bytes(gf_ctx* ctx, int64_t bytes);
 
 int gf_join_pp(gf_ctx* ctx, const gf_grid* ugrid, const gf_grid* qgrid, const gf_points* ordinary,
                const gf_points* query, double r, int approximate, int metric, uint32_t* pairs,
diff --git a/spatialflink_amd/_lib.py b/spatialflink_amd/_lib.py
--- a/spatialflink_amd/_lib.py
+++ b/spatialflink_amd/_lib.py
@@ -55,7 +55,7 @@
     "gf_knn_sliding_create", "gf_knn_sliding_destroy", "gf_knn_sliding_geometry", "gf_knn_sliding_push",
     "gf_knn_sliding_flush", "gf_knn_sliding_decode", "gf_range_sliding_create", "gf_range_sliding_destroy",
     "gf_range_sliding_geometry", "gf_range_sliding_push", "gf_pane_bounds", "gf_csv_parse", "gf_csv_parse_dict", "gf_geojson_parse",
-    "gf_geojson_parse_geoms",
+    "gf_geojson_parse_geoms", "gf_geojson_geoms_set_long_line_bytes",
     "gf_objid_dict_create", "gf_objid_dict_destroy", "gf_ctx_objid_dict", "gf_objid_dict_size", "gf_objid_intern",
     "gf_objid_decode", "gf_join_pp", "gf_join_pp_async",
     "gf_join_ppoly_plan_create", "gf_join_ppoly_run", "gf_join_ppoly",
@@ -334,6 +334,7 @@
                                          pi64], C.c_int),
             "gf_geom_join_info": ([P, pi64, pi64, pi64, pi64, pi64, pi64], C.c_int),
             "gf_geom_join_set_tuning": ([P, i32, i64, C.c_int], C.c_int),
+            "gf_geojson_geoms_set_long_line_bytes": ([P, i64], C.c_int),
         }
         for name, (argt, rest) in sig.items():
             if os.environ.get("GF_LIB_PATH") and not hasattr(L, name):
@@ -394,6 +395,10 @@
     def set_timing_period(self, period: int):
         check(lib().gf_ctx_set_timing_period(self.handle, int(period)), self.handle, "set_timing_period")
 
+    def set_geom_long_line_bytes(self, nbytes: int):
+        check(lib().gf_geojson_geoms_set_long_line_bytes(self.handle, int(nbytes)), self.handle,
+              "set_geom_long_line_bytes")
+
     def timing(self, kernel_id: int):
         ms, n = C.c_double(), C.c_int64()
         check(lib().gf_ctx_timing(self.handle, int(kernel_id), C.byref(ms), C.byref(n)), self.handle, "timing")
diff --git a/spatialflink_amd/csrc/geomingest.cpp b/spatialflink_amd/csrc/geomingest.cpp
--- a/spatialflink_amd/csrc/geomingest.cpp
+++ b/spatialflink_amd/csrc/geomingest.cpp
@@ -11,6 +11,7 @@
 
 constexpr int64_t kGeomMeanLineDefault = 768;
 
+static_assert(kGeomLongLds <= 16 * 1024, "a long line's wave works in the smallest staging area");
 static int32_t geom_lds_cap(int64_t mean) {
   const int64_t cap = (mean * kGeomLines * 5 / 4 + 1023) & ~(int64_t)1023;
   return (int32_t)std::min<int64_t>(std::max<int64_t>(cap, 16 * 1024), kCsvLdsMax);
@@ -24,6 +25,13 @@
                                "malformed JSON / no geometry / a ring or linestring JTS refuses", "empty line"};
   const int k = he.kind >= 0 && he.kind <= 4 ? he.kind : 1;
   return set_err(ctx, GF_ERR_ARG, "gf_geojson_parse_geoms: line " + std::to_string(he.line) + ": " + what[k]);
+}
+
+extern "C" int gf_geojson_geoms_set_long_line_bytes(gf_ctx* ctx, int64_t bytes) {
+  if (!ctx) return GF_ERR_ARG;
+  if (bytes < 0) return set_err(ctx, GF_ERR_ARG, "gf_geojson_geoms_set_long_line_bytes: negative");
+  ctx->geom_long_line_bytes = bytes;
+  return GF_OK;
 }
 
 extern "C" int gf_geojson_parse_geoms(gf_ctx* ctx, gf_objid_dict* dict, const char* text, int64_t len,
@@ -86,6 +94,8 @@
     int64_t* nl = nullptr;
     ar.take(d_head, 1);
     ar.take(tot, 1);
+    ar.take(a.long_n, 1);
+    ar.take(a.long_list, (size_t)G);
     ar.take(err, 1);
     ar.take(nl, (size_t)nl_cap);
     ar.take(cnt_r, (size_t)G);
@@ -120,6 +130,10 @@
     a.dict_work = (DictWork*)dict->work[0];
     a.dict_n = (uint32_t*)(dict->counters + 2);
     a.dict_bytes = dict->counters + 3;
+    a.long_bytes = ctx->geom_long_line_bytes;
+    a.long_blocks = (int32_t)std::min<int64_t>(kGeomLongBlocks, G);
+    GF_HIP_CHECK(ctx, hipMemsetAsync(a.long_n, 0, sizeof(uint32_t), ctx->stream));
+    GF_HIP_CHECK(ctx, launch_geomingest_route(ctx, a));
     GF_HIP_CHECK(ctx, launch_geomingest_a(ctx, a));
     if ((st = scan1(ctx, cnt_r, G, off_r))) return st;
     if ((st = scan1(ctx, cnt_v, G, off_v))) return st;
diff --git a/spatialflink_amd/csrc/gf_geojson.hpp b/spatialflink_amd/csrc/gf_geojson.hpp
--- a/spatialflink_amd/csrc/gf_geojson.hpp
+++ b/spatialflink_amd/csrc/gf_geojson.hpp
@@ -41,6 +41,16 @@
         p = jstr_end(s, p, e, &esc);
         if (p < 0) return -1;
         continue;
+      }
+      if constexpr (SrcHasSpan<Src>::value) {
+        if (c == '[') {
+          const SpanInfo sp = s.span(p, e);
+          if (sp.end >= 0) {
+            if (depth == 0) return sp.end;
+            p = sp.end;
+            continue;
+          }
+        }
       }
       if (c == '{' || c == '[') ++depth;
       else if ((c == '}' || c == ']') && --depth == 0) return p + 1;
@@ -153,6 +163,16 @@
     } else if (c == '"') {
       str = true;
     } else if (c == '{' || c == '[') {
+      if constexpr (SrcHasSpan<Src>::value) {
+        if (c == '[') {
+          const SpanInfo sp = s.span(i, e);
+          if (sp.end >= 0) {
+            if (d + sp.depth > kGeoMaxDepth) return true;
+            i = sp.end - 1;
+            continue;
+          }
+        }
+      }
       if (++d > kGeoMaxDepth) return true;
     } else if (c == '}' || c == ']') {
       --d;
@@ -222,6 +242,16 @@
     if (i >= e) break;
     const char c = s(i);
     if (st == V || st == A0) {
+      if constexpr (SrcHasSpan<Src>::value) {
+        if (c == '[') {
+          const SpanInfo sp = s.span(i, e);
+          if (sp.end >= 0) {
+            i = sp.end;
+            st = AF;
+            continue;
+          }
+        }
+      }
       if (c == '{' || c == '[') {
         const int d = depth++;
         const uint64_t bit = 1ull << (d & 63);
diff --git a/spatialflink_amd/csrc/gf_geojson_geom.hpp b/spatialflink_amd/csrc/gf_geojson_geom.hpp
--- a/spatialflink_amd/csrc/gf_geojson_geom.hpp
+++ b/spatialflink_amd/csrc/gf_geojson_geom.hpp
@@ -9,6 +9,33 @@
   int32_t nrings;
   int32_t nverts;
   int64_t cpos;
+};
+
+constexpr int kGeomChunkShift = 12;
+constexpr int64_t kGeomChunk = (int64_t)1 << kGeomChunkShift;
+constexpr int64_t kGeomWinBytes = 2 * kGeomChunk + 16;
+constexpr int kGeomSpanQueue = 128;
+constexpr int64_t kGeomSpanCacheOff = kGeomWinBytes, kGeomSpanQueueOff = kGeomSpanCacheOff + 64;
+constexpr int64_t kGeomLongLds = kGeomSpanQueueOff + kGeomSpanQueue * 9;
+struct WinBytes {
+  GF_LDS_PTR(char) win;
+  GF_DHD char operator()(int64_t i) const { return win[i & (2 * kGeomChunk - 1)]; }
+};
+template <class Fill>
+struct ChunkWin {
+  GF_LDS_PTR(char) win;
+  GF_LDS_PTR(int32_t) tag;
+  Fill fill;
+  GF_DHD char operator()(int64_t i) const {
+    const int32_t c = (int32_t)(i >> kGeomChunkShift);
+    const int32_t w = (int32_t)(i & (2 * kGeomChunk - 1));
+    char b = win[w];
+    if (tag[c & 1] != c) {
+      fill(c);
+      b = win[w];
+    }
+    return b;
+  }
 };
 
 GF_DHD inline bool jnum_start(char c) { return c == '-' || (c >= '0' && c <= '9'); }
@@ -86,6 +113,15 @@
 GF_DHD inline int geom_struct(const Src& s, int64_t cpos, int64_t e, int tcode, int64_t* nrings, int64_t* nverts) {
   const bool poly = tcode == kTyPolygon || tcode == kTyMultiPolygon;
   int64_t end = 0, nr = 0, nv = 0;
+  if constexpr (SrcHasSpan<Src>::value) {
+    const SpanInfo sp = s.span(cpos, e);
+    const int want = tcode == kTyLineString ? 2 : tcode == kTyMultiPolygon ? 4 : 3;
+    if (sp.end >= 0 && sp.depth == want && sp.min_chain >= (poly ? 4 : 2)) {
+      *nrings = tcode == kTyPolygon ? sp.chains : tcode == kTyMultiPolygon ? sp.first_poly_chains : 0;
+      *nverts = tcode == kTyMultiPolygon ? sp.first_poly_leaves : tcode == kTyMultiLineString ? sp.first_chain : sp.leaves;
+      return kCsvOk;
+    }
+  }
   if (tcode == kTyPolygon) return gpoly_check(s, cpos, e, nrings, nverts, &end);
   *nrings = 0;
   if (tcode == kTyLineString) return gchain_check(s, cpos, e, 2, nverts, &end);
diff --git a/spatialflink_amd/csrc/gf_internal.hpp b/spatialflink_amd/csrc/gf_internal.hpp
--- a/spatialflink_amd/csrc/gf_internal.hpp
+++ b/spatialflink_amd/csrc/gf_internal.hpp
@@ -37,6 +37,7 @@
   unsigned long long* geojson_check = nullptr;
   int64_t csv_mean_line[2] = {0, 0};
   int64_t geom_mean_line = 0;
+  int64_t geom_long_line_bytes = 2048;
   int join_async_done = 0;
   double join_ppp = 0.0;
   hipStream_t aux = nullptr;
diff --git a/spatialflink_amd/csrc/gf_text.hpp b/spatialflink_amd/csrc/gf_text.hpp
--- a/spatialflink_amd/csrc/gf_text.hpp
+++ b/spatialflink_amd/csrc/gf_text.hpp
@@ -31,6 +31,21 @@
   Field f_obj;
 };
 
+struct SpanInfo {
+  int64_t end;
+  int32_t depth;
+  int32_t leaves;
+  int32_t chains;
+  int32_t min_chain;
+  int32_t first_chain;
+  int32_t first_poly_chains;
+  int32_t first_poly_leaves;
+};
+template <class Src>
+struct SrcHasSpan {
+  static constexpr bool value = false;
+};
+
 struct GBytes {
   const char* p;
   GF_DHD char operator()(int64_t i) const { return p[i]; }
diff --git a/spatialflink_amd/csrc/k_geomingest.hip b/spatialflink_amd/csrc/k_geomingest.hip
--- a/spatialflink_amd/csrc/k_geomingest.hip
+++ b/spatialflink_amd/csrc/k_geomingest.hip
@@ -11,6 +11,13 @@
   newlines = (int64_t)*a.nl_total;
   lines = newlines + (a.text[a.len - 1] != '\n' ? 1 : 0);
   return newlines <= a.nl_cap && lines <= a.grid_lines;
+}
+__device__ __forceinline__ void geom_extent(const GeomIngestArgs& a, int64_t j, int64_t newlines, int64_t& b, int64_t& e0) {
+  b = j == 0 ? 0 : a.nl[j - 1] + 1;
+  e0 = j < newlines ? a.nl[j] : a.len;
+}
+__device__ __forceinline__ bool geom_is_long(const GeomIngestArgs& a, int64_t b, int64_t e0) {
+  return e0 - b >= a.long_bytes;
 }
 template <class Src>
 __device__ __forceinline__ int geom_bounds(const GeomIngestArgs& a, const Src& s, int64_t j, int64_t newlines, int64_t& p,
@@ -23,19 +30,52 @@
   if (p >= e || s(p) != '{') return kCsvMissingField;
   return kCsvOk;
 }
+__device__ __forceinline__ void geom_copy(const GeomIngestArgs& a, char* lds, int64_t from, int64_t to, int64_t at) {
+  for (int64_t off = from + 16 * threadIdx.x; off < to; off += 16 * kGeomLines) {
+    if (off + 16 <= a.len) {
+      *reinterpret_cast<uint4*>(lds + (at + off - from)) = *reinterpret_cast<const uint4*>(a.text + off);
+    } else {
+      for (int k = 0; k < 16 && off + k < a.len; ++k) lds[at + off - from + k] = a.text[off + k];
+    }
+  }
+}
 __device__ __forceinline__ bool geom_stage(const GeomIngestArgs& a, char* lds, int64_t L0, int64_t L1, int64_t newlines,
-                                           int64_t& a0) {
+                                           bool lng, int64_t jb, int64_t je, int64_t& a0) {
   const int64_t b0 = L0 == 0 ? 0 : a.nl[L0 - 1] + 1;
   const int64_t b1 = L1 - 1 < newlines ? a.nl[L1 - 1] : a.len;
-  a0 = b0 & ~(int64_t)15;
-  if (b1 - a0 > a.lds_cap) return false;
-  for (int64_t off = a0 + 16 * threadIdx.x; off < b1; off += 16 * kGeomLines) {
-    if (off + 16 <= a.len) {
-      *reinterpret_cast<uint4*>(lds + (off - a0)) = *reinterpret_cast<const uint4*>(a.text + off);
-    } else {
-      for (int k = 0; k < 16 && off + k < a.len; ++k) lds[off - a0 + k] = a.text[off + k];
-    }
-  }
+  const int64_t base = b0 & ~(int64_t)15;
+  const uint64_t m = __ballot(lng);
+  if (m == 0) {
+    a0 = base;
+    if (b1 - base > a.lds_cap) return false;
+    geom_copy(a, lds, base, b1, 0);
+    __syncthreads();
+    return true;
+  }
+  const int lane = threadIdx.x & 63;
+  const long long cb = lng ? (long long)((jb + 15) & ~(int64_t)15) : 0;
+  long long cn = lng ? (long long)(je & ~(int64_t)15) - cb : 0;
+  if (cn < 0) cn = 0;
+  int64_t cut = 0, before = 0;
+  for (uint64_t mm = m; mm; mm &= mm - 1) {
+    const int l = __ffsll((unsigned long long)mm) - 1;
+    const int64_t n = (int64_t)__shfl(cn, l, 64);
+    cut += n;
+    if (lane > l) before += n;
+  }
+  a0 = base + before;
+  if (b1 - base - cut > a.lds_cap) return false;
+  int64_t cur = base, done = 0;
+  for (uint64_t mm = m; mm; mm &= mm - 1) {
+    const int l = __ffsll((unsigned long long)mm) - 1;
+    const int64_t rb = (int64_t)__shfl(cb, l, 64), n = (int64_t)__shfl(cn, l, 64);
+    if (n > 0) {
+      geom_copy(a, lds, cur, rb, cur - base - done);
+      done += n;
+      cur = rb + n;
+    }
+  }
+  geom_copy(a, lds, cur, b1, cur - base - done);
   __syncthreads();
   return true;
 }
@@ -44,6 +84,269 @@
     keys[i] = i < kGeoPropMax ? a.prop_ts[i] : a.prop_obj[i - kGeoPropMax];
   __syncthreads();
   return GeoProps{keys, keys + kGeoPropMax, a.len_ts, a.len_obj, a.date_fmt, a.tz_off_ms, kPow5Geom};
+}
+
+struct WaveFill {
+  char* win;
+  int32_t* tag;
+  const char* text;
+  int64_t len;
+  __device__ __forceinline__ void operator()(int32_t c) const {
+    const int lane = threadIdx.x & 63;
+    const int64_t g0 = (int64_t)c << kGeomChunkShift;
+    char* dst = win + ((int64_t)(c & 1) << kGeomChunkShift);
+    wave_lds_sync();
+#pragma unroll
+    for (int k = 0; k < (int)(kGeomChunk / (16 * 64)); ++k) {
+      const int64_t off = (int64_t)k * 16 * 64 + 16 * lane;
+      if (g0 + off + 16 <= len) {
+        *reinterpret_cast<uint4*>(dst + off) = *reinterpret_cast<const uint4*>(text + g0 + off);
+      } else {
+        for (int q = 0; q < 16 && g0 + off + q < len; ++q) dst[off + q] = text[g0 + off + q];
+      }
+    }
+    if (lane == 0) tag[c & 1] = c;
+    wave_lds_sync();
+  }
+};
+enum { kSpWs, kSpOpen, kSpClose, kSpComma, kSpTok, kSpBad };
+__device__ __forceinline__ int span_cls(char c) {
+  if (jws(c)) return kSpWs;
+  if (c == '[') return kSpOpen;
+  if (c == ']') return kSpClose;
+  if (c == ',') return kSpComma;
+  if ((c >= '0' && c <= '9') || c == '-' || c == '+' || c == '.' || c == 'e' || c == 'E') return kSpTok;
+  return kSpBad;
+}
+template <bool B>
+__device__ __forceinline__ bool span_leaf(const WinBytes& w, int64_t pos, int64_t lim, double* x, double* y, bool* last) {
+  int64_t i = jskip(w, pos + 1, lim);
+  for (int k = 0; k < 2; ++k) {
+    int64_t q = i;
+    while (q < lim && jtok_char(w(q))) ++q;
+    if (q == i || q >= lim) return false;
+    if constexpr (B) {
+      int64_t ve = 0;
+      (k ? *y : *x) = jnum_value(w, i, q, kPow5Geom, &ve);
+    } else {
+      if (jtok_valid(w, i, q, kPow5Geom) != 0) return false;
+    }
+    i = jskip(w, q, lim);
+    if (i >= lim) return false;
+    if (k == 0) {
+      if (w(i) != ',') return false;
+      i = jskip(w, i + 1, lim);
+      if (i >= lim) return false;
+    }
+  }
+  if (w(i) != ']') return false;
+  if constexpr (B) {
+    i = jskip(w, i + 1, lim);
+    if (i >= lim) return false;
+    *last = w(i) == ']';
+  }
+  return true;
+}
+
+struct SpanCache {
+  int64_t sb, fail;
+  SpanInfo info;
+};
+static_assert(sizeof(SpanCache) <= 64, "SpanCache's LDS slot");
+
+struct WaveSrc : ChunkWin<WaveFill> {
+  char* base;
+  __device__ SpanInfo span(int64_t p, int64_t e) const;
+};
+template <>
+struct SrcHasSpan<WaveSrc> {
+  static constexpr bool value = true;
+};
+
+template <bool B>
+__device__ bool geom_span_scan(const WaveSrc& s, int64_t p, int64_t e, SpanInfo* out, int32_t take, double* vx, double* vy,
+                               bool closure, bool* unclosed) {
+  const int lane = threadIdx.x & 63;
+  const uint64_t lt = (1ull << lane) - 1ull;
+  const WinBytes w{s.win};
+  int64_t* q = reinterpret_cast<int64_t*>(s.base + kGeomSpanQueueOff);
+  uint8_t* qf = reinterpret_cast<uint8_t*>(s.base + kGeomSpanQueueOff + kGeomSpanQueue * 8);
+  int depth = 0, D = 0;
+  int ccls = kSpComma, cpcls = kSpComma;
+  int64_t cpos = p - 1, oldest = 0, end = -1;
+  bool ctok = false;
+  int32_t tl = 0, chains = 0, cur = 0, minc = INT32_MAX, firstc = -1, fpc = -1, fpl = -1, qn = 0, done = 0;
+  double cfx = 0.0, cfy = 0.0;
+  for (int64_t b = p; b < e && end < 0; b += 64) {
+    const int64_t lastb = b + 63 < e ? b + 63 : e - 1;
+    (void)s(b);
+    (void)s(lastb);
+    const int64_t i = b + lane;
+    const bool in = i < e;
+    const int cls = in ? span_cls(w(i)) : kSpWs;
+    int incl = cls == kSpOpen ? 1 : cls == kSpClose ? -1 : 0;
+#pragma unroll
+    for (int o = 1; o < 64; o <<= 1) {
+      const int t = __shfl_up(incl, o, 64);
+      if (lane >= o) incl += t;
+    }
+    const int dafter = depth + incl;
+    const uint64_t endm = __ballot(in && cls == kSpClose && dafter == 0);
+    const int E = endm ? __ffsll((unsigned long long)endm) - 1 : 63;
+    const bool v = in && lane <= E;
+    if (__ballot(v && cls == kSpBad)) return false;
+    if (!endm && b + 64 >= e) return false;
+    const uint64_t sig = __ballot(v && cls != kSpWs);
+    const uint64_t lo = sig & lt;
+    const int pl = lo ? 63 - __clzll((unsigned long long)lo) : 0;
+    const int cls_pl = __shfl(cls, pl, 64);
+    const int pc = lo ? cls_pl : ccls;
+    const int pc_pl = __shfl(pc, pl, 64);
+    const int ppc = lo ? pc_pl : cpcls;
+    const int64_t ppos = lo ? b + pl : cpos;
+    const int cls_up = __shfl_up(cls, 1, 64);
+    const bool prevtok = lane ? cls_up == kSpTok : ctok;
+    const bool tokstart = v && cls == kSpTok && !prevtok;
+    bool viol = false;
+    if (v) {
+      if (cls == kSpOpen) viol = !(pc == kSpOpen || pc == kSpComma);
+      else if (cls == kSpClose || cls == kSpComma) viol = !(pc == kSpClose || pc == kSpTok);
+      else if (tokstart) viol = !(pc == kSpOpen || pc == kSpComma);
+    }
+    if (__ballot(viol)) return false;
+    const uint64_t tokm = __ballot(tokstart);
+    if (tokm) {
+      const int d1 = __shfl(dafter, __ffsll((unsigned long long)tokm) - 1, 64);
+      if (D == 0) D = d1;
+      if (D < 2 || D > 4 || __ballot(tokstart && dafter != D)) return false;
+    }
+    const bool leaf = tokstart && pc == kSpOpen;
+    const uint64_t leafm = __ballot(leaf);
+    if (leafm) {
+      if (qn == 0) oldest = __shfl(ppos, __ffsll((unsigned long long)leafm) - 1, 64);
+      if (leaf) {
+        const int at = qn + __popcll(leafm & lt);
+        q[at] = ppos;
+        qf[at] = ppc == kSpOpen;
+      }
+      qn += __popcll(leafm);
+    }
+    if (D) {
+      const uint64_t ccm = __ballot(v && cls == kSpClose && dafter == D - 2);
+      const uint64_t pcm = D == 4 ? __ballot(v && cls == kSpClose && dafter == 1) : 0ull;
+      if (fpc < 0 && pcm) {
+        const uint64_t below = (1ull << (__ffsll((unsigned long long)pcm) - 1)) - 1ull;
+        fpc = chains + __popcll(ccm & below);
+        fpl = tl + __popcll(leafm & below);
+      }
+      uint64_t seen = 0;
+      for (uint64_t mm = ccm; mm; mm &= mm - 1) {
+        const int l = __ffsll((unsigned long long)mm) - 1;
+        const uint64_t below = (1ull << l) - 1ull;
+        const int32_t n = cur + __popcll(leafm & below & ~seen);
+        seen = below;
+        cur = 0;
+        ++chains;
+        minc = n < minc ? n : minc;
+        if (firstc < 0) firstc = n;
+      }
+      cur += __popcll(leafm & ~seen);
+      tl += __popcll(leafm);
+    }
+    if (endm) end = b + E + 1;
+    while (qn >= 64 || (qn > 0 && (end >= 0 || b + 64 - oldest > kGeomChunk / 2))) {
+      wave_lds_sync();
+      const int64_t c0 = oldest >> kGeomChunkShift;
+      const int64_t nx = (c0 + 1) << kGeomChunkShift, lim2 = (c0 + 2) << kGeomChunkShift;
+      (void)s(oldest);
+      if (nx < e) (void)s(nx);
+      const int64_t lim = lim2 < e ? lim2 : e;
+      const int n = qn < 64 ? qn : 64;
+      const bool my = lane < n;
+      const int64_t pos = my ? q[lane] : 0;
+      const bool ff = my && qf[lane];
+      double x = 0.0, y = 0.0;
+      bool last = false;
+      const bool ok = !my || span_leaf<B>(w, pos, lim, &x, &y, &last);
+      if (__ballot(!ok)) return false;
+      if constexpr (B) {
+        const int32_t g = done + lane;
+        if (my && g < take) {
+          vx[g] = x;
+          vy[g] = y;
+        }
+        const uint64_t fm = __ballot(ff);
+        const uint64_t le = fm & (lt | (1ull << lane));
+        const int src = le ? 63 - __clzll((unsigned long long)le) : 0;
+        const double sx = __shfl(x, src, 64), sy = __shfl(y, src, 64);
+        const double fx = le ? sx : cfx, fy = le ? sy : cfy;
+        if (closure && __ballot(my && last && !(fx == x && fy == y))) *unclosed = true;
+        if (fm) {
+          const int t = 63 - __clzll((unsigned long long)fm);
+          cfx = __shfl(x, t, 64);
+          cfy = __shfl(y, t, 64);
+        }
+      }
+      const int rem = qn - n;
+      if (rem > 0) {
+        const int64_t mv = lane < rem ? q[64 + lane] : 0;
+        const uint8_t mf = lane < rem ? qf[64 + lane] : 0;
+        wave_lds_sync();
+        if (lane < rem) {
+          q[lane] = mv;
+          qf[lane] = mf;
+        }
+        wave_lds_sync();
+        oldest = q[0];
+      }
+      done += n;
+      qn = rem;
+    }
+    if (sig) {
+      const int L = 63 - __clzll((unsigned long long)sig);
+      ccls = __shfl(cls, L, 64);
+      cpcls = __shfl(pc, L, 64);
+      cpos = b + L;
+    }
+    ctok = __shfl(cls, 63, 64) == kSpTok;
+    depth += __shfl(incl, 63, 64);
+  }
+  if (end < 0 || D == 0) return false;
+  *out = SpanInfo{end, D, tl, chains, minc, firstc, fpc, fpl};
+  return true;
+}
+
+__device__ SpanInfo WaveSrc::span(int64_t p, int64_t e) const {
+  SpanCache* c = reinterpret_cast<SpanCache*>(base + kGeomSpanCacheOff);
+  const SpanInfo none{-1, 0, 0, 0, 0, 0, 0, 0};
+  const int64_t sb = c->sb;
+  if (sb == p) return c->info;
+  if (c->fail == p || (p > sb && p < c->info.end)) return none;
+  SpanInfo r = none;
+  bool un = false;
+  const bool ok = geom_span_scan<false>(*this, p, e, &r, 0, nullptr, nullptr, false, &un);
+  wave_lds_sync();
+  if ((threadIdx.x & 63) == 0) {
+    if (ok) {
+      c->sb = p;
+      c->info = r;
+    } else {
+      c->fail = p;
+    }
+  }
+  wave_lds_sync();
+  return ok ? r : none;
+}
+__device__ __forceinline__ WaveSrc geom_window(const GeomIngestArgs& a, char* lds) {
+  int32_t* tag = reinterpret_cast<int32_t*>(lds + 2 * kGeomChunk);
+  SpanCache* c = reinterpret_cast<SpanCache*>(lds + kGeomSpanCacheOff);
+  if ((threadIdx.x & 63) < 2) tag[threadIdx.x & 63] = -1;
+  if ((threadIdx.x & 63) == 0) {
+    c->sb = c->fail = -1;
+    c->info.end = -1;
+  }
+  wave_lds_sync();
+  return WaveSrc{{(GF_LDS_PTR(char))lds, (GF_LDS_PTR(int32_t))tag, WaveFill{lds, tag, a.text, a.len}}, lds};
 }
 
 template <class Src>
@@ -76,12 +379,46 @@
   return o.dict;
 }
 
+__global__ __launch_bounds__(256) void geom_route_kernel(GeomIngestArgs a) {
+  int64_t newlines, lines;
+  const bool ok = geom_counts(a, newlines, lines);
+  const int64_t j = (int64_t)blockIdx.x * blockDim.x + threadIdx.x;
+  bool lng = false;
+  if (ok && j < lines) {
+    int64_t b, e0;
+    geom_extent(a, j, newlines, b, e0);
+    lng = geom_is_long(a, b, e0);
+  }
+  const uint64_t m = __ballot(lng);
+  if (!m) return;
+  const int lane = threadIdx.x & 63;
+  uint32_t base = 0;
+  if (lane == 0) base = atomicAdd(a.long_n, (uint32_t)__popcll(m));
+  base = __shfl(base, 0, 64);
+  if (lng) a.long_list[base + (uint32_t)__popcll(m & ((1ull << lane) - 1ull))] = (uint32_t)j;
+}
+
 __global__ __launch_bounds__(kGeomLines) void geom_pass_a_kernel(GeomIngestArgs a) {
   extern __shared__ __attribute__((aligned(16))) char lds[];
   __shared__ char keys[2 * kGeoPropMax];
   int64_t newlines, lines;
   const bool ok = geom_counts(a, newlines, lines);
-  const int64_t L0 = (int64_t)blockIdx.x * kGeomLines;
+  if ((int)blockIdx.x < a.long_blocks) {
+    const uint32_t nlong = ok ? *a.long_n : 0u;
+    if (blockIdx.x >= nlong) return;
+    const GeoProps gp = geom_props(a, keys);
+    const WaveSrc s = geom_window(a, lds);
+    for (uint32_t k = blockIdx.x; k < nlong; k += (uint32_t)a.long_blocks) {
+      DictWork w{0, 0, 0};
+      const bool need = geom_a_line(a, gp, s, (int64_t)a.long_list[k], newlines, &w);
+      if (need && threadIdx.x == 0) {
+        atomicAdd(a.dict_bytes, (unsigned long long)w.n);
+        a.dict_work[atomicAdd(a.dict_n, 1u)] = w;
+      }
+    }
+    return;
+  }
+  const int64_t L0 = (int64_t)((int)blockIdx.x - a.long_blocks) * kGeomLines;
   const int64_t j = L0 + threadIdx.x;
   if (!ok || L0 >= lines) {
     if (j < a.grid_lines) {
@@ -93,11 +430,15 @@
   const int64_t L1 = L0 + kGeomLines < lines ? L0 + kGeomLines : lines;
   const GeoProps gp = geom_props(a, keys);
   DictWork w{0, 0, 0};
-  bool need = false;
-  int64_t a0 = 0;
-  if (geom_stage(a, lds, L0, L1, newlines, a0)) {
-    if (j < L1) need = geom_a_line(a, gp, LBytes{(GF_LDS_PTR(char))lds, a0}, j, newlines, &w);
-  } else if (j < L1) {
+  bool need = false, lng = false;
+  int64_t a0 = 0, jb = 0, je = 0;
+  if (j < L1) {
+    geom_extent(a, j, newlines, jb, je);
+    lng = geom_is_long(a, jb, je);
+  }
+  if (geom_stage(a, lds, L0, L1, newlines, lng, jb, je, a0)) {
+    if (j < L1 && !lng) need = geom_a_line(a, gp, LBytes{(GF_LDS_PTR(char))lds, a0}, j, newlines, &w);
+  } else if (j < L1 && !lng) {
     need = geom_a_line(a, gp, GBytes{a.text}, j, newlines, &w);
   }
   if (j >= L1 && j < a.grid_lines) {
@@ -120,18 +461,21 @@
   }
 }
 
-__global__ void geom_head_kernel(GeomIngestArgs a) {
+__global__ __launch_bounds__(kGeomLines) void geom_head_kernel(GeomIngestArgs a) {
   __shared__ char keys[2 * kGeoPropMax];
+  __shared__ __attribute__((aligned(16))) char win[kGeomLongLds];
   int64_t newlines, lines;
   const bool ok = geom_counts(a, newlines, lines);
   const GeoProps gp = geom_props(a, keys);
-  if (threadIdx.x != 0) return;
   const unsigned long long j = a.err->line;
+  int kind = 0;
   if (ok && j != ~0ull) {
     GeomNote n{0, 0, 0, 0};
     LineOut o{0, 0, 0.0, 0.0, false, {0, 0}};
-    a.err->kind = geom_eval_line(a, gp, GBytes{a.text}, (int64_t)j, newlines, true, &n, &o);
-  }
+    kind = geom_eval_line(a, gp, geom_window(a, win), (int64_t)j, newlines, true, &n, &o);
+  }
+  if (threadIdx.x != 0) return;
+  if (ok && j != ~0ull) a.err->kind = kind;
   a.head->newlines = (unsigned long long)newlines;
   a.head->lines = (unsigned long long)lines;
   a.head->nrings = ok ? a.off_r[a.grid_lines] : 0ull;
@@ -171,34 +515,92 @@
   geom_fill(s, e, n, kPow5Geom, v0, poly ? a.vert_off + r0 : (int32_t*)nullptr, t, a.vx, a.vy);
 }
 
+__device__ __forceinline__ void geom_b_long(const GeomIngestArgs& a, const WaveSrc& s, int64_t j, int64_t newlines,
+                                            int64_t lines) {
+  const int32_t nr = (int32_t)a.cnt_r[j];
+  if (nr <= 1) {
+    const int64_t e0 = j < newlines ? a.nl[j] : a.len;
+    const int64_t b = j == 0 ? 0 : a.nl[j - 1] + 1;
+    const int64_t e = e0 > b && s(e0 - 1) == '\r' ? e0 - 1 : e0;
+    const int32_t tcode = a.tcode[j], v0 = (int32_t)a.off_v[j], r0 = (int32_t)a.off_r[j];
+    const bool poly = a.kind == GF_GEOM_POLYGON;
+    SpanInfo sp;
+    bool unclosed = false;
+    if (geom_span_scan<true>(s, a.cpos[j], e, &sp, a.fill ? (int32_t)a.cnt_v[j] : 0, a.vx + v0, a.vy + v0,
+                             tcode == kTyPolygon || tcode == kTyMultiPolygon, &unclosed)) {
+      if (unclosed) atomicMin(&a.err->line, (unsigned long long)j);
+      if (!a.fill) return;
+      if (poly) {
+        a.ring_off[j] = r0;
+        a.vert_off[r0] = v0;
+      } else {
+        a.vert_off[j] = v0;
+      }
+      a.ts[j] = a.ts_s[j];
+      a.objID[j] = a.obj_s[j];
+      if (j == lines - 1) {
+        const int32_t tr = (int32_t)a.off_r[a.grid_lines], tv = (int32_t)a.off_v[a.grid_lines];
+        if (poly) {
+          a.ring_off[lines] = tr;
+          a.vert_off[tr] = tv;
+        } else {
+          a.vert_off[lines] = tv;
+        }
+      }
+      return;
+    }
+  }
+  geom_b_line(a, s, j, newlines, lines);
+}
+
 __global__ __launch_bounds__(kGeomLines) void geom_pass_b_kernel(GeomIngestArgs a) {
   extern __shared__ __attribute__((aligned(16))) char lds[];
   int64_t newlines, lines;
   geom_counts(a, newlines, lines);
-  const int64_t L0 = (int64_t)blockIdx.x * kGeomLines;
+  if ((int)blockIdx.x < a.long_blocks) {
+    const uint32_t nlong = *a.long_n;
+    if (blockIdx.x >= nlong) return;
+    const WaveSrc s = geom_window(a, lds);
+    for (uint32_t k = blockIdx.x; k < nlong; k += (uint32_t)a.long_blocks) {
+      const int64_t j = (int64_t)a.long_list[k];
+      if (j < a.limit) geom_b_long(a, s, j, newlines, lines);
+    }
+    return;
+  }
+  const int64_t L0 = (int64_t)((int)blockIdx.x - a.long_blocks) * kGeomLines;
   if (L0 >= a.limit) return;
   const int64_t L1 = L0 + kGeomLines < a.limit ? L0 + kGeomLines : a.limit;
   const int64_t j = L0 + threadIdx.x;
-  int64_t a0 = 0;
-  if (geom_stage(a, lds, L0, L1, newlines, a0)) {
-    if (j < L1) geom_b_line(a, LBytes{(GF_LDS_PTR(char))lds, a0}, j, newlines, lines);
-  } else if (j < L1) {
+  bool lng = false;
+  int64_t a0 = 0, jb = 0, je = 0;
+  if (j < L1) {
+    geom_extent(a, j, newlines, jb, je);
+    lng = geom_is_long(a, jb, je);
+  }
+  if (geom_stage(a, lds, L0, L1, newlines, lng, jb, je, a0)) {
+    if (j < L1 && !lng) geom_b_line(a, LBytes{(GF_LDS_PTR(char))lds, a0}, j, newlines, lines);
+  } else if (j < L1 && !lng) {
     geom_b_line(a, GBytes{a.text}, j, newlines, lines);
   }
 }
 
+hipError_t launch_geomingest_route(gf_ctx* ctx, const GeomIngestArgs& a) {
+  const unsigned blocks = (unsigned)((a.grid_lines + 255) / 256);
+  hipLaunchKernelGGL(geom_route_kernel, dim3(blocks), dim3(256), 0, ctx->stream, a);
+  return hipGetLastError();
+}
 hipError_t launch_geomingest_a(gf_ctx* ctx, const GeomIngestArgs& a) {
-  const unsigned blocks = (unsigned)((a.grid_lines + kGeomLines - 1) / kGeomLines);
+  const unsigned blocks = (unsigned)a.long_blocks + (unsigned)((a.grid_lines + kGeomLines - 1) / kGeomLines);
   hipLaunchKernelGGL(geom_pass_a_kernel, dim3(blocks), dim3(kGeomLines), (size_t)a.lds_cap, ctx->stream, a);
   return hipGetLastError();
 }
 hipError_t launch_geomingest_head(gf_ctx* ctx, const GeomIngestArgs& a) {
-  hipLaunchKernelGGL(geom_head_kernel, dim3(1), dim3(64), 0, ctx->stream, a);
+  hipLaunchKernelGGL(geom_head_kernel, dim3(1), dim3(kGeomLines), 0, ctx->stream, a);
   return hipGetLastError();
 }
 hipError_t launch_geomingest_b(gf_ctx* ctx, const GeomIngestArgs& a) {
   if (a.limit <= 0) return hipSuccess;
-  const unsigned blocks = (unsigned)((a.limit + kGeomLines - 1) / kGeomLines);
+  const unsigned blocks = (unsigned)a.long_blocks + (unsigned)((a.limit + kGeomLines - 1) / kGeomLines);
   hipLaunchKernelGGL(geom_pass_b_kernel, dim3(blocks), dim3(kGeomLines), (size_t)a.lds_cap, ctx->stream, a);
   return hipGetLastError();
 }
diff --git a/spatialflink_amd/csrc/k_geomingest.hpp b/spatialflink_amd/csrc/k_geomingest.hpp
--- a/spatialflink_amd/csrc/k_geomingest.hpp
+++ b/spatialflink_amd/csrc/k_geomingest.hpp
@@ -6,6 +6,7 @@
 namespace gf {
 
 constexpr int kGeomLines = 64;
+constexpr int kGeomLongBlocks = 1024;
 struct GeomHead {
   unsigned long long newlines;
   unsigned long long lines;
@@ -26,6 +27,10 @@
   char prop_obj[kGeoPropMax];
   char prop_ts[kGeoPropMax];
   int32_t lds_cap;
+  int64_t long_bytes;
+  uint32_t* long_list;
+  uint32_t* long_n;
+  int32_t long_blocks;
   uint32_t* cnt_r;
   uint32_t* cnt_v;
   int64_t* cpos;
@@ -50,6 +55,7 @@
   RingTmp tmp;
 };
 
+hipError_t launch_geomingest_route(gf_ctx* ctx, const GeomIngestArgs& a);
 hipError_t launch_geomingest_a(gf_ctx* ctx, const GeomIngestArgs& a);
 hipError_t launch_geomingest_head(gf_ctx* ctx, const GeomIngestArgs& a);
 hipError_t launch_geomingest_b(gf_ctx* ctx, const GeomIngestArgs& a);
```

After: 790.2 billion, median of 2. About the same (+0.2%).
